# 0xfaded/pislam

Measured on AMD Instinct MI355X. Metric: ORB keypoints+descriptors/sec, 640x480 8-level pyramid, higher is better.
Workload: dtype u8

## Files before the change

### include/pislam_hip.h

```cpp
#ifndef PISLAM_HIP_H_
#define PISLAM_HIP_H_

#include <stddef.h>
#include <stdint.h>

#ifdef __cplusplus
extern "C" {
#endif

#define PISLAM_OK 0
#define PISLAM_ERR_INVALID (-1)
#define PISLAM_ERR_HIP (-2)
#define PISLAM_ERR_NOMEM (-3)
#define PISLAM_ERR_DIST (-4)

#define PISLAM_ABI_VERSION 2

typedef struct pislam_ctx pislam_ctx;

int pislam_abi_version(void);
int pislam_ctx_create(int device, pislam_ctx **ctx);
int pislam_ctx_destroy(pislam_ctx *ctx);
int pislam_ctx_set_stream(pislam_ctx *ctx, void *hip_stream);
int pislam_ctx_set_option(pislam_ctx *ctx, const char *key, int value);
int pislam_ctx_synchronize(pislam_ctx *ctx);
const char *pislam_last_error(const pislam_ctx *ctx);


int pislam_fast_detect(pislam_ctx *ctx, int vstep, int border, int width, int height,
                       const uint8_t *img, uint8_t *out, int threshold);

int pislam_fast_score_harris(pislam_ctx *ctx, int vstep, int border, int width, int height,
                             const uint8_t *img, int32_t threshold, uint8_t *out);

int pislam_fast_extract(pislam_ctx *ctx, int vstep, int border, int logBucketSize,
                        int bucketLimit, int width, int height, const uint8_t *out,
                        uint32_t *results, size_t capacity, size_t *count);

int pislam_orb_compute(pislam_ctx *ctx, int vstep, int words, const uint8_t *img,
                       const uint32_t *points, size_t n, uint32_t *descriptors);


int pislam_harris_score_points(pislam_ctx *ctx, int vstep, const uint8_t *img,
                               const uint32_t *points, size_t n, int32_t threshold,
                               uint8_t *scores);

size_t pislam_centroids_size(size_t n);
int pislam_orb_centroids(pislam_ctx *ctx, int vstep, const uint8_t *img,
                         const uint32_t *points, size_t n, int32_t *centroids);

int pislam_orb_angles(pislam_ctx *ctx, const int32_t *centroids, size_t n8, uint8_t *angles);

int pislam_brief_describe(pislam_ctx *ctx, int vstep, int words, const uint8_t *img,
                          const uint32_t *points, const uint8_t *rots, size_t n,
                          uint32_t *descriptors);

const int8_t *pislam_brief_table(void);


int pislam_gaussian5x5(pislam_ctx *ctx, int vstep, int width, int height, const uint8_t *img,
                       uint8_t *out);

int pislam_bilinear7_8(pislam_ctx *ctx, int vstep, int width, int height, const uint8_t *img,
                       uint8_t *out);
int pislam_bilinear13_16(pislam_ctx *ctx, int vstep, int width, int height, const uint8_t *img,
                         uint8_t *out);

typedef struct pislam_warp pislam_warp;
int pislam_warp_create(pislam_ctx *ctx, int width, int height, int src_width, int src_height, int log_cell,
                       const int32_t *mesh_x, const int32_t *mesh_y, int border, pislam_warp **warp);
int pislam_warp_destroy(pislam_warp *warp);
int pislam_warp_mesh_dims(int width, int height, int log_cell, int32_t *mesh_w, int32_t *mesh_h);
int pislam_warp_info(const pislam_warp *warp, int32_t info[4]);
int pislam_warp_batch(pislam_ctx *ctx, const pislam_warp *warp, const uint8_t *src, int src_vstep, size_t src_stride,
                      uint8_t *dst, int dst_vstep, size_t dst_stride, int batch);


typedef struct pislam_level {
  int32_t width;
  int32_t height;
  int32_t row0;
  int32_t col0;
} pislam_level;

typedef struct pislam_frontend_params {
  int32_t vstep;
  int32_t rows;
  int32_t nlevels;
  int32_t border;
  int32_t fast_threshold;
  int32_t harris_threshold;
  int32_t log_bucket_size;
  int32_t bucket_limit;
  int32_t words;
  int32_t max_keypoints;
} pislam_frontend_params;

int pislam_pyramid_layout(int width, int height, int nlevels, const int32_t *steps, int vstep_min,
                          pislam_level *levels, int32_t *vstep, int32_t *rows);
#define PISLAM_BUILD_BLUR 1
#define PISLAM_BUILD_MARGINS_CLEAN 2
#define PISLAM_BUILD_CHECK_MARGINS 4
int pislam_pyramid_build_batch(pislam_ctx *ctx, int nlevels, const int32_t *steps, const pislam_level *levels,
                               const uint8_t *frames, int frame_vstep, size_t frame_stride, int batch,
                               uint8_t *pyramids, int vstep, int rows, size_t pyramid_stride, int flags);

int pislam_orb_frontend_batch(pislam_ctx *ctx, const pislam_frontend_params *params,
                              const pislam_level *levels, const uint8_t *pyramids,
                              size_t pyramid_stride, int batch, uint32_t *keypoints,
                              uint32_t *descriptors, uint32_t *counts);

int pislam_frontend_reserve(pislam_ctx *ctx, const pislam_frontend_params *params,
                            const pislam_level *levels, int batch);

int pislam_frontend_get_score_map(pislam_ctx *ctx, int b, uint8_t *dst);

int pislam_frontend_last_timing(pislam_ctx *ctx, float *total_ms, float stage_ms[3]);

int pislam_frontend_last_stats(pislam_ctx *ctx, uint32_t stats[2]);

#define PISLAM_PATH_STAGED 1u
#define PISLAM_PATH_FUSED 2u
#define PISLAM_PATH_ONE_LAUNCH 4u
#define PISLAM_PATH_BUCKET_SELECT 8u
#define PISLAM_PATH_BUCKETS_IN_STRIPS 16u
#define PISLAM_PATH_GENERIC_ORB 32u
#define PISLAM_PATH_FRAME_TIMED_OUT 64u
unsigned pislam_frontend_last_path(const pislam_ctx *ctx);
#define PISLAM_COUNT_INVALID 0xffffffffu

int pislam_debug_build_plan(const pislam_frontend_params *params, const pislam_level *levels, int batch, int num_cus,
                            int lanes_in_flight, const char *options, uint32_t summary[8], char *err, size_t err_cap);

typedef struct pislam_pipeline pislam_pipeline;
int pislam_pipeline_create(int device, int depth, pislam_pipeline **pipe);
int pislam_pipeline_destroy(pislam_pipeline *pipe);
int pislam_pipeline_depth(const pislam_pipeline *pipe);
int pislam_pipeline_set_option(pislam_pipeline *pipe, const char *key, int value);
int pislam_pipeline_reserve(pislam_pipeline *pipe, const pislam_frontend_params *params, const pislam_level *levels,
                            int batch);
int pislam_pipeline_submit(pislam_pipeline *pipe, const pislam_frontend_params *params, const pislam_level *levels,
                           const uint8_t *pyramids, size_t pyramid_stride, int batch, uint32_t *keypoints,
                           uint32_t *descriptors, uint32_t *counts, void *input_stream, int order_after_input,
                           uint64_t *ticket);
int pislam_pipeline_wait(pislam_pipeline *pipe, uint64_t ticket, void *stream);
int pislam_pipeline_synchronize(pislam_pipeline *pipe);
int pislam_pipeline_stats(const pislam_pipeline *pipe, uint64_t stats[4]);
void *pislam_pipeline_stream(pislam_pipeline *pipe, uint64_t ticket);
pislam_ctx *pislam_pipeline_lane(pislam_pipeline *pipe, int lane);
const char *pislam_pipeline_last_error(const pislam_pipeline *pipe);

int pislam_debug_shader_clock(pislam_ctx *ctx, int micros, double *ghz);


int pislam_match_hamming(pislam_ctx *ctx, int words, const uint32_t *query, size_t nq,
                         const uint32_t *train, size_t nt, int32_t *idx, uint32_t *dist,
                         uint32_t *dist2);

int pislam_match_hamming_batch(pislam_ctx *ctx, int words, const uint32_t *query,
                               const uint32_t *qcounts, size_t q_stride, const uint32_t *train,
                               const uint32_t *tcounts, size_t t_stride, int batch, int32_t *idx,
                               uint32_t *dist, uint32_t *dist2);

int pislam_match_window_reserve(pislam_ctx *ctx, int words, const pislam_level *levels, int nlevels,
                                const int32_t *radius, size_t t_stride, int batch);
int pislam_match_hamming_window_batch(pislam_ctx *ctx, int words,
                                      const pislam_level *levels, int nlevels, const int32_t *radius,
                                      const uint32_t *qkp, const uint32_t *qdesc, const uint32_t *qcounts,
                                      size_t q_stride, const uint32_t *tkp, const uint32_t *tdesc,
                                      const uint32_t *tcounts, size_t t_stride, int batch, int32_t *idx,
                                      uint32_t *dist, uint32_t *dist2);

int pislam_match_scaled_window_reserve(pislam_ctx *ctx, int words, const pislam_level *levels, int nlevels,
                                       const int32_t *scale_q16, const int32_t *radius0, int level_span,
                                       size_t t_stride, int batch);
int pislam_match_hamming_scaled_window_batch(pislam_ctx *ctx, int words,
                                             const pislam_level *levels, int nlevels,
                                             const int32_t *scale_q16, const int32_t *radius0, int level_span,
                                             const uint32_t *qkp, const uint32_t *qdesc, const uint32_t *qcounts,
                                             const int32_t *qpred, size_t q_stride,
                                             const uint32_t *tkp, const uint32_t *tdesc, const uint32_t *tcounts,
                                             size_t t_stride, int batch, int32_t *idx, uint32_t *dist, uint32_t *dist2);

typedef struct pislam_stereo_params {
  int32_t level_span, min_disp, max_disp, max_hamming, sad_radius, search_radius, median_filter;
} pislam_stereo_params;
int pislam_match_stereo_reserve(pislam_ctx *ctx, int words, const pislam_level *levels, int nlevels,
                                const int32_t *scale_q16, const int32_t *row_radius0, const pislam_stereo_params *p,
                                size_t r_stride, int batch);
int pislam_match_stereo_batch(pislam_ctx *ctx, int words, const pislam_level *levels, int nlevels,
                              const int32_t *scale_q16, const int32_t *row_radius0, const pislam_stereo_params *p,
                              const uint8_t *left_pyr, const uint8_t *right_pyr, int vstep, int rows,
                              size_t pyramid_stride,
                              const uint32_t *lkp, const uint32_t *ldesc, const uint32_t *lcounts, size_t l_stride,
                              const uint32_t *rkp, const uint32_t *rdesc, const uint32_t *rcounts, size_t r_stride,
                              int batch, int32_t *idx, uint32_t *dist, int32_t *disp_q8, uint32_t *sad,
                              uint32_t *nstereo);


typedef struct pislam_vocab pislam_vocab;
int pislam_vocab_create(pislam_ctx *ctx, int words, int nnodes, const uint32_t *node_desc,
                        const int32_t *first_child, const int32_t *child_count, int group_depth,
                        pislam_vocab **vocab);
int pislam_vocab_destroy(pislam_vocab *vocab);
int pislam_vocab_nwords(const pislam_vocab *vocab);
int pislam_vocab_ngroups(const pislam_vocab *vocab);

int pislam_bow_transform_batch(pislam_ctx *ctx, const pislam_vocab *vocab, const uint32_t *desc,
                               const uint32_t *counts, size_t stride, int batch,
                               uint32_t *word, uint32_t *group, uint32_t *wdist);

int pislam_bow_vector_batch(pislam_ctx *ctx, const uint32_t *word, const uint32_t *counts, size_t stride, int batch,
                            uint32_t *bow_word, uint32_t *bow_tf, uint32_t *bow_n);

int pislam_match_bow_reserve(pislam_ctx *ctx, int words, int ngroups, size_t t_stride, int batch);
int pislam_match_hamming_bow_batch(pislam_ctx *ctx, int words, int ngroups,
                                   const uint32_t *qdesc, const uint32_t *qgroup, const uint32_t *qcounts, size_t q_stride,
                                   const uint32_t *tdesc, const uint32_t *tgroup, const uint32_t *tcounts, size_t t_stride,
                                   int batch, int32_t *idx, uint32_t *dist, uint32_t *dist2);


int pislam_orb_angles_batch(pislam_ctx *ctx, const uint8_t *pyramids, int vstep, int rows, size_t pyramid_stride,
                            const uint32_t *keypoints, const uint32_t *counts, size_t stride, int batch,
                            uint8_t *angles);

typedef struct pislam_select_params {
  int32_t max_dist;
  int32_t ratio_num, ratio_den;
  int32_t unique;
  int32_t rot_keep;
  int32_t rot_min_pct;
} pislam_select_params;
int pislam_match_select_batch(pislam_ctx *ctx, const pislam_select_params *p,
                              const int32_t *idx, const uint32_t *dist, const uint32_t *dist2,
                              const uint32_t *qcounts, size_t q_stride,
                              const uint32_t *tcounts, size_t t_stride,
                              const int32_t *back_idx, const uint8_t *qangle, const uint8_t *tangle, int batch,
                              int32_t *sel_q, int32_t *sel_t, uint32_t *nsel, uint8_t *status, uint32_t *rot_hist);


int pislam_bow_weight_batch(pislam_ctx *ctx, const uint32_t *bow_word, const uint32_t *bow_tf, const uint32_t *bow_n,
                            size_t stride, int batch, const uint32_t *idf, uint32_t nwords, uint32_t *bow_weight);

typedef struct pislam_bowdb pislam_bowdb;
int pislam_bowdb_create(pislam_ctx *ctx, uint32_t nwords, size_t stride, int capacity, pislam_bowdb **db);
int pislam_bowdb_destroy(pislam_bowdb *db);
int pislam_bowdb_size(const pislam_bowdb *db);
int pislam_bowdb_add_batch(pislam_ctx *ctx, pislam_bowdb *db, const uint32_t *bow_word, const uint32_t *bow_weight,
                           const uint32_t *bow_n, size_t stride, int batch, int32_t *first_id);
int pislam_bowdb_remove(pislam_ctx *ctx, pislam_bowdb *db, const int32_t *ids, int n);
int pislam_bowdb_clear(pislam_ctx *ctx, pislam_bowdb *db);

int pislam_bowdb_query_reserve(pislam_ctx *ctx, const pislam_bowdb *db, int batch, int topk);
int pislam_bowdb_query_batch(pislam_ctx *ctx, const pislam_bowdb *db, const uint32_t *q_word, const uint32_t *q_weight,
                             const uint32_t *q_n, size_t stride, int batch, const int32_t *id_limit, int min_common_pct,
                             int topk, int32_t *top_id, uint32_t *top_score, uint32_t *top_common, uint32_t *max_common);


#define PISLAM_DIST_ID_BYTES 128

int pislam_dist_shard(int global_batch, int rank, int world, int *first, int *count);

int pislam_dist_get_unique_id(uint8_t id[PISLAM_DIST_ID_BYTES]);

int pislam_dist_init(pislam_ctx *ctx, const uint8_t id[PISLAM_DIST_ID_BYTES], int rank, int world);
int pislam_dist_rank(const pislam_ctx *ctx);
int pislam_dist_world(const pislam_ctx *ctx);
int pislam_dist_comm_count(pislam_ctx *ctx);

int pislam_dist_allgather_counts(pislam_ctx *ctx, const uint32_t *local_counts, size_t n,
                                 uint32_t *all_counts);

int pislam_dist_fence(pislam_ctx *ctx, int back);

int pislam_dist_allgather_counts_on(pislam_ctx *ctx, void *producer_stream, const uint32_t *local_counts, size_t n,
                                    uint32_t *all_counts);
int pislam_dist_fence_on(pislam_ctx *ctx, int back, void *consumer_stream);

int pislam_dist_synchronize(pislam_ctx *ctx);

int pislam_dist_allreduce_max(pislam_ctx *ctx, double *value);

int pislam_dist_finalize(pislam_ctx *ctx);

#ifdef __cplusplus
// ... 4 lines not shown
```

### pislam_amd/capi.py

```python
from __future__ import annotations

import ctypes
import os

import numpy as np

from . import build as _build

PISLAM_OK = 0
ABI_VERSION = 2

_vp, _i, _sz = ctypes.c_void_p, ctypes.c_int, ctypes.c_size_t


class Level(ctypes.Structure):
    _fields_ = [("width", ctypes.c_int32), ("height", ctypes.c_int32),
                ("row0", ctypes.c_int32), ("col0", ctypes.c_int32)]


class FrontendParams(ctypes.Structure):
    _fields_ = [(n, ctypes.c_int32) for n in (
        "vstep", "rows", "nlevels", "border", "fast_threshold", "harris_threshold",
        "log_bucket_size", "bucket_limit", "words", "max_keypoints")]


class StereoParams(ctypes.Structure):
    _fields_ = [(n, ctypes.c_int32) for n in (
        "level_span", "min_disp", "max_disp", "max_hamming", "sad_radius", "search_radius", "median_filter")]


class SelectParams(ctypes.Structure):
    _fields_ = [(n, ctypes.c_int32) for n in (
        "max_dist", "ratio_num", "ratio_den", "unique", "rot_keep", "rot_min_pct")]


SYMBOLS = {
    "pislam_abi_version": (_i, []),
    "pislam_ctx_create": (_i, [_i, ctypes.POINTER(_vp)]),
    "pislam_ctx_destroy": (_i, [_vp]),
    "pislam_ctx_set_stream": (_i, [_vp, _vp]),
    "pislam_ctx_set_option": (_i, [_vp, ctypes.c_char_p, _i]),
    "pislam_ctx_synchronize": (_i, [_vp]),
    "pislam_last_error": (ctypes.c_char_p, [_vp]),
    "pislam_fast_detect": (_i, [_vp, _i, _i, _i, _i, _vp, _vp, _i]),
    "pislam_fast_score_harris": (_i, [_vp, _i, _i, _i, _i, _vp, ctypes.c_int32, _vp]),
    "pislam_fast_extract": (_i, [_vp, _i, _i, _i, _i, _i, _i, _vp, _vp, _sz, ctypes.POINTER(_sz)]),
    "pislam_orb_compute": (_i, [_vp, _i, _i, _vp, _vp, _sz, _vp]),
    "pislam_harris_score_points": (_i, [_vp, _i, _vp, _vp, _sz, ctypes.c_int32, _vp]),
    "pislam_centroids_size": (_sz, [_sz]),
    "pislam_orb_centroids": (_i, [_vp, _i, _vp, _vp, _sz, _vp]),
    "pislam_orb_angles": (_i, [_vp, _vp, _sz, _vp]),
    "pislam_brief_describe": (_i, [_vp, _i, _i, _vp, _vp, _vp, _sz, _vp]),
    "pislam_brief_table": (ctypes.POINTER(ctypes.c_int8), []),
    "pislam_gaussian5x5": (_i, [_vp, _i, _i, _i, _vp, _vp]),
    "pislam_bilinear7_8": (_i, [_vp, _i, _i, _i, _vp, _vp]),
    "pislam_bilinear13_16": (_i, [_vp, _i, _i, _i, _vp, _vp]),
    "pislam_warp_create": (_i, [_vp, _i, _i, _i, _i, _i, _vp, _vp, _i, ctypes.POINTER(_vp)]),
    "pislam_warp_destroy": (_i, [_vp]),
    "pislam_warp_mesh_dims": (_i, [_i, _i, _i, ctypes.POINTER(ctypes.c_int32), ctypes.POINTER(ctypes.c_int32)]),
    "pislam_warp_info": (_i, [_vp, ctypes.POINTER(ctypes.c_int32 * 4)]),
    "pislam_warp_batch": (_i, [_vp, _vp, _vp, _i, _sz, _vp, _i, _sz, _i]),
    "pislam_pyramid_layout": (_i, [_i, _i, _i, ctypes.POINTER(ctypes.c_int32), _i, ctypes.POINTER(Level),
                                   ctypes.POINTER(ctypes.c_int32), ctypes.POINTER(ctypes.c_int32)]),
    "pislam_pyramid_build_batch": (_i, [_vp, _i, ctypes.POINTER(ctypes.c_int32), ctypes.POINTER(Level), _vp, _i, _sz,
                                        _i, _vp, _i, _i, _sz, _i]),
    "pislam_orb_frontend_batch": (_i, [_vp, ctypes.POINTER(FrontendParams), ctypes.POINTER(Level), _vp,
                                       _sz, _i, _vp, _vp, _vp]),
    "pislam_frontend_reserve": (_i, [_vp, ctypes.POINTER(FrontendParams), ctypes.POINTER(Level), _i]),
    "pislam_frontend_get_score_map": (_i, [_vp, _i, _vp]),
    "pislam_frontend_last_timing": (_i, [_vp, ctypes.POINTER(ctypes.c_float),
                                         ctypes.POINTER(ctypes.c_float * 3)]),
    "pislam_frontend_last_stats": (_i, [_vp, ctypes.POINTER(ctypes.c_uint32 * 2)]),
    "pislam_frontend_last_path": (ctypes.c_uint, [_vp]),
    "pislam_debug_build_plan": (_i, [ctypes.POINTER(FrontendParams), ctypes.POINTER(Level), _i, _i, _i, ctypes.c_char_p,
                                     ctypes.POINTER(ctypes.c_uint32 * 8), ctypes.c_char_p, _sz]),
    "pislam_pipeline_create": (_i, [_i, _i, ctypes.POINTER(_vp)]),
    "pislam_pipeline_destroy": (_i, [_vp]),
    "pislam_pipeline_depth": (_i, [_vp]),
    "pislam_pipeline_set_option": (_i, [_vp, ctypes.c_char_p, _i]),
    "pislam_pipeline_reserve": (_i, [_vp, ctypes.POINTER(FrontendParams), ctypes.POINTER(Level), _i]),
    "pislam_pipeline_submit": (_i, [_vp, ctypes.POINTER(FrontendParams), ctypes.POINTER(Level), _vp, _sz, _i, _vp, _vp, _vp,
                                    _vp, _i, ctypes.POINTER(ctypes.c_uint64)]),
    "pislam_pipeline_wait": (_i, [_vp, ctypes.c_uint64, _vp]),
    "pislam_pipeline_synchronize": (_i, [_vp]),
    "pislam_pipeline_stats": (_i, [_vp, ctypes.POINTER(ctypes.c_uint64 * 4)]),
    "pislam_pipeline_stream": (_vp, [_vp, ctypes.c_uint64]),
    "pislam_pipeline_lane": (_vp, [_vp, _i]),
    "pislam_pipeline_last_error": (ctypes.c_char_p, [_vp]),
    "pislam_match_hamming": (_i, [_vp, _i, _vp, _sz, _vp, _sz, _vp, _vp, _vp]),
    "pislam_match_hamming_batch": (_i, [_vp, _i, _vp, _vp, _sz, _vp, _vp, _sz, _i, _vp, _vp, _vp]),
    "pislam_match_window_reserve": (_i, [_vp, _i, ctypes.POINTER(Level), _i, ctypes.POINTER(ctypes.c_int32), _sz, _i]),
    "pislam_match_hamming_window_batch": (_i, [_vp, _i, ctypes.POINTER(Level), _i, ctypes.POINTER(ctypes.c_int32), _vp, _vp,
                                               _vp, _sz, _vp, _vp, _vp, _sz, _i, _vp, _vp, _vp]),
    "pislam_match_scaled_window_reserve": (_i, [_vp, _i, ctypes.POINTER(Level), _i, ctypes.POINTER(ctypes.c_int32),
                                                ctypes.POINTER(ctypes.c_int32), _i, _sz, _i]),
    "pislam_match_hamming_scaled_window_batch": (_i, [_vp, _i, ctypes.POINTER(Level), _i, ctypes.POINTER(ctypes.c_int32),
                                                      ctypes.POINTER(ctypes.c_int32), _i, _vp, _vp, _vp, _vp, _sz, _vp,
                                                      _vp, _vp, _sz, _i, _vp, _vp, _vp]),
    "pislam_match_stereo_reserve": (_i, [_vp, _i, ctypes.POINTER(Level), _i, ctypes.POINTER(ctypes.c_int32),
                                         ctypes.POINTER(ctypes.c_int32), ctypes.POINTER(StereoParams), _sz, _i]),
    "pislam_match_stereo_batch": (_i, [_vp, _i, ctypes.POINTER(Level), _i, ctypes.POINTER(ctypes.c_int32),
                                       ctypes.POINTER(ctypes.c_int32), ctypes.POINTER(StereoParams), _vp, _vp, _i, _i,
                                       _sz, _vp, _vp, _vp, _sz, _vp, _vp, _vp, _sz, _i, _vp, _vp, _vp, _vp, _vp]),
    "pislam_vocab_create": (_i, [_vp, _i, _i, _vp, _vp, _vp, _i, ctypes.POINTER(_vp)]),
    "pislam_vocab_destroy": (_i, [_vp]),
    "pislam_vocab_nwords": (_i, [_vp]),
    "pislam_vocab_ngroups": (_i, [_vp]),
    "pislam_bow_transform_batch": (_i, [_vp, _vp, _vp, _vp, _sz, _i, _vp, _vp, _vp]),
    "pislam_bow_vector_batch": (_i, [_vp, _vp, _vp, _sz, _i, _vp, _vp, _vp]),
    "pislam_match_bow_reserve": (_i, [_vp, _i, _i, _sz, _i]),
    "pislam_match_hamming_bow_batch": (_i, [_vp, _i, _i, _vp, _vp, _vp, _sz, _vp, _vp, _vp, _sz, _i, _vp, _vp, _vp]),
    "pislam_orb_angles_batch": (_i, [_vp, _vp, _i, _i, _sz, _vp, _vp, _sz, _i, _vp]),
    "pislam_match_select_batch": (_i, [_vp, ctypes.POINTER(SelectParams), _vp, _vp, _vp, _vp, _sz, _vp, _sz, _vp, _vp, _vp,
                                       _i, _vp, _vp, _vp, _vp, _vp]),
    "pislam_bow_weight_batch": (_i, [_vp, _vp, _vp, _vp, _sz, _i, _vp, ctypes.c_uint32, _vp]),
    "pislam_bowdb_create": (_i, [_vp, ctypes.c_uint32, _sz, _i, ctypes.POINTER(_vp)]),
    "pislam_bowdb_destroy": (_i, [_vp]),
    "pislam_bowdb_size": (_i, [_vp]),
    "pislam_bowdb_add_batch": (_i, [_vp, _vp, _vp, _vp, _vp, _sz, _i, ctypes.POINTER(ctypes.c_int32)]),
    "pislam_bowdb_remove": (_i, [_vp, _vp, _vp, _i]),
    "pislam_bowdb_clear": (_i, [_vp, _vp]),
    "pislam_bowdb_query_reserve": (_i, [_vp, _vp, _i, _i]),
    "pislam_bowdb_query_batch": (_i, [_vp, _vp, _vp, _vp, _vp, _sz, _i, _vp, _i, _i, _vp, _vp, _vp, _vp]),
    "pislam_dist_shard": (_i, [_i, _i, _i, ctypes.POINTER(_i), ctypes.POINTER(_i)]),
    "pislam_dist_get_unique_id": (_i, [ctypes.c_char_p]),
    "pislam_dist_init": (_i, [_vp, ctypes.c_char_p, _i, _i]),
    "pislam_dist_rank": (_i, [_vp]),
    "pislam_dist_world": (_i, [_vp]),
    "pislam_dist_comm_count": (_i, [_vp]),
    "pislam_dist_allgather_counts": (_i, [_vp, _vp, _sz, _vp]),
    "pislam_dist_fence": (_i, [_vp, _i]),
    "pislam_dist_allgather_counts_on": (_i, [_vp, _vp, _vp, _sz, _vp]),
    "pislam_dist_fence_on": (_i, [_vp, _i, _vp]),
    "pislam_debug_shader_clock": (_i, [_vp, _i, ctypes.POINTER(ctypes.c_double)]),
    "pislam_dist_synchronize": (_i, [_vp]),
    "pislam_dist_allreduce_max": (_i, [_vp, ctypes.POINTER(ctypes.c_double)]),
    "pislam_dist_finalize": (_i, [_vp]),
}

_LIB = None


def library_path() -> str:
    return _build.LIB


def load(rebuild_if_stale: bool = True):
    global _LIB
    if _LIB is not None:
        return _LIB
    try:
        import torch
    except ImportError:
        pass
    _build.check_override()
    path = _build.LIB
    if rebuild_if_stale:
        try:
            path = _build.build()
        except Exception:
            if not os.path.exists(path):
                raise
    if not os.path.exists(path):
        raise ImportError(f"{path} is missing: run `python -m pislam_amd.build` (hipcc, gfx950). "
                          "pislam_amd has no CPU fallback.")
    lib = ctypes.CDLL(path)
    for name, (res, args) in SYMBOLS.items():
        fn = getattr(lib, name)
        fn.restype, fn.argtypes = res, args
    if lib.pislam_abi_version() != ABI_VERSION:
        raise ImportError("libpislam_hip.so ABI version mismatch")
    _LIB = lib
    return lib


class PislamError(RuntimeError):
    pass


def dist_unique_id() -> bytes:
    buf = ctypes.create_string_buffer(128)
    rc = load().pislam_dist_get_unique_id(buf)
    if rc != PISLAM_OK:
        raise PislamError(f"pislam_dist_get_unique_id failed ({rc}): RCCL not loadable?")
    return buf.raw


def dist_shard(global_batch: int, rank: int, world: int):
    first, count = _i(0), _i(0)
    rc = load().pislam_dist_shard(global_batch, rank, world, ctypes.byref(first), ctypes.byref(count))
    if rc != PISLAM_OK:
        raise PislamError(f"pislam_dist_shard failed ({rc})")
    return first.value, first.value + count.value


def ptr(a) -> int:
    if a is None:
        return 0
    if isinstance(a, np.ndarray):
        if not a.flags.c_contiguous:
            raise ValueError("array must be C-contiguous")
        return a.ctypes.data
    if hasattr(a, "data_ptr"):
        if not a.is_contiguous():
            raise ValueError("tensor must be contiguous")
        return a.data_ptr()
    if isinstance(a, int):
        return a
    raise TypeError(f"cannot take the address of {type(a)}")


class Context:

    def __init__(self, device: int = -1, stream: int | None = None):
        self.lib = load()
        h = _vp()
        rc = self.lib.pislam_ctx_create(device, ctypes.byref(h))
        if rc != PISLAM_OK:
            raise PislamError(f"pislam_ctx_create failed ({rc}): no usable HIP device? "
                              "(there is no CPU fallback)")
        self.h = h
        if stream is not None:
            self.set_stream(stream)

    @classmethod
    def borrowed(cls, handle):
        c = cls.__new__(cls)
        c.lib = load()
# ... 137 lines not shown
```

### pislam_amd/csrc/pislam_fused_kernels.h

```cpp
#pragma once
#include "pislam_dev.h"

#ifndef PISLAM_FRAME_SLEEP
#define PISLAM_FRAME_SLEEP 16
#endif
#ifndef PISLAM_OVL
#define PISLAM_OVL 1
#endif
#ifndef PISLAM_DIAG
#define PISLAM_DIAG 1
#endif
#ifndef PISLAM_ORB_PITCH_DW
#define PISLAM_ORB_PITCH_DW 12
#endif

namespace pf {

using namespace pdev;

typedef __attribute__((address_space(3))) uint8_t lds_u8;
typedef __attribute__((address_space(3))) uint32_t lds_u32;
typedef uint32_t u32x4 __attribute__((ext_vector_type(4)));
typedef __attribute__((address_space(3))) u32x4 lds_u4;

constexpr int MAX_ORDER = 160;
constexpr int MAX_LEVELS = 24;
constexpr int WAVES = 4;
constexpr int NT = WAVES * 64;
constexpr int QCAP_G = 128;
constexpr int QCAP_F = 192;
constexpr int QCAP = QCAP_G + QCAP_F;
constexpr int QH_SHARED = 1024;
constexpr int QN_SHARED = 512;
constexpr int QS_SHARED = 256;
constexpr int SHARED_Q = QH_SHARED + QN_SHARED;
constexpr int NMS_SCRATCH = 3 * QS_SHARED;
static_assert(NMS_SCRATCH <= WAVES * QCAP, "NMS scratch must fit the per-wave queue area");
static_assert(QS_SHARED <= NT, "one survivor per thread (ranks are held in a register across a barrier)");
constexpr uint32_t STRIP_DESCRIBED = 0x80000000u;

struct FusedLevel {
  int w, h;
  int row0, col0;
  int R;
  int nstrips;
  int strip0;
  int slot0;
  int nbx;
  int xend;
  int pitch;
  int tpitch;
  int nruns, run0;
  int apad;
  int qh;
  int tbytes;
  uint32_t vpr_recip;
  uint32_t tp_recip;
  int ex0, ex1;
  int xscore;
  int gfirst, gn;
};

struct FusedParams {
  int nlevels, strips_per_pyr, slots_per_pyr;
  int runs_per_pyr, run_len;
  int vstep, rows, border, thr;
  int32_t hthr;
  int batch;
  int lbs, limit;
  int words;
  int orb_in_strip;
  int order_n;
  int dump_score;
  int ablate;
  FusedLevel lv[MAX_LEVELS];
  uint32_t order[MAX_ORDER];
};

__device__ __forceinline__ void lds_barrier() {
  __builtin_amdgcn_fence(__ATOMIC_RELEASE, "workgroup", "local");
  __builtin_amdgcn_s_barrier();
  __builtin_amdgcn_fence(__ATOMIC_ACQUIRE, "workgroup", "local");
}

__device__ __forceinline__ uint32_t lds_add_rtn(uint32_t *p, uint32_t v) {
  uint32_t old;
  const uint32_t a = (uint32_t)(uintptr_t)(lds_u32 *)p;
  asm volatile("ds_add_rtn_u32 %0, %1, %2\n\ts_waitcnt lgkmcnt(0)" : "=v"(old) : "v"(a), "v"(v) : "memory");
  return old;
}

constexpr int PF_MAX = 4;

__device__ __forceinline__ uint32_t pack_xy(int x, int r) { return (uint32_t)x | ((uint32_t)r << 16); }


__device__ __attribute__((noinline)) void harris_overflow(lds_u8 *tile, lds_u8 *sc, int tpitch, int pitch, int32_t hthr,
                                                          bool valid, uint32_t e) {
  if (valid) {
    const int x = e & 0xffff, r = (e >> 16) & 0xff;
    sc[r * pitch + x] = harris_score_mm(tile + r * tpitch + x - 3, tpitch, hthr);
  }
}

constexpr int OWAVES = 4;
constexpr int ORB_PITCH = 4 * PISLAM_ORB_PITCH_DW;
__host__ __device__ constexpr int orb_row_ofs(int r) { return PISLAM_ORB_PITCH_DW == 12 ? r * 48 + 4 * (r >> 3) : r * ORB_PITCH; }
constexpr int ORB_PATCH_BYTES = PISLAM_ORB_PITCH_DW == 12 ? 32 * 48 + 32 : (31 * ORB_PITCH + 4 + 15) / 16 * 16;

__device__ __forceinline__ void half_sum2(int &a, int &b, int half) {
  a += __builtin_amdgcn_update_dpp(0, a, 0x111, 0xf, 0xf, true);
  b += __builtin_amdgcn_update_dpp(0, b, 0x111, 0xf, 0xf, true);
  a += __builtin_amdgcn_update_dpp(0, a, 0x112, 0xf, 0xf, true);
  b += __builtin_amdgcn_update_dpp(0, b, 0x112, 0xf, 0xf, true);
  a += __builtin_amdgcn_update_dpp(0, a, 0x114, 0xf, 0xf, true);
  b += __builtin_amdgcn_update_dpp(0, b, 0x114, 0xf, 0xf, true);
  a += __builtin_amdgcn_update_dpp(0, a, 0x118, 0xf, 0xf, true);
  b += __builtin_amdgcn_update_dpp(0, b, 0x118, 0xf, 0xf, true);
  a += __builtin_amdgcn_update_dpp(0, a, 0x142, 0xa, 0xf, false);
  b += __builtin_amdgcn_update_dpp(0, b, 0x142, 0xa, 0xf, false);
  const int a0 = __builtin_amdgcn_readlane(a, 31), a1 = __builtin_amdgcn_readlane(a, 63);
  const int b0 = __builtin_amdgcn_readlane(b, 31), b1 = __builtin_amdgcn_readlane(b, 63);
  a = half ? a1 : a0;
  b = half ? b1 : b0;
}

#ifndef PISLAM_FETCH_X3
#define PISLAM_FETCH_X3 1
#endif
#if PISLAM_FETCH_X3
constexpr int ORB_NLD = 4;
struct OrbPiece {
  uint32_t x, y, z;
};
struct OrbWin {
  OrbPiece w[ORB_NLD];
};
#else
constexpr int ORB_NLD = 3;
struct OrbWin {
  uint4 w[3];
};
#endif
struct OrbLane {
  int half, r;
  int sl_h[ORB_NLD], sl_park[ORB_NLD], sl_rel[ORB_NLD];
  bool sl_on[ORB_NLD];
  uint32_t m01[8], mdx[8];
};
__device__ __forceinline__ OrbLane orb_lane(int lane, int vstep) {
  OrbLane G;
  G.half = lane >> 5;
  G.r = lane & 31;
  const uint32_t *row = ::g_orb_masks.v[G.r];
#pragma unroll
  for (int k = 0; k < 8; k++) {
    G.m01[k] = row[k];
    G.mdx[k] = row[8 + k];
  }
#if PISLAM_FETCH_X3
#pragma unroll
  for (int j = 0; j < ORB_NLD; j++) {
    const int slot = lane + 64 * j;
    const int q = slot >> 2, k = slot & 3;
    const int h = q >= 31 ? 1 : 0, row = q - 31 * h;
    G.sl_h[j] = h;
    G.sl_on[j] = q < 62;
    G.sl_rel[j] = row * vstep + 12 * k;
    G.sl_park[j] = h * ORB_PATCH_BYTES + orb_row_ofs(row) + 12 * k;
  }
#else
#pragma unroll
  for (int j = 0; j < 3; j++) {
    const int slot = lane + 64 * j;
    const int h = slot >= 93 ? 1 : 0, within = slot - 93 * h;
    const int row = within / 3, chunk = within - 3 * row;
    G.sl_h[j] = h;
    G.sl_on[j] = slot < 186;
    G.sl_rel[j] = row * vstep + 16 * chunk;
    G.sl_park[j] = h * ORB_PATCH_BYTES + orb_row_ofs(row) + 16 * chunk;
  }
#endif
  return G;
}
__device__ __forceinline__ OrbWin orb_fetch(const OrbLane &G, uint32_t p0, uint32_t p1, const uint8_t *__restrict__ im,
                                            int vstep, uint32_t img_bytes32) {
  OrbWin f;
  const int org0 = (decode_y(p0) - 15) * vstep + (decode_x(p0) - 15);
  const int org1 = (decode_y(p1) - 15) * vstep + (decode_x(p1) - 15);
  const int d01 = org1 - org0;
#if PISLAM_FETCH_X3
#pragma unroll
  for (int j = 0; j < ORB_NLD; j++) {
    const uint32_t a = min(((uint32_t)(org0 + (d01 & -G.sl_h[j])) & ~15u) + (uint32_t)G.sl_rel[j], img_bytes32 - 12u);
    f.w[j] = *(const OrbPiece *)(im + a);
  }
#else
#pragma unroll
  for (int j = 0; j < 3; j++) {
    const uint32_t a = min((uint32_t)(org0 + G.sl_rel[j] + (d01 & -G.sl_h[j])) & ~15u, img_bytes32 - 16u);
    f.w[j] = *(const uint4 *)(im + a);
  }
#endif
  return f;
}
template <class TAB, bool GHOOKS = false>
__device__ __forceinline__ void orb_describe_rows(const OrbLane &G, const lds_u8 *prow4, const uint32_t sh3, const lds_u8 *bp,
                                                  const uint32_t *__restrict__ tab_base, const bool valid, const TAB *rtab,
                                                  int words, uint8_t *__restrict__ dst_base, const uint32_t dst_word,
                                                  const int glevel = 0) {
  const int half = G.half, r = G.r;
  uint32_t row[8];
  {
    uint32_t in[9];
#pragma unroll
    for (int k = 0; k < 9; k++) in[k] = *(const lds_u32 *)(prow4 + 4 * k);
#pragma unroll
    for (int k = 0; k < 8; k++) row[k] = __builtin_amdgcn_alignbyte(in[k + 1], in[k], sh3);
  }
  uint32_t sv = 0, left = 0, right = 0;
#pragma unroll
  for (int k = 0; k < 8; k++) sv = __builtin_amdgcn_udot4(row[k], G.m01[k], sv, false);
#pragma unroll
  for (int k = 0; k < 4; k++) left = __builtin_amdgcn_udot4(row[k], G.mdx[k], left, false);
#pragma unroll
  for (int k = 4; k < 8; k++) right = __builtin_amdgcn_udot4(row[k], G.mdx[k], right, false);
  int m10 = (int)right - (int)left, m01 = __mul24(r - 15, (int)sv);
  half_sum2(m10, m01, half);
  if (GHOOKS && glevel == 4) {
    asm volatile("" ::"v"(m10), "v"(m01));
    return;
  }
  const uint32_t rot = angle_bin_fast(m10, m01, rtab);
  if (GHOOKS && glevel == 5) {
    asm volatile("" ::"v"(rot));
    return;
  }
  const uint32_t *tab = tab_base + rot * 256 + r;
  uint32_t ent[8];
#pragma unroll
  for (int t = 0; t < 8; t++) ent[t] = tab[32 * t];
  if (GHOOKS && glevel == 6) {
#pragma unroll
    for (int t = 0; t < 8; t++) asm volatile("" ::"v"(ent[t]));
    return;
  }
  uint32_t pa[8], pb[8];
#pragma unroll
  for (int t = 0; t < 8; t++) pa[t] = bp[ent[t] & 0xffffu], pb[t] = bp[ent[t] >> 16];
  uint32_t acc = 0;
#pragma unroll
  for (int t = 7; t >= 0; t--) acc = __builtin_amdgcn_alignbit(acc, pa[t] - pb[t], 31);
  const uint32_t n1 = (uint32_t)__builtin_amdgcn_update_dpp(0, (int)acc, 0xf5, 0xf, 0xf, true);
  const uint32_t hw = __builtin_amdgcn_perm(n1, acc, 0x0c0c0400u);
  const uint32_t n2 = (uint32_t)__builtin_amdgcn_update_dpp(0, (int)hw, 0xaa, 0xf, 0xf, true);
  const uint32_t word4 = __builtin_amdgcn_perm(n2, hw, 0x05040100u);
  const uint32_t word = (uint32_t)__builtin_amdgcn_ds_bpermute((int)(4u * (32u * (uint32_t)half + 4u * ((uint32_t)r & 7u))), (int)word4);
  if (GHOOKS && glevel == 7) {
    asm volatile("" ::"v"(word));
    return;
  }
  if (valid && r < words) *(uint32_t *)(dst_base + (dst_word * 4u + 4u * (uint32_t)r)) = word;
}

template <class TAB, bool GHOOKS = false>
__device__ __forceinline__ void orb_describe(const OrbLane &G, const OrbWin &cur, uint32_t p0, uint32_t p1,
                                             lds_u8 *wave_patches, int vstep, const TAB *rtab, int words,
                                             uint8_t *__restrict__ dst_base, const uint32_t dst_word, const int glevel = 0) {
  const int half = G.half, r = G.r;
  if (GHOOKS && glevel == 2) {
#pragma unroll
    for (int j = 0; j < ORB_NLD; j++) asm volatile("" ::"v"(cur.w[j].x), "v"(cur.w[j].y), "v"(cur.w[j].z));
    return;
  }
  const uint32_t pme = half ? p1 : p0;
  const bool valid = pme != 0;
  const int x = decode_x(pme), y = decode_y(pme);
  const uint32_t sh = (uint32_t)(x + 1) & 15u;
#pragma unroll
  for (int j = 0; j < ORB_NLD; j++)
    if (G.sl_on[j]) {
      lds_u32 *d = (lds_u32 *)(wave_patches + G.sl_park[j]);
      d[0] = cur.w[j].x;
      d[1] = cur.w[j].y;
      d[2] = cur.w[j].z;
#if !PISLAM_FETCH_X3
      d[3] = cur.w[j].w;
#endif
    }
  if (GHOOKS && glevel == 3) return;
  lds_u8 *patch_l = wave_patches + half * ORB_PATCH_BYTES;
  orb_describe_rows<TAB, GHOOKS>(G, patch_l + orb_row_ofs(r) + (sh & ~3u), sh & 3u, patch_l + sh, ::g_brief_ofs.v, valid, rtab, words,
                                 dst_base, dst_word, glevel);
}

struct StripArgs {
  int border, thr, ablate, dump_score, lbs, limit, vstep, slots_per_pyr, strips_per_pyr;
  int32_t hthr;
  int words, orb;
};

template <bool VEC16, bool HOOKS, bool ALIAS, bool ORBK, bool BUCK>
__device__ __forceinline__ void strip_body(const StripArgs A, const FusedLevel L, const int pyr, const int s,
                                           const int ys, const int ye, lds_u8 *tile0, lds_u8 *sc, lds_u32 *queues,
                                           lds_u32 *shq, uint32_t *sh_ctr, uint32_t *sh_ctr_prev, bool &deferred,
                                           const uint8_t *__restrict__ im, const ptrdiff_t lim,
                                           uint32_t *__restrict__ stage_kp,
                                           uint32_t *__restrict__ strip_count, uint8_t *__restrict__ score_dump,
                                           size_t score_stride, const bool carry, const int tid,
                                           unsigned long long *__restrict__ prof, u32x4 (&pf)[PF_MAX],
                                           const bool pf_have, const bool pf_want, bool &pf_issued,
                                           uint32_t *__restrict__ ovf, const uint32_t ovf_id,
                                           uint32_t *__restrict__ stage_desc, const uint8_t *__restrict__ imb,
                                           const uint32_t img_bytes32) {
  const int B = A.border;
  const int Albs = BUCK ? A.lbs : 0;
  constexpr bool ORB = ALIAS && VEC16 && ORBK;
  const int pitch = L.pitch, tpitch = L.tpitch;
  const int cxa = B, cxb = L.xend;
  const int xbase = (cxa - 4) & ~15;
  lds_u8 *tile = tile0 - xbase;
  long long t_last = 0;
  if (HOOKS && prof) t_last = clock64();
  auto mark = [&](int phase) {
    if (HOOKS && prof && tid == 0) {
      const long long t = clock64();
      (void)__hip_atomic_fetch_add(&prof[phase], (unsigned long long)(t - t_last), __ATOMIC_RELAXED, __HIP_MEMORY_SCOPE_AGENT);
      t_last = t;
    }
  };
  const int lane = tid & 63;
  const int wave = __builtin_amdgcn_readfirstlane(tid >> 6);
  const bool carry_img = carry;
  constexpr bool OVL = PISLAM_OVL && ALIAS && !BUCK && !ORBK;
  const int cwave = OVL ? 1 : 0;
  bool need_sync = true;
  if (carry) {
    const int R = L.R;
    if (carry_img) {
      const int nv = (10 * tpitch) >> 4;
      if (OVL && VEC16 && pf_have) {
        const int i0 = (tid - (R - 10) * (tpitch >> 4)) & (NT - 1);
        for (int i = i0; i < nv; i += NT) ((lds_u4 *)tile0)[i] = ((const lds_u4 *)(tile0 + R * tpitch))[i];
        need_sync = false;
      } else {
        for (int i = tid; i < nv; i += NT) ((lds_u4 *)tile0)[i] = ((const lds_u4 *)(tile0 + R * tpitch))[i];
      }
    }
    if (!ALIAS) {
      const int nvs = (3 * pitch) >> 4;
      for (int i = tid; i < nvs; i += NT) ((lds_u4 *)sc)[i] = ((const lds_u4 *)(sc + R * pitch))[i];
    }
    if (wave == cwave) {
      lds_u32 *qn = ALIAS ? shq : shq + QH_SHARED;
      const int tn = (int)sh_ctr_prev[ALIAS ? 0 : 2];
      int kept = 0;
      for (int c0 = 0; c0 < tn; c0 += 64) {
        const uint32_t e = qn[min(c0 + lane, tn - 1)];
        const bool k = c0 + lane < tn && (int)((e >> 16) & 0xff) >= R && (!ALIAS || (e >> 24) != 0);
        const uint64_t m = __ballot(k);
        if (k) qn[kept + ballot_rank(m)] = e - ((uint32_t)R << 16);
        kept += __popcll(m);
      }
      if (lane < 8)
        sh_ctr[lane] = lane == 1 ? (uint32_t)(ALIAS ? L.qh : QH_SHARED) : (lane == 2 || (ALIAS && lane == 0)) ? (uint32_t)kept : 0u;
    }
    if (need_sync) lds_barrier();
    if (!ALIAS) {
      const int nz = (L.R * pitch) >> 4;
      for (int i = tid; i < nz; i += NT) ((lds_u4 *)(sc + 3 * pitch))[i] = (u32x4)(0u);
    }
  } else {
    if (!ALIAS) {
      const int nz = ((L.R + 3) * pitch) >> 4;
      for (int i = tid; i < nz; i += NT) ((lds_u4 *)sc)[i] = (u32x4)(0u);
    }
    if (tid < 8) sh_ctr[tid] = tid == 1 ? (uint32_t)(ALIAS ? L.qh : QH_SHARED) : 0u;
  }
  lds_u32 *qg = queues + wave * QCAP;
  lds_u32 *qf = qg + QCAP_G;
  lds_u32 *shq_h = shq;
  lds_u32 *shq_n = shq_h + QH_SHARED;
  const int qcap = ALIAS ? L.qh : QH_SHARED;
  int ng = 0, nf = 0;
  const int thr = A.thr;
  const int32_t hthr = A.hthr;
  const int ablate = HOOKS ? A.ablate : 0;
  const int Lw = L.w, Lxend = L.xend, Lh = L.h;
  const bool wmod = (Lw & 15) != 0;

  auto push_nonzero = [&](bool nz, uint32_t e) {
    const uint64_t m = __ballot(nz);
    if (m) {
      const int cnt = __popcll(m);
      int base = 0;
      if (lane == 0) base = (int)lds_add_rtn(&sh_ctr[2], (uint32_t)cnt);
      base = __builtin_amdgcn_readfirstlane(base);
      if (base + cnt <= QN_SHARED) {
        if (nz) shq_n[base + ballot_rank(m)] = e;
      } else if (lane == 0) {
        sh_ctr[3] = 1;
        sh_ctr[7] |= 2;
      }
    }
  };
  auto harris_batch = [&](bool valid, uint32_t e, int at) {
    uint8_t score = 0;
    if (ALIAS) {
      if (valid) {
        const int r = (int)__umulhi(e, L.tp_recip);
        const int x = (int)e - r * tpitch + xbase;
        score = x >= L.xscore ? (uint8_t)0xff : (ablate & 32) ? (uint8_t)200 : harris_score_mm(tile0 + e - 3, tpitch, hthr);
        shq_h[at] = (uint32_t)x | ((uint32_t)r << 16) | ((uint32_t)score << 24);
      }
    } else {
      if (valid) {
        const int x = e & 0xffff, r = (e >> 16) & 0xff;
        score = (ablate & 32) ? (uint8_t)200 : harris_score_mm(tile + r * tpitch + x - 3, tpitch, hthr);
        sc[r * pitch + x] = score;
      }
      push_nonzero(score != 0, e);
    }
  };
  const lds_u8 *tile3 = tile0 + 3 * tpitch;
  const uint32_t tp_recip = L.tp_recip;
  auto fast_batch = [&](bool valid, uint32_t k) {
    bool corner = false;
    if (valid) corner = fast9_mm(tile3 + k, tpitch, thr);
    uint32_t e = k;
    bool toh = corner;
    if (!ALIAS) {
      const int r = (int)__umulhi(k, tp_recip);
      const int x = (int)k - r * tpitch + xbase;
      e = (uint32_t)x | ((uint32_t)r << 16);
      toh = corner && x < L.xscore;
      if (corner && !toh) sc[r * pitch + x] = 0xff;
      push_nonzero(corner && !toh, e);
    }
    const bool q = ALIAS ? corner : toh;
    const uint64_t m = __ballot(q);
    if (m) {
      const int cnt = __popcll(m);
      int base = 0;
      if (lane == 0) base = (int)lds_add_rtn(&sh_ctr[0], (uint32_t)cnt);
      base = __builtin_amdgcn_readfirstlane(base);
      if (base + cnt <= qcap) {
        if (q) shq_h[base + ballot_rank(m)] = e;
      } else {
        if (lane == 0) {
          atomicMin(&sh_ctr[1], (uint32_t)base);
          sh_ctr[3] = 1;
          sh_ctr[7] |= 1;
        }
        if (!ALIAS) harris_overflow(tile, sc, tpitch, pitch, hthr, toh, e);
      }
    }
  };

  const int r_lo = carry ? 3 : (ys - 1 < B) ? 1 : 0;
  const int r_hi = min(ye + 2, Lh - B) - (ys - 1);
  const uint32_t nkb4 = ~((uint32_t)min(128 + ((thr + 1) >> 1), 255) * 0x01010101u);
  const uint32_t nkd4 = ~((uint32_t)(129 - ((thr + 2) >> 1)) * 0x01010101u);
  const bool aligned4 = ((B | Lxend) & 3) == 0;

  const uint32_t cspan = (uint32_t)((cxb + 3) & ~3) - (uint32_t)(cxa & ~3);
  const int xrel = xbase - (cxa & ~3);
  const uint32_t grp_base = (uint32_t)(uintptr_t)(tile3 - 4);
  auto pretest_batch = [&](const bool lane_valid, const uint32_t grp) {
    const uint32_t key = grp - grp_base;
    const int x0r = (int)key - (int)__umulhi(key, tp_recip) * tpitch + xrel;
    const bool valid = lane_valid && (uint32_t)x0r < cspan;
    const int x0 = x0r + (cxa & ~3);
    const lds_u8 *pb = (const lds_u8 *)(uintptr_t)grp;
    const uint32_t wl = *(const lds_u32 *)pb;
    const uint32_t wc = *(const lds_u32 *)(pb + 4);
    const uint32_t wr = *(const lds_u32 *)(pb + 8);
    const uint32_t wu = *(const lds_u32 *)(pb + 4 - 3 * tpitch);
    const uint32_t wd = *(const lds_u32 *)(pb + 4 + 3 * tpitch);
    const uint32_t nC = ~wc;
    const uint32_t hU = __builtin_amdgcn_lerp(wu, nC, 0x01010101u), hD = __builtin_amdgcn_lerp(wd, nC, 0x01010101u);
    const uint32_t hL = __builtin_amdgcn_lerp(__builtin_amdgcn_alignbyte(wc, wl, 1), nC, 0x01010101u);
    const uint32_t hR = __builtin_amdgcn_lerp(__builtin_amdgcn_alignbyte(wr, wc, 3), nC, 0x01010101u);
    const uint32_t bU = __builtin_amdgcn_lerp(hU, nkb4, 0x01010101u), bD = __builtin_amdgcn_lerp(hD, nkb4, 0x01010101u);
    const uint32_t bL = __builtin_amdgcn_lerp(hL, nkb4, 0x01010101u), bR = __builtin_amdgcn_lerp(hR, nkb4, 0x01010101u);
    const uint32_t dU = __builtin_amdgcn_lerp(hU, nkd4, 0x01010101u), dD = __builtin_amdgcn_lerp(hD, nkd4, 0x01010101u);
    const uint32_t dL = __builtin_amdgcn_lerp(hL, nkd4, 0x01010101u), dR = __builtin_amdgcn_lerp(hR, nkd4, 0x01010101u);
    uint32_t bright = (bU | bD) & (bL | bR);
    uint32_t notdark = (dU & dD) | (dL & dR);
#if PISLAM_DIAG
    {
      const lds_u8 *pu2 = pb - 2 * tpitch, *pd2 = pb + 2 * tpitch;
      const uint32_t ul = *(const lds_u32 *)pu2, uc = *(const lds_u32 *)(pu2 + 4), ur = *(const lds_u32 *)(pu2 + 8);
      const uint32_t dl = *(const lds_u32 *)pd2, dc = *(const lds_u32 *)(pd2 + 4), dr = *(const lds_u32 *)(pd2 + 8);
      const uint32_t h15 = __builtin_amdgcn_lerp(__builtin_amdgcn_alignbyte(uc, ul, 2), nC, 0x01010101u);
      const uint32_t h3 = __builtin_amdgcn_lerp(__builtin_amdgcn_alignbyte(ur, uc, 2), nC, 0x01010101u);
      const uint32_t h11 = __builtin_amdgcn_lerp(__builtin_amdgcn_alignbyte(dc, dl, 2), nC, 0x01010101u);
      const uint32_t h7 = __builtin_amdgcn_lerp(__builtin_amdgcn_alignbyte(dr, dc, 2), nC, 0x01010101u);
      const uint32_t b3 = __builtin_amdgcn_lerp(h3, nkb4, 0x01010101u), b11 = __builtin_amdgcn_lerp(h11, nkb4, 0x01010101u);
      const uint32_t b7 = __builtin_amdgcn_lerp(h7, nkb4, 0x01010101u), b15 = __builtin_amdgcn_lerp(h15, nkb4, 0x01010101u);
      const uint32_t d3 = __builtin_amdgcn_lerp(h3, nkd4, 0x01010101u), d11 = __builtin_amdgcn_lerp(h11, nkd4, 0x01010101u);
      const uint32_t d7 = __builtin_amdgcn_lerp(h7, nkd4, 0x01010101u), d15 = __builtin_amdgcn_lerp(h15, nkd4, 0x01010101u);
      bright &= (b3 | b11) & (b7 | b15);
      notdark |= (d3 & d11) | (d7 & d15);
    }
#endif
    const uint32_t pass = bright | ~notdark;
    uint64_t m0, m1, m2, m3;
    asm volatile("v_cmp_gt_i32_sdwa %0, 0, sext(%4) src0_sel:DWORD src1_sel:BYTE_0\n\t"
                 "v_cmp_gt_i32_sdwa %1, 0, sext(%4) src0_sel:DWORD src1_sel:BYTE_1\n\t"
                 "v_cmp_gt_i32_sdwa %2, 0, sext(%4) src0_sel:DWORD src1_sel:BYTE_2\n\t"
                 "v_cmp_gt_i32_e64 %3, 0, %4\n\ts_nop 1"
        : "=&s"(m0), "=&s"(m1), "=&s"(m2), "=&s"(m3)
        : "v"(valid ? pass : 0u));
    if (!aligned4) {
      m0 &= __ballot(x0 + 0 >= cxa && x0 + 0 < cxb);
      m1 &= __ballot(x0 + 1 >= cxa && x0 + 1 < cxb);
      m2 &= __ballot(x0 + 2 >= cxa && x0 + 2 < cxb);
      m3 &= __ballot(x0 + 3 >= cxa && x0 + 3 < cxb);
    }
    if ((m0 | m1 | m2 | m3) == 0) return;
    const bool p0 = __builtin_amdgcn_inverse_ballot_w64(m0), p1 = __builtin_amdgcn_inverse_ballot_w64(m1);
    const bool p2 = __builtin_amdgcn_inverse_ballot_w64(m2), p3 = __builtin_amdgcn_inverse_ballot_w64(m3);
    {
      lds_u32 *q = qf + nf;
      if (p0) q[ballot_rank(m0)] = key;
      q += __popcll(m0);
      if (p1) q[ballot_rank(m1)] = key + 1;
      nf += __popcll(m0) + __popcll(m1);
    }
    while (nf >= 64) {
      nf -= 64;
      if (!(ablate & 2)) fast_batch(true, qf[nf + lane]);
    }
    {
      lds_u32 *q = qf + nf;
      if (p2) q[ballot_rank(m2)] = key + 2;
      q += __popcll(m2);
      if (p3) q[ballot_rank(m3)] = key + 3;
      nf += __popcll(m2) + __popcll(m3);
    }
    while (nf >= 64) {
      nf -= 64;
      if (!(ablate & 2)) fast_batch(true, qf[nf + lane]);
    }
  };

  int h_begin = 0;
  {
    {
      const int y_lo = ys - 4;
      const int nrows = min(ye + 6, Lh) - y_lo;
      const int r_st0 = carry_img ? 10 : 0;
      if (carry_img && (ablate & 2048)) {
      } else if (VEC16 && carry_img && pf_have) {
        const int nvec = (nrows - 10) * (tpitch >> 4);
        lds_u4 *dstv = (lds_u4 *)(tile0 + 10 * tpitch) + tid;
#pragma unroll
        for (int k = 0; k < PF_MAX; k++)
          if (tid + NT * k < nvec) dstv[NT * k] = pf[k];
      } else if (VEC16) {
        const int vpr = tpitch >> 4;
        const int nvec = (nrows - r_st0) * vpr;
        const int gap = A.vstep - tpitch;
        const uint8_t *src0 = im + (uint32_t)((y_lo + r_st0) * A.vstep + xbase);
        lds_u4 *dstv = (lds_u4 *)(tile0 + r_st0 * tpitch);
        const bool tail = (uint32_t)((y_lo + nrows - 1) * A.vstep + xbase + tpitch) > (uint32_t)lim;
        if (!tail) {
          constexpr int ST_MAX = 6;
          for (int i0 = tid; i0 < nvec; i0 += NT * ST_MAX) {
            u32x4 st[ST_MAX];
#pragma unroll
            for (int k = 0; k < ST_MAX; k++) {
              const int i = i0 + NT * k;
              if (i < nvec) {
                const int row = (int)__umulhi((uint32_t)i, L.vpr_recip);
                st[k] = *(const u32x4 *)(src0 + (uint32_t)(16 * i + row * gap));
              }
            }
#pragma unroll
            for (int k = 0; k < ST_MAX; k++)
              if (i0 + NT * k < nvec) dstv[i0 + NT * k] = st[k];
          }
        } else {
          for (int i = tid; i < nvec; i += NT) {
            const int row = (int)__umulhi((uint32_t)i, L.vpr_recip);
            const ptrdiff_t off = (ptrdiff_t)(y_lo + r_st0) * A.vstep + xbase + (ptrdiff_t)16 * i + (ptrdiff_t)row * gap;
            u32x4 d;
            if (off + 16 <= lim) {
              d = *(const u32x4 *)(im + off);
            } else {
              uint32_t w0 = 0, w1 = 0, w2 = 0, w3 = 0;
#pragma unroll
              for (int k = 0; k < 16; k++) {
                const uint32_t b = off + k < lim ? (uint32_t)im[off + k] << (8 * (k & 3)) : 0u;
                if (k < 4) w0 |= b; else if (k < 8) w1 |= b; else if (k < 12) w2 |= b; else w3 |= b;
              }
              d = (u32x4){w0, w1, w2, w3};
            }
            dstv[i] = d;
          }
        }
      } else {
        for (int i = r_st0 * tpitch + tid; i < nrows * tpitch; i += NT) {
          const int r = i / tpitch, cx = i - r * tpitch;
          const ptrdiff_t off = (ptrdiff_t)(y_lo + r) * A.vstep + xbase + cx;
          tile0[r * tpitch + cx] = off < lim ? im[off] : (uint8_t)0;
        }
      }
    }
    lds_barrier();
    mark(0);
    if (ALIAS) h_begin = (int)sh_ctr[2];
    pf_issued = false;
    if (VEC16 && pf_want && L.R >= 10 && L.R * (tpitch >> 4) <= PF_MAX * NT) {
      const int vpr = tpitch >> 4;
      const int ylo_n = ye - 4, ye_n = min(ye + L.R, Lh - B);
      const int nrows_n = min(ye_n + 6, Lh) - ylo_n;
      if ((uint32_t)((ylo_n + nrows_n - 1) * A.vstep + xbase + tpitch) <= (uint32_t)lim) {
        const int nvec_n = (nrows_n - 10) * vpr, gap = A.vstep - tpitch;
        const uint8_t *src_n = im + (uint32_t)((ylo_n + 10) * A.vstep + xbase);
#pragma unroll
        for (int k = 0; k < PF_MAX; k++) {
          const int i = tid + NT * k;
          if (i < nvec_n) pf[k] = *(const u32x4 *)(src_n + (uint32_t)(16 * i + (int)__umulhi((uint32_t)i, L.vpr_recip) * gap));
        }
        pf_issued = true;
      }
    }
    if (ablate & 1) return;

    const int lin_lo = r_lo * tpitch, lin_n = max(r_hi - r_lo, 0) * tpitch;
    const int nfull = lin_n >> 8, rem = lin_n & 255;
    const uint32_t thr1x2 = (uint32_t)(thr + 1) * 0x10001u;
    auto prefilter_step = [&](const lds_u8 *pm, const lds_u8 *pu, const lds_u8 *pd, bool lane_ok) {
      const uint32_t wl = *(const lds_u32 *)pm;
      const uint32_t wc = *(const lds_u32 *)(pm + 4);
      const uint32_t wr = *(const lds_u32 *)(pm + 8);
      const uint32_t wu = *(const lds_u32 *)pu;
      const uint32_t wd = *(const lds_u32 *)pd;
      const uint32_t a = __builtin_amdgcn_sad_hi_u8(__builtin_amdgcn_alignbyte(wc, wl, 1), wc, __builtin_amdgcn_sad_u8(wu, wc, 0u));
      const uint32_t b = __builtin_amdgcn_sad_hi_u8(__builtin_amdgcn_alignbyte(wr, wc, 3), wc, __builtin_amdgcn_sad_u8(wd, wc, 0u));
      typedef unsigned short us2v __attribute__((ext_vector_type(2)));
      const uint32_t mm = __builtin_bit_cast(uint32_t, __builtin_elementwise_max(__builtin_bit_cast(us2v, a), __builtin_bit_cast(us2v, b)));
      const uint32_t mn = __builtin_bit_cast(uint32_t, __builtin_elementwise_min(__builtin_bit_cast(us2v, mm), __builtin_bit_cast(us2v, thr1x2)));
      const bool g = lane_ok && (mn == thr1x2);
      const uint64_t m = __ballot(g);
      if (m == 0) return;
      if (g) qg[ng + ballot_rank(m)] = (uint32_t)(uintptr_t)pm;
      ng += __popcll(m);
      if (ng >= 64) {
        ng -= 64;
        if (!(ablate & 16)) pretest_batch(true, qg[ng + lane]);
      }
    };
    {
      const lds_u8 *pm = tile3 + lin_lo + 256 * wave + 4 * lane - 4;
      const lds_u8 *pu = pm + 4 - 3 * tpitch, *pd = pm + 4 + 3 * tpitch;
      for (int st = wave; st < nfull; st += WAVES) {
        prefilter_step(pm, pu, pd, true);
        pm += 256 * WAVES;
        pu += 256 * WAVES;
        pd += 256 * WAVES;
      }
      if (rem && (nfull & (WAVES - 1)) == wave) prefilter_step(pm, pu, pd, 4 * lane < rem);
    }
    if (ng > 0 && !(ablate & 16)) pretest_batch(lane < ng, lane < ng ? qg[lane] : grp_base + (uint32_t)lin_lo);
    ng = 0;
    if (nf > 0 && !(ablate & 2)) fast_batch(lane < nf, qf[min(lane, nf - 1)]);
    nf = 0;
    lds_barrier();
    mark(1);
    {
      const int th = (int)min(sh_ctr[0], sh_ctr[1]);
      if (!(ablate & 4))
        for (int c0 = h_begin + wave * 64; c0 < th; c0 += WAVES * 64) {
          const int at = min(c0 + lane, th - 1);
          harris_batch(c0 + lane < th, shq_h[at], at);
        }
    }
    lds_barrier();
    mark(2);
  }
  tile = tile0;
  if ((ablate & 512) && tid == 0) sh_ctr[3] = 1;
  if (ablate & 512) lds_barrier();
  auto defer = [&]() {
    deferred = true;
    if (tid == 0) {
      const uint32_t at = atomicAdd(&ovf[0], 1u);
      if (ovf_id != 0xffffffffu) ovf[2 + at] = ovf_id;
      if (HOOKS && prof) prof[5] += (sh_ctr[7] & 1 ? 1ull : 0ull) + (sh_ctr[7] & 2 ? 1ull << 20 : 0ull) +
                                    (sh_ctr[7] & 4 ? 1ull << 40 : 0ull);
      sh_ctr[6] = 1;
    }
  };
  if (ALIAS) {
    if (sh_ctr[3] != 0) {
      defer();
      return;
    }
    const int nz = ((L.R + 3) * pitch) >> 4;
    for (int i = tid; i < nz; i += NT) ((lds_u4 *)sc)[i] = (u32x4)(0u);
    lds_barrier();
    const int tn = (int)sh_ctr[0];
    for (int i = tid; i < tn; i += NT) {
      const uint32_t e = shq_h[i];
      if (e >> 24) sc[(int)((e >> 16) & 0xff) * pitch + (int)(e & 0xffff)] = (uint8_t)(e >> 24);
    }
    lds_barrier();
  }

  if (HOOKS && A.dump_score) {
    uint8_t *dst = score_dump + (size_t)pyr * score_stride + (size_t)L.row0 * A.vstep + L.col0;
    for (int i = tid; i < (ye - ys) * pitch; i += NT) {
      const int r = i / pitch, x = i - r * pitch;
      if (x >= B && x < max(Lxend, wmod ? Lw + 2 : 0)) dst[(ptrdiff_t)(ys + r) * A.vstep + x] = sc[(r + 1) * pitch + x];
    }
  }

  if (ablate & 8) return;
  if (sh_ctr[3] == 0) {
    lds_u32 *shq_s = queues;
    lds_u32 *shq_k = shq_s + QS_SHARED;
    const int tn = (int)sh_ctr[ALIAS ? 0 : 2];
    const lds_u32 *nq = ALIAS ? shq_h : shq_n;
    const int own_rows = ye - ys;
    const int ex0q = L.ex0, ex1q = L.ex1;
    for (int c0 = wave * 64; c0 < tn; c0 += WAVES * 64) {
      const uint32_t e = nq[min(c0 + lane, tn - 1)];
      const bool valid = c0 + lane < tn && (!ALIAS || (e >> 24) != 0);
      const int x = e & 0xffff, r = (e >> 16) & 0xff;
      const int bx = B + ((x - B) & ~1);
      const bool owned = valid && r >= 1 && r <= own_rows && bx >= ex0q && bx < ex1q;
      uint32_t res = 0;
      if (owned) {
        const int cb = (x - 1) & ~3;
        const uint32_t shb = (uint32_t)(x - 1) & 3u;
        uint32_t w[3];
#pragma unroll
        for (int k = 0; k < 3; k++) {
          const lds_u8 *rowp = sc + (r - 1 + k) * pitch + cb;
          w[k] = __builtin_amdgcn_alignbyte(*(const lds_u32 *)(rowp + 4), *(const lds_u32 *)rowp, shb);
        }
        const uint32_t me = (w[1] >> 8) & 0xffu;
        const uint32_t rep = me * 0x01010101u;
        const uint32_t before = __builtin_amdgcn_perm(w[1], w[0], 0x04020100u);
        const uint32_t after = __builtin_amdgcn_perm(w[2], w[1], 0x06050402u);
        const uint32_t ge = __builtin_amdgcn_lerp(rep, ~before, 0x01010101u);
        const uint32_t le = __builtin_amdgcn_lerp(after, ~rep, 0x01010101u);
        if (((~ge | le) & 0x80808080u) == 0) res = encode_fast(me, (uint32_t)x, (uint32_t)(ys - 1 + r));
      }
      const uint64_t m = __ballot(res != 0);
      if (m) {
        const int cnt = __popcll(m);
        int base = 0;
        if (lane == 0) base = (int)lds_add_rtn(&sh_ctr[4], (uint32_t)cnt);
        base = __builtin_amdgcn_readfirstlane(base);
        if (base + cnt <= QS_SHARED) {
          if (res) {
            const int slot_i = base + ballot_rank(m);
            shq_s[slot_i] = res;
            shq_k[slot_i] = ((uint32_t)(decode_y(res) - B) >> 1) << 12 | ((uint32_t)(decode_x(res) - B) >> 1);
          }
        } else if (lane == 0) {
          sh_ctr[7] |= 4;
          sh_ctr[3] = 2;
        }
      }
    }
    lds_barrier();
    mark(3);
    if (sh_ctr[3] == 0) {
      if (ablate & 128) return;
      const int ns = (int)sh_ctr[4];
      const size_t strip_slot = (size_t)pyr * A.slots_per_pyr + L.slot0 + (size_t)s * (L.R >> 1) * L.nbx;
      const uint32_t add_xy = ((uint32_t)L.col0 << 12) | (uint32_t)L.row0;
      const bool orb = ORB && A.orb != 0;
      auto describe_strip = [&](const int n, const uint32_t my_rank) {
        lds_u8 *patches = (lds_u8 *)queues + NMS_SCRATCH * 4;
        lds_u8 *rtab = patches + WAVES * 2 * ORB_PATCH_BYTES;
        lds_barrier();
        if (tid < n) shq_k[tid] = my_rank;
        rtab[tid] = ::g_vrecpe_tab.v[tid & 255];
        lds_barrier();
        const OrbLane G = orb_lane(lane, A.vstep);
        lds_u8 *wave_patches = patches + wave * 2 * ORB_PATCH_BYTES;
        uint32_t *dbase = stage_desc + ((size_t)pyr * A.strips_per_pyr + L.strip0 + s) * (size_t)(QS_SHARED * A.words);
        for (int it = wave; 2 * it < n; it += WAVES) {
          const int i0 = 2 * it, i1 = min(i0 + 1, n - 1);
          const uint32_t r0 = shq_k[i0], r1 = i0 + 1 < n ? shq_k[i1] : 0xffffffffu;
          const uint32_t p0 = r0 != 0xffffffffu ? shq_s[i0] + add_xy : 0u;
          const uint32_t p1 = r1 != 0xffffffffu ? shq_s[i1] + add_xy : 0u;
          if ((p0 | p1) == 0) continue;
          const OrbWin w = orb_fetch(G, p0, p1, imb, A.vstep, img_bytes32);
          orb_describe(G, w, p0, p1, wave_patches, A.vstep, (const lds_u8 *)rtab, A.words, (uint8_t *)dbase,
                       (G.half ? r1 : r0) * (uint32_t)A.words);
        }
      };
      if (Albs == 0) {
        uint32_t my_rank = 0;
        if (ns <= 64) {
          if (wave == 0) {
            const uint32_t key = lane < ns ? shq_k[lane] : 0xffffffffu;
            int rank = 0;
            int r1 = 0, r2 = 0, r3 = 0;
            for (int j = 0; j < ns; j += 4) {
              rank += (uint32_t)__builtin_amdgcn_readlane((int)key, j) < key;
              r1 += (uint32_t)__builtin_amdgcn_readlane((int)key, j + 1) < key;
              r2 += (uint32_t)__builtin_amdgcn_readlane((int)key, j + 2) < key;
              r3 += (uint32_t)__builtin_amdgcn_readlane((int)key, j + 3) < key;
            }
            rank += r1 + r2 + r3;
            if (lane < ns) stage_kp[strip_slot + rank] = shq_s[lane] + add_xy;
            my_rank = (uint32_t)rank;
          }
        } else {
          for (int i = tid; i < ns; i += NT) {
            const uint32_t key = shq_k[i];
            int rank = 0;
            for (int j = 0; j < ns; j++) rank += shq_k[j] < key;
            stage_kp[strip_slot + rank] = shq_s[i] + add_xy;
            my_rank = (uint32_t)rank;
          }
        }
        if (tid == 0)
          strip_count[(size_t)pyr * A.strips_per_pyr + L.strip0 + s] = (uint32_t)ns | (orb ? STRIP_DESCRIBED : 0u);
        mark(4);
        if (orb && ns > 0) describe_strip(ns, my_rank);
        return;
      }
      const int lbs = Albs, limit = A.limit;
      if (ns <= 64) {
        uint32_t my_rank = 0xffffffffu;
        uint32_t kept = 0;
        if (wave == 0) {
          const uint32_t v = lane < ns ? shq_s[lane] : 0u;
          const uint32_t cell = lane < ns ? ((((uint32_t)(decode_y(v) - B) >> lbs) << 12) | ((uint32_t)(decode_x(v) - B) >> lbs)) : 0xffffffffu;
          int greater = 0, g1 = 0, less = 0, l1 = 0;
          for (int j = 0; j < ns; j += 2) {
            const uint32_t c0 = (uint32_t)__builtin_amdgcn_readlane((int)cell, j), v0 = (uint32_t)__builtin_amdgcn_readlane((int)v, j);
            const uint32_t c1 = (uint32_t)__builtin_amdgcn_readlane((int)cell, j + 1), v1 = (uint32_t)__builtin_amdgcn_readlane((int)v, j + 1);
            greater += (c0 == cell) & (v0 > v);
            g1 += (c1 == cell) & (v1 > v);
            less += (c0 < cell) | ((c0 == cell) & (v0 < v));
            l1 += (c1 < cell) | ((c1 == cell) & (v1 < v));
          }
          greater += g1;
          int rank = less + l1;
          const bool keep = lane < ns && greater < limit;
          const uint64_t km = __ballot(keep);
          uint64_t dm = __ballot(lane < ns && !keep);
          while (dm) {
            const int j = __builtin_ctzll(dm);
            dm &= dm - 1;
            const uint32_t cj = (uint32_t)__builtin_amdgcn_readlane((int)cell, j), vj = (uint32_t)__builtin_amdgcn_readlane((int)v, j);
            rank -= (cj < cell) | ((cj == cell) & (vj < v));
          }
          if (keep) {
            stage_kp[strip_slot + rank] = v + add_xy;
            my_rank = (uint32_t)rank;
          }
          kept = (uint32_t)__popcll(km);
        }
        if (tid == 0) strip_count[(size_t)pyr * A.strips_per_pyr + L.strip0 + s] = kept | (orb ? STRIP_DESCRIBED : 0u);
        mark(4);
        if (orb && ns > 0) describe_strip(ns, my_rank);
        return;
      }
      for (int i = tid; i < ns; i += NT) {
        const uint32_t v = shq_s[i];
        const uint32_t cell = (((uint32_t)(decode_y(v) - B) >> lbs) << 12) | ((uint32_t)(decode_x(v) - B) >> lbs);
        shq_k[i] = cell;
      }
      lds_barrier();
      lds_u32 *keep = shq_k + QS_SHARED;
      for (int i = tid; i < ns; i += NT) {
        const uint32_t v = shq_s[i], cell = shq_k[i];
        int greater = 0;
        for (int j = 0; j < ns; j++) greater += (shq_k[j] == cell) & (shq_s[j] > v);
        keep[i] = greater < limit;
      }
      lds_barrier();
      int kept_here = 0;
      uint32_t my_rank = 0xffffffffu;
      for (int i = tid; i < ns; i += NT) {
        if (!keep[i]) continue;
        const uint32_t v = shq_s[i], cell = shq_k[i];
        int rank = 0;
        for (int j = 0; j < ns; j++)
          rank += keep[j] & ((shq_k[j] < cell) | ((shq_k[j] == cell) & (shq_s[j] < v)));
        stage_kp[strip_slot + rank] = v + add_xy;
        my_rank = (uint32_t)rank;
        kept_here++;
      }
      if (kept_here) atomicAdd(&sh_ctr[5], (uint32_t)kept_here);
      lds_barrier();
      if (tid == 0) strip_count[(size_t)pyr * A.strips_per_pyr + L.strip0 + s] = sh_ctr[5] | (orb ? STRIP_DESCRIBED : 0u);
      if (orb && ns > 0) describe_strip(ns, my_rank);
      return;
    }
  }
  if constexpr (ALIAS) {
    defer();
    return;
  } else {
  if (tid == 0) sh_ctr[6] = 1;
  if (Albs != 0) {
    const int lbs = Albs, limit = A.limit, bs = 1 << lbs, hb = bs >> 1;
    const int cx0 = (L.ex0 - B) >> lbs;
    const int ncx = (L.ex1 - B - 1) / bs + 1 - cx0;
    const int ncy = (ye - ys + bs - 1) / bs;
    const int ncell = ncx * ncy, nblk = hb * hb;
    const int capc = min(limit, nblk);
    lds_u32 *cellres = (lds_u32 *)tile0;
    lds_u32 *cellcnt = cellres + ncell * capc;
    lds_u32 *cand = queues + wave * QCAP;
    const int xlimc = L.ex1;
    for (int cell = wave; cell < ncell; cell += WAVES) {
      const int cy = cell / ncx, cx = cx0 + (cell - cy * ncx);
      for (int i = lane; i < nblk; i += 64) {
        const int by = i / hb, bxi = i - by * hb;
        const int x = B + cx * bs + 2 * bxi, y = ys + cy * bs + 2 * by;
        uint32_t r0 = 0;
        if (x < xlimc && y < ye) r0 = nms_block(sc + (y - ys + 1) * pitch + x, pitch, x, y);
        cand[i] = r0;
      }
      int nf_c = 0;
      for (int k = 0; k < capc; k++) {
        uint32_t best = 0;
        for (int i = lane; i < nblk; i += 64) best = max(best, cand[i]);
        best = wave_max_u32(best);
        if (best == 0) break;
        for (int i = lane; i < nblk; i += 64)
          if (cand[i] == best) cand[i] = 0;
        if (lane == 0) cellres[cell * capc + k] = best;
        nf_c++;
      }
      if (lane == 0) cellcnt[cell] = (uint32_t)nf_c;
    }
    lds_barrier();
    const size_t strip_slot = (size_t)pyr * A.slots_per_pyr + L.slot0 + (size_t)s * (L.R >> 1) * L.nbx;
    const uint32_t add_xy = ((uint32_t)L.col0 << 12) | (uint32_t)L.row0;
    for (int cell = wave; cell < ncell; cell += WAVES) {
      const uint32_t n = cellcnt[cell];
      if (n == 0) continue;
      uint32_t off = 0;
      for (int k = lane; k < cell; k += 64) off += cellcnt[k];
      off = (uint32_t)wave_sum((int)off);
      if ((uint32_t)lane < n) stage_kp[strip_slot + off + lane] = cellres[cell * capc + (n - 1 - lane)] + add_xy;
    }
    if (wave == 0) {
      uint32_t tot = 0;
      for (int k = lane; k < ncell; k += 64) tot += cellcnt[k];
      tot = (uint32_t)wave_sum((int)tot);
      if (lane == 0) strip_count[(size_t)pyr * A.strips_per_pyr + L.strip0 + s] = tot;
    }
    return;
  }
  __shared__ uint32_t rowcnt[64];
  const int nbr = (ye - ys + 1) >> 1;
  const int xlim = L.ex1, xfirst = L.ex0;
  const int nbx = L.nbx;
  lds_u32 *rowbuf = (lds_u32 *)tile0;
  auto nms_pair = [&](const lds_u8 *srow, int x0, int y, uint32_t &ra, uint32_t &rb) {
    ra = rb = 0;
    const uint32_t m = *(const lds_u32 *)(srow + x0) | *(const lds_u32 *)(srow + pitch + x0);
    if (m != 0) {
      const lds_u8 *p0 = srow - pitch + x0;
      uint32_t a[4], b[4];
#pragma unroll
      for (int k = 0; k < 4; k++) {
        const uint32_t wl = *(const lds_u32 *)(p0 + k * pitch - 4), wc = *(const lds_u32 *)(p0 + k * pitch),
                       wr = *(const lds_u32 *)(p0 + k * pitch + 4);
        a[k] = __builtin_amdgcn_alignbyte(wc, wl, 3);
        b[k] = __builtin_amdgcn_alignbyte(wr, wc, 1);
      }
      const uint32_t a0 = a[0], a1 = a[1], a2 = a[2], a3 = a[3], b0 = b[0], b1 = b[1], b2 = b[2], b3 = b[3];
      if (x0 < xlim) ra = nms_block_regs(a0, a1, a2, a3, x0, y);
      if (x0 + 2 < xlim) rb = nms_block_regs(b0, b1, b2, b3, x0 + 2, y);
    }
  };
  const bool pairs = (xfirst & 3) == 0;
  for (int br = wave; br < nbr; br += WAVES) {
    const lds_u8 *srow = sc + (2 * br + 1) * pitch;
    lds_u32 *rb_out = rowbuf + br * nbx;
    uint32_t cnt = 0;
    if (pairs) {
      for (int x0 = xfirst + 4 * lane; x0 - 4 * lane < xlim; x0 += 256) {
        uint32_t ra, rb;
        nms_pair(srow, x0, ys + 2 * br, ra, rb);
        const uint64_t ma = __ballot(ra != 0), mb = __ballot(rb != 0);
        if ((ma | mb) == 0) continue;
        const uint32_t pos = cnt + ballot_rank(ma) + ballot_rank(mb);
        if (ra) rb_out[pos] = ra;
        if (rb) rb_out[pos + (ra != 0)] = rb;
        cnt += __popcll(ma) + __popcll(mb);
      }
    } else {
      for (int bx0 = 0; bx0 < nbx; bx0 += 64) {
        const int bx = bx0 + lane;
        uint32_t res = 0;
        if (xfirst + 2 * bx < xlim) res = nms_block(srow + xfirst + 2 * bx, pitch, xfirst + 2 * bx, ys + 2 * br);
        const uint64_t m = __ballot(res != 0);
        if (res) rb_out[cnt + ballot_rank(m)] = res;
        cnt += __popcll(m);
      }
    }
    if (lane == 0) rowcnt[br] = cnt;
  }
  lds_barrier();
  if (ablate & 128) return;
  const size_t strip_slot = (size_t)pyr * A.slots_per_pyr + L.slot0 + (size_t)s * (L.R >> 1) * nbx;
  const uint32_t add_xy = ((uint32_t)L.col0 << 12) | (uint32_t)L.row0;
  for (int br = wave; br < nbr; br += WAVES) {
    const uint32_t n = rowcnt[br];
    if (n == 0) continue;
    uint32_t off = 0;
    for (int k = 0; k < br; k++) off += rowcnt[k];
    for (uint32_t k = lane; k < n; k += 64) stage_kp[strip_slot + off + k] = rowbuf[br * nbx + k] + add_xy;
  }
  if (tid == 0) {
    uint32_t tot = 0;
    for (int k = 0; k < nbr; k++) tot += rowcnt[k];
    strip_count[(size_t)pyr * A.strips_per_pyr + L.strip0 + s] = tot;
  }
  }
}

struct StripLds {
  lds_u8 *tile, *sc;
  lds_u32 *queues, *shq;
};
template <bool ALIAS>
__device__ __forceinline__ StripLds strip_lds(uint8_t *smem, const FusedLevel &L) {
  StripLds m;
  if (ALIAS) {
    m.queues = (lds_u32 *)smem;
    m.sc = (lds_u8 *)smem + NMS_SCRATCH * 4;
    m.tile = (lds_u8 *)smem + WAVES * QCAP * 4 + L.apad;
    m.shq = (lds_u32 *)(m.tile + (L.R + 10) * L.tpitch);
  } else {
    m.tile = (lds_u8 *)smem;
    m.sc = m.tile + L.tbytes;
    m.queues = (lds_u32 *)(m.sc + (L.R + 3) * L.pitch);
    m.shq = m.queues + WAVES * QCAP;
  }
  return m;
}

template <bool VEC16, bool HOOKS, bool ALIAS, bool ORBK, bool BUCK, bool INLINE_OVF = false>
__device__ __forceinline__ void strips_role(const FusedParams &P, const uint8_t *__restrict__ pyramids, size_t pyr_stride,
                                            uint32_t *__restrict__ stage_kp, uint32_t *__restrict__ strip_count,
                                            uint8_t *__restrict__ score_dump, size_t score_stride,
                                            unsigned long long *__restrict__ prof, uint32_t *__restrict__ ovf,
                                            uint32_t *__restrict__ stage_desc, uint8_t *smem, uint32_t *sh_ctr, const int pyr,
                                            int run) {
  int li = 0;
  if (P.order_n > 0) {
    const uint32_t o = P.order[run];
    li = (int)(o >> 16);
    run = (int)(o & 0xffffu);
  } else {
    while (li + 1 < P.nlevels && run >= P.lv[li + 1].run0) li++;
    run -= P.lv[li].run0;
  }
  const int s0 = run * P.run_len, s1 = min(s0 + P.run_len, P.lv[li].nstrips);
  long long t_wg = 0;
  if (HOOKS && prof) {
    prof += (size_t)blockIdx.x * 8;
    t_wg = clock64();
  }
  bool carry = false, pf_have = false;
  unsigned long long redo = 0;
  u32x4 pf[PF_MAX];
#pragma unroll
  for (int k = 0; k < PF_MAX; k++) pf[k] = (u32x4)(0u);
  for (int s = s0; s < s1; s++) {
    int li_o = li, tid_o = (int)threadIdx.x;
    asm volatile("" : "+s"(li_o));
    asm volatile("" : "+v"(tid_o));
    const FusedLevel L = P.lv[li_o];
    const StripLds m = strip_lds<ALIAS>(smem, L);
    const uint8_t *im = pyramids + (size_t)pyr * pyr_stride + (size_t)L.row0 * P.vstep + L.col0;
    const ptrdiff_t lim = (ptrdiff_t)P.rows * P.vstep - ((ptrdiff_t)L.row0 * P.vstep + L.col0);
    StripArgs A{P.border, P.thr, P.ablate, P.dump_score, P.lbs, P.limit, P.vstep, P.slots_per_pyr,
                P.strips_per_pyr, P.hthr, P.words, P.orb_in_strip};
    asm volatile("" : "+s"(A.border), "+s"(A.thr), "+s"(A.lbs), "+s"(A.limit), "+s"(A.vstep), "+s"(A.slots_per_pyr),
                 "+s"(A.strips_per_pyr), "+s"(A.hthr), "+s"(A.words), "+s"(A.orb));
    const int ys = A.border + s * L.R;
    const int ye = min(ys + L.R, L.h - A.border);
    constexpr bool OVL = PISLAM_OVL && ALIAS && !BUCK && !ORBK;
    uint32_t *ctr = sh_ctr + (OVL ? 8 * (s & 1) : 0), *ctr_prev = sh_ctr + (OVL ? 8 * ((s & 1) ^ 1) : 0);
    bool deferred = false;
    strip_body<VEC16, HOOKS, ALIAS, ORBK, BUCK>(A, L, pyr, s, ys, ye, m.tile, m.sc, m.queues, m.shq, ctr, ctr_prev, deferred, im, lim,
                                    stage_kp, strip_count, score_dump, score_stride, carry, tid_o, prof, pf, pf_have, s + 1 < s1,
                                    pf_have, ovf, INLINE_OVF ? 0xffffffffu : ((uint32_t)pyr << 16) | (uint32_t)(L.strip0 + s), stage_desc,
                                    pyramids + (size_t)pyr * pyr_stride, (uint32_t)((size_t)P.rows * P.vstep));
    if (INLINE_OVF && ALIAS && deferred) redo |= 1ull << (s - s0);
    if (s + 1 < s1) {
      if (OVL && !(HOOKS && (P.ablate & 0xfbf))) {
        if (deferred) lds_barrier();
        carry = !deferred && L.R >= 10;
      } else {
        lds_barrier();
        carry = ctr[6] == 0 && L.R >= 10 && !(HOOKS && (P.ablate & 1024));
        lds_barrier();
      }
      if (HOOKS && prof && threadIdx.x == 0) prof[6] += 1ull;
    }
  }
  if (HOOKS && prof && threadIdx.x == 0) prof[7] += (unsigned long long)(clock64() - t_wg);
  if (INLINE_OVF && ALIAS) {
    redo = ((unsigned long long)(uint32_t)__builtin_amdgcn_readfirstlane((int)(uint32_t)redo)) |
           ((unsigned long long)(uint32_t)__builtin_amdgcn_readfirstlane((int)(uint32_t)(redo >> 32)) << 32);
    while (redo) {
      const int s = s0 + __builtin_ctzll(redo);
      redo &= redo - 1;
      lds_barrier();
      int li_o = li, tid_o = (int)threadIdx.x;
      asm volatile("" : "+s"(li_o));
      asm volatile("" : "+v"(tid_o));
      const FusedLevel L = P.lv[li_o];
      const StripLds m2 = strip_lds<false>(smem, L);
      const uint8_t *im = pyramids + (size_t)pyr * pyr_stride + (size_t)L.row0 * P.vstep + L.col0;
      const ptrdiff_t lim = (ptrdiff_t)P.rows * P.vstep - ((ptrdiff_t)L.row0 * P.vstep + L.col0);
      const StripArgs A{P.border, P.thr, 0, 0, P.lbs, P.limit, P.vstep, P.slots_per_pyr, P.strips_per_pyr, P.hthr, P.words, 0};
      const int ys = A.border + s * L.R, ye = min(ys + L.R, L.h - A.border);
      bool d2 = false, issued = false;
      strip_body<VEC16, false, false, false, true>(A, L, pyr, s, ys, ye, m2.tile, m2.sc, m2.queues, m2.shq, sh_ctr, sh_ctr, d2, im, lim,
                                                   stage_kp, strip_count, nullptr, 0, false, tid_o, nullptr, pf, false, false, issued,
                                                   nullptr, 0u, nullptr, nullptr, 0u);
    }
  }
}

template <bool VEC16, bool HOOKS, bool ALIAS, bool ORBK = false, bool BUCK = true>
__global__ __launch_bounds__(NT) void k_fused_strips(
    const FusedParams P, const uint8_t *__restrict__ pyramids, size_t pyr_stride,
    uint32_t *__restrict__ stage_kp, uint32_t *__restrict__ strip_count,
    uint8_t *__restrict__ score_dump, size_t score_stride, unsigned long long *__restrict__ prof,
    uint32_t *__restrict__ ovf, uint32_t *__restrict__ stage_desc) {
  extern __shared__ __attribute__((aligned(16))) uint8_t smem[];
  __shared__ uint32_t sh_ctr[16];
  const int xcd = blockIdx.x & 7, slot = blockIdx.x >> 3;
  const int groups = (P.batch + 7) >> 3;
  const int pyr = (slot % groups) * 8 + xcd;
  if (pyr >= P.batch) return;
  strips_role<VEC16, HOOKS, ALIAS, ORBK, BUCK>(P, pyramids, pyr_stride, stage_kp, strip_count, score_dump, score_stride, prof, ovf,
                                         stage_desc, smem, sh_ctr, pyr, slot / groups);
}

template <bool VEC16, bool HOOKS>
__global__ __launch_bounds__(NT) void k_fused_overflow(
    const FusedParams P, const uint8_t *__restrict__ pyramids, size_t pyr_stride,
    uint32_t *__restrict__ stage_kp, uint32_t *__restrict__ strip_count,
    uint8_t *__restrict__ score_dump, size_t score_stride, const uint32_t *__restrict__ ovf) {
  extern __shared__ __attribute__((aligned(16))) uint8_t smem[];
  __shared__ uint32_t sh_ctr[8];
  const uint32_t n = ovf[0];
  u32x4 pf[PF_MAX];
#pragma unroll
  for (int k = 0; k < PF_MAX; k++) pf[k] = (u32x4)(0u);
  for (uint32_t it = blockIdx.x; it < n; it += gridDim.x) {
    const uint32_t id = ovf[2 + it];
    int pyr_o = (int)(id >> 16), sg_o = (int)(id & 0xffffu), tid_o = (int)threadIdx.x;
    asm volatile("" : "+s"(pyr_o), "+s"(sg_o));
    asm volatile("" : "+v"(tid_o));
    if (pyr_o >= P.batch || sg_o >= P.strips_per_pyr) continue;
    int li = 0;
    while (li + 1 < P.nlevels && sg_o >= P.lv[li + 1].strip0) li++;
    const FusedLevel L = P.lv[li];
    const int s = sg_o - L.strip0;
    const StripLds m = strip_lds<false>(smem, L);
    const uint8_t *im = pyramids + (size_t)pyr_o * pyr_stride + (size_t)L.row0 * P.vstep + L.col0;
    const ptrdiff_t lim = (ptrdiff_t)P.rows * P.vstep - ((ptrdiff_t)L.row0 * P.vstep + L.col0);
    const StripArgs A{P.border, P.thr, P.ablate, P.dump_score, P.lbs, P.limit, P.vstep, P.slots_per_pyr,
                      P.strips_per_pyr, P.hthr, P.words, 0};
    const int ys = A.border + s * L.R;
    const int ye = min(ys + L.R, L.h - A.border);
    bool issued = false;
    bool deferred = false;
    strip_body<VEC16, HOOKS, false, false, true>(A, L, pyr_o, s, ys, ye, m.tile, m.sc, m.queues, m.shq, sh_ctr, sh_ctr, deferred, im, lim, stage_kp,
                                    strip_count, score_dump, score_stride, false, tid_o, nullptr, pf, false, false, issued,
                                    nullptr, 0u, nullptr, nullptr, 0u);
    lds_barrier();
  }
}

struct PlanStrip {
  int li;
  int s;
};
__device__ __forceinline__ PlanStrip plan_strip(const FusedParams &P, int i) {
  int li = 0;
  while (li + 1 < P.nlevels && i >= P.lv[li + 1].strip0) li++;
  return {li, i - P.lv[li].strip0};
}
__device__ __forceinline__ uint32_t strip_slot_of(const FusedParams &P, int li, int s) {
  return (uint32_t)(P.lv[li].slot0 + s * (P.lv[li].R >> 1) * P.lv[li].nbx);
}
template <class OFF>
__device__ __forceinline__ uint32_t final_position(const FusedParams &P, const OFF *soff, const uint32_t *__restrict__ stage,
                                                   int li, int s, uint32_t k, uint32_t v) {
  const int gn = P.lv[li].gn;
  if (gn == 1) return soff[P.lv[li].strip0 + s] + k;
  const int g0 = P.lv[li].gfirst;
  const int shift = P.lbs ? P.lbs : 1;
  const int r = (decode_y(v) - P.lv[li].row0 - P.border) >> shift;
  uint32_t pos = soff[P.lv[g0].strip0] + k;
  for (int t = 0; t < gn; t++) {
    const int e = g0 + t, j = P.lv[e].strip0 + s;
    pos += soff[j] - soff[P.lv[e].strip0];
    if (e == li) continue;
    const int lim = r + (e < li ? 1 : 0);
    const uint32_t *list = stage + strip_slot_of(P, e, s);
    uint32_t lo = 0, hi = soff[j + 1] - soff[j];
    while (lo < hi) {
      const uint32_t m = (lo + hi) >> 1;
      if (((decode_y(list[m]) - P.lv[e].row0 - P.border) >> shift) < lim) lo = m + 1; else hi = m;
    }
    pos += lo;
  }
  return pos;
}

__global__ __launch_bounds__(256) void k_gather(const FusedParams P,
                                                const uint32_t *__restrict__ stage_kp,
                                                const uint32_t *__restrict__ strip_count,
                                                uint32_t *__restrict__ kp, size_t kp_stride,
                                                uint32_t cap, uint32_t *__restrict__ counts,
                                                uint32_t *__restrict__ ovf_reset) {
  extern __shared__ uint32_t soff[];
  __shared__ uint32_t wsum[4];
  __shared__ uint32_t carry;
  if (ovf_reset && blockIdx.x == 0 && threadIdx.x == 0) {
    ovf_reset[1] = ovf_reset[0];
    ovf_reset[0] = 0;
  }
  const int pyr = blockIdx.x, tid = threadIdx.x, lane = tid & 63, wv = tid >> 6;
  const int S = P.strips_per_pyr;
  const uint32_t *cnt = strip_count + (size_t)pyr * S;
  if (tid == 0) carry = 0;
  __syncthreads();
  for (int base = 0; base < S; base += 256) {
    const int i = base + tid;
    const uint32_t v = i < S ? (cnt[i] & ~STRIP_DESCRIBED) : 0;
    uint32_t incl = v;
#pragma unroll
    for (int d = 1; d < 64; d <<= 1) {
      const uint32_t t = (uint32_t)__shfl_up((int)incl, d, 64);
      if (lane >= d) incl += t;
    }
    if (lane == 63) wsum[wv] = incl;
    __syncthreads();
    uint32_t pre = carry;
    for (int w = 0; w < wv; w++) pre += wsum[w];
    if (i < S) soff[i] = pre + incl - v;
    __syncthreads();
    if (tid == 255) carry = pre + incl;
    __syncthreads();
  }
  if (tid == 0) {
    soff[S] = carry;
    counts[pyr] = carry;
  }
  __syncthreads();
  const uint32_t *stage = stage_kp + (size_t)pyr * P.slots_per_pyr;
  for (int st = wv; st < S; st += 4) {
    const uint32_t n = soff[st + 1] - soff[st];
    if (n == 0) continue;
    const PlanStrip ps = plan_strip(P, st);
    const uint32_t *list = stage + strip_slot_of(P, ps.li, ps.s);
    for (uint32_t k = lane; k < n; k += 64) {
      const uint32_t v = list[k];
      const uint32_t pos = final_position(P, soff, stage, ps.li, ps.s, k, v);
      if (pos < cap) kp[(size_t)pyr * kp_stride + pos] = v;
    }
  }
}

struct SelectPlan {
  int nlevels, lbs, limit, border;
  int units_per_pyr, uslots_per_pyr;
  int row0[16], col0[16], h[16];
  int g0[16], gn[16];
  int unit0[16], nunits[16];
  int cap[16], uslot0[16];
  int nb_max;
};
static_assert(sizeof(FusedParams) + sizeof(SelectPlan) + 5 * sizeof(void *) <= 4096, "k_bucket_select's arguments exceed the 4 KiB kernarg segment");
constexpr int SEL_WAVES = 4;
constexpr int SEL_NB = 1024;
constexpr int SEL_REC = 24, SEL_ML = 6;
__global__ __launch_bounds__(64 * SEL_WAVES) void k_bucket_select(const FusedParams F, const SelectPlan Q,
                                                                   const uint32_t *__restrict__ stage_kp,
                                                                   const uint32_t *__restrict__ strip_count,
                                                                   uint32_t *__restrict__ ustage, uint32_t *__restrict__ ucount,
                                                                   const uint32_t *__restrict__ utab) {
  extern __shared__ uint32_t sel_lds[];
  const int lane = threadIdx.x & 63, wv = __builtin_amdgcn_readfirstlane((int)(threadIdx.x >> 6));
  uint32_t *sbuf = sel_lds + (size_t)wv * (64 + 2 * Q.nb_max);
  uint32_t *bcnt = sbuf + 64, *bpre = bcnt + Q.nb_max;
  const int pyr = blockIdx.y, u = (int)blockIdx.x * SEL_WAVES + wv;
  if (u >= Q.units_per_pyr) return;
  const uint32_t *rec = utab + (size_t)u * SEL_REC;
  const int nl_rec = (int)rec[0], l = (int)rec[1], cr = (int)rec[2];
  const int lbs = Q.lbs, limit = Q.limit, B = Q.border;
  const int y0 = B + (cr << lbs), y1 = min(y0 + (1 << lbs), Q.h[l] - B);
  const int yrow0 = (int)rec[4] - B, xcol0 = (int)rec[5];
  const uint32_t *stage = stage_kp + (size_t)pyr * F.slots_per_pyr;
  const uint32_t *cnt = strip_count + (size_t)pyr * F.strips_per_pyr;
  uint32_t *out = ustage + (size_t)pyr * Q.uslots_per_pyr + rec[3];
  auto for_each_chunk = [&](auto f) {
    for (int t = 0; t < Q.gn[l]; t++) {
      const int e = Q.g0[l] + t, R = F.lv[e].R;
      const int s_lo = (y0 - B) / R, s_hi = min((y1 - 1 - B) / R, F.lv[e].nstrips - 1);
      for (int sidx = s_lo; sidx <= s_hi; sidx++) {
        const uint32_t n = cnt[F.lv[e].strip0 + sidx] & ~STRIP_DESCRIBED;
        const uint32_t *list = stage + F.lv[e].slot0 + (size_t)sidx * (R >> 1) * F.lv[e].nbx;
        for (uint32_t q0 = 0; q0 < n; q0 += 64) {
          const uint32_t q = q0 + (uint32_t)lane;
          const uint32_t v = q < n ? list[q] : 0u;
          f(v, q < n && (int)((uint32_t)(decode_y(v) - yrow0 - B) >> lbs) == cr);
        }
      }
    }
  };
  auto bucket_of = [&](uint32_t v) -> uint32_t { return (uint32_t)(decode_x(v) - xcol0) >> lbs; };
  int n_unit = 0;
  auto collect = [&](uint32_t v, bool in) {
    const uint64_t m = __ballot(in);
    if (in) {
      const int at = n_unit + ballot_rank(m);
      if (at < 64) sbuf[at] = v;
    }
    n_unit += __popcll(m);
  };
  constexpr int ML = SEL_ML;
  if (nl_rec >= 0 && nl_rec <= ML) {
    const int nl = nl_rec;
    uint32_t vj[ML], nj[ML];
#pragma unroll
    for (int j = 0; j < ML; j++)
      if (j < nl) {
        nj[j] = cnt[rec[16 + j]] & ~STRIP_DESCRIBED;
        vj[j] = stage[rec[8 + j] + (uint32_t)lane];
      }
#pragma unroll
    for (int j = 0; j < ML; j++)
      if (j < nl) {
        const uint32_t n = nj[j];
        collect(vj[j], (uint32_t)lane < n && (int)((uint32_t)(decode_y(vj[j]) - yrow0 - B) >> lbs) == cr);
        const uint32_t *list = stage + rec[8 + j];
        for (uint32_t q0 = 64; q0 < n; q0 += 64) {
          const uint32_t q = q0 + (uint32_t)lane;
          const uint32_t v = q < n ? list[q] : 0u;
          collect(v, q < n && (int)((uint32_t)(decode_y(v) - yrow0 - B) >> lbs) == cr);
        }
      }
  } else {
    for_each_chunk(collect);
  }
  if (n_unit == 0) {
    if (lane == 0) ucount[(size_t)pyr * Q.units_per_pyr + u] = 0;
    return;
  }
  if (n_unit <= 64) {
    const uint32_t v = lane < n_unit ? sbuf[lane] : 0u;
    const uint32_t b = lane < n_unit ? bucket_of(v) : 0xffffffffu;
    int greater = 0, g1 = 0, less = 0, l1 = 0;
    for (int j = 0; j < n_unit; j += 2) {
      const uint32_t b0 = (uint32_t)__builtin_amdgcn_readlane((int)b, j), v0 = (uint32_t)__builtin_amdgcn_readlane((int)v, j);
      const uint32_t b1 = (uint32_t)__builtin_amdgcn_readlane((int)b, j + 1), v1 = (uint32_t)__builtin_amdgcn_readlane((int)v, j + 1);
      greater += (b0 == b) & (v0 > v);
      g1 += (b1 == b) & (v1 > v);
      less += (b0 < b) | ((b0 == b) & (v0 < v));
      l1 += (b1 < b) | ((b1 == b) & (v1 < v));
    }
    greater += g1;
    int rank = less + l1;
    const bool keep = lane < n_unit && greater < limit;
    const uint64_t km = __ballot(keep);
    uint64_t dm = __ballot(lane < n_unit && !keep);
    while (dm) {
      const int j = __builtin_ctzll(dm);
      dm &= dm - 1;
      const uint32_t bj = (uint32_t)__builtin_amdgcn_readlane((int)b, j), vj = (uint32_t)__builtin_amdgcn_readlane((int)v, j);
      rank -= (bj < b) | ((bj == b) & (vj < v));
    }
    if (keep) out[rank] = v;
    if (lane == 0) ucount[(size_t)pyr * Q.units_per_pyr + u] = (uint32_t)__popcll(km);
    return;
  }
  const int ncx = Q.cap[l] / limit;
  for (int i = lane; i < ncx; i += 64) bcnt[i] = 0;
  for_each_chunk([&](uint32_t v, bool in) {
    if (in) atomicAdd(&bcnt[bucket_of(v)], 1u);
  });
  constexpr int PER = SEL_NB / 64;
  uint32_t sum = 0;
  for (int k = 0; k < PER; k++) {
    const int i = PER * lane + k;
    sum += i < ncx ? min(bcnt[i], (uint32_t)limit) : 0u;
  }
  uint32_t incl = sum;
#pragma unroll
  for (int d = 1; d < 64; d <<= 1) {
    const uint32_t t = (uint32_t)__shfl_up((int)incl, d, 64);
    if (lane >= d) incl += t;
  }
  const uint32_t total = (uint32_t)__builtin_amdgcn_readlane((int)incl, 63);
  uint32_t run = incl - sum;
  for (int k = 0; k < PER; k++) {
    const int i = PER * lane + k;
    if (i < ncx) {
      bpre[i] = run;
      run += min(bcnt[i], (uint32_t)limit);
    }
  }
  for_each_chunk([&](uint32_t v, bool in) {
    const uint32_t b = in ? bucket_of(v) : 0xffffffffu;
    int greater = 0, smaller = 0;
    for_each_chunk([&](uint32_t w, bool win) {
      const uint32_t bw = win ? bucket_of(w) : 0xfffffffeu;
      for (int j = 0; j < 64; j++) {
        const uint32_t bj = (uint32_t)__builtin_amdgcn_readlane((int)bw, j), wj = (uint32_t)__builtin_amdgcn_readlane((int)w, j);
        greater += (bj == b) & (wj > v);
        smaller += (bj == b) & (wj < v);
      }
    });
    if (in && greater < limit) {
      const uint32_t c = bcnt[b];
      out[bpre[b] + (uint32_t)smaller - (c - min(c, (uint32_t)limit))] = v;
    }
  });
  if (lane == 0) ucount[(size_t)pyr * Q.units_per_pyr + u] = total;
}

struct OrbShared {
  uint32_t wsum[4];
  uint32_t carry, ntodo, flag, pad;
  uint8_t rtab[256];
};
__host__ __device__ constexpr size_t orb_lds_bytes(int strips_per_pyr, size_t per_max) {
  return sizeof(OrbShared) + (size_t)OWAVES * 2 * ORB_PATCH_BYTES + sizeof(uint32_t) * (((size_t)strips_per_pyr + 1 + 3) & ~(size_t)3) +
         sizeof(uint32_t) * (((size_t)strips_per_pyr + 3) & ~(size_t)3) +
         sizeof(uint32_t) * 2 * per_max;
}

struct NoWait {
  __device__ __forceinline__ bool operator()() const { return true; }
};
template <class WAIT = NoWait, bool GHOOKS = false>
__device__ __forceinline__ void orb_role(const FusedParams &P, const uint8_t *__restrict__ pyramids, size_t pyr_stride,
                                         const uint32_t *__restrict__ stage_kp, const uint32_t *__restrict__ strip_count,
                                         const uint32_t *__restrict__ stage_desc, uint32_t *__restrict__ kp, size_t kp_stride,
                                         uint32_t cap, uint32_t *__restrict__ counts, uint32_t *__restrict__ desc,
                                         size_t desc_stride, int words, uint32_t per_max, uint8_t *osm_all, const int pyr,
                                         const int ch, const int nch, WAIT wait_producers = WAIT()) {
  OrbShared *sh = (OrbShared *)osm_all;
  uint8_t *osm = osm_all + sizeof(OrbShared);
  sh->rtab[threadIdx.x] = ::g_vrecpe_tab.v[threadIdx.x];
  const lds_u8 *rtab = (const lds_u8 *)sh->rtab;
  const int tid = threadIdx.x, lane = tid & 63;
  const int wv = __builtin_amdgcn_readfirstlane(tid >> 6);
  const int S = P.strips_per_pyr;
  const OrbLane G = orb_lane(lane, P.vstep);
  if (!wait_producers()) return;
  uint8_t *patches = osm;
  uint32_t *soff = (uint32_t *)(osm + OWAVES * 2 * ORB_PATCH_BYTES);
  uint32_t *sslot = soff + ((S + 1 + 3) & ~3);
  uint32_t *kpl = sslot + ((S + 3) & ~3);
  uint32_t *kpos = kpl + per_max;
  for (int i = tid; i < S; i += 256) {
    const PlanStrip ps = plan_strip(P, i);
    sslot[i] = strip_slot_of(P, ps.li, ps.s) | (P.lv[ps.li].gn > 1 ? 0x80000000u : 0u);
  }

  const uint32_t *cnt = strip_count + (size_t)pyr * S;
  if (tid == 0) sh->carry = 0;
  __syncthreads();
  for (int base = 0; base < S; base += 256) {
    const int i = base + tid;
    const uint32_t v = i < S ? (cnt[i] & ~STRIP_DESCRIBED) : 0;
    uint32_t incl = v;
#pragma unroll
    for (int d = 1; d < 64; d <<= 1) {
      const uint32_t t = (uint32_t)__shfl_up((int)incl, d, 64);
      if (lane >= d) incl += t;
    }
    if (lane == 63) sh->wsum[wv] = incl;
    __syncthreads();
    uint32_t pre = sh->carry;
    for (int w = 0; w < wv; w++) pre += sh->wsum[w];
    if (i < S) soff[i] = pre + incl - v;
    __syncthreads();
    if (tid == 255) sh->carry = pre + incl;
    __syncthreads();
  }
  const uint32_t total = sh->carry;
  if (tid == 0) {
    soff[S] = total;
    if (ch == 0) counts[pyr] = total;
  }
  __syncthreads();
  const uint32_t per = (total + nch - 1) / nch;
  const uint32_t lo = min((uint32_t)ch * per, total), hi = min(lo + per, total);
  if (lo >= hi) return;

  const uint32_t *stage = stage_kp + (size_t)pyr * P.slots_per_pyr;
  const uint32_t *sd = stage_desc + (size_t)pyr * S * QS_SHARED * words;
  uint32_t *dsc = desc + (size_t)pyr * desc_stride;
  const uint8_t *im = pyramids + (size_t)pyr * pyr_stride;
  const uint32_t img_bytes32 = (uint32_t)((size_t)P.rows * P.vstep);
  const int vstep = P.vstep;
  lds_u8 *wave_patches = (lds_u8 *)(patches + (wv * 2) * ORB_PATCH_BYTES);
  const lds_u32 *kpl_l = (const lds_u32 *)kpl, *kpos_l = (const lds_u32 *)kpos;
  for (uint32_t c0 = lo; c0 < hi; c0 += per_max) {
    const uint32_t c1 = min(c0 + per_max, hi);
    if (tid == 0) sh->ntodo = 0;
    __syncthreads();
    for (uint32_t e = c0 + tid; e < c1; e += 256) {
      int a = 0, b = S;
      while (b - a > 1) {
        const int m = (a + b) >> 1;
        if (soff[m] <= e) a = m; else b = m;
      }
      const uint32_t k = e - soff[a];
      const uint32_t ss = sslot[a];
      const uint32_t v = stage[(ss & 0x7fffffffu) + k];
      uint32_t pos = e;
      if (ss >> 31) {
        const PlanStrip ps = plan_strip(P, a);
        pos = final_position(P, soff, stage, ps.li, ps.s, k, v);
      }
      if (pos >= cap) continue;
      kp[(size_t)pyr * kp_stride + pos] = v;
      if (cnt[a] & STRIP_DESCRIBED) {
        const uint32_t *src = sd + ((size_t)a * QS_SHARED + k) * words;
        for (int w = 0; w < words; w++) dsc[(size_t)pos * words + w] = src[w];
      } else {
        const uint32_t slot = atomicAdd(&sh->ntodo, 1u);
        kpl[slot] = v;
        kpos[slot] = pos;
      }
    }
    __syncthreads();
    const uint32_t nt = sh->ntodo;
    const int glevel = GHOOKS ? (P.ablate >> 20) & 15 : 0;
    if (nt != 0 && !(P.ablate & 64) && glevel != 1) {
      const uint32_t npairs = (nt + 1) >> 1;
      auto pair_of = [&](uint32_t it, uint32_t &p0, uint32_t &p1, uint32_t &q0, uint32_t &q1) {
        const bool h0 = it < npairs, h1 = it < npairs && 2 * it + 1 < nt;
        p0 = h0 ? kpl_l[2 * it] : 0u;
        q0 = h0 ? kpos_l[2 * it] : 0u;
        p1 = h1 ? kpl_l[2 * it + 1] : 0u;
        q1 = h1 ? kpos_l[2 * it + 1] : 0u;
      };
      uint32_t a0, a1, b0, b1, qa0, qa1, qb0, qb1;
      pair_of(wv, a0, a1, qa0, qa1);
      OrbWin wa = orb_fetch(G, a0, a1, im, vstep, img_bytes32), wb;
      for (uint32_t it = wv; it < npairs; it += 2 * OWAVES) {
        pair_of(it + OWAVES, b0, b1, qb0, qb1);
        wb = orb_fetch(G, b0, b1, im, vstep, img_bytes32);
        orb_describe<lds_u8, GHOOKS>(G, wa, a0, a1, wave_patches, vstep, rtab, words, (uint8_t *)dsc, (G.half ? qa1 : qa0) * (uint32_t)words, glevel);
        if (it + OWAVES >= npairs) break;
        pair_of(it + 2 * OWAVES, a0, a1, qa0, qa1);
        wa = orb_fetch(G, a0, a1, im, vstep, img_bytes32);
        orb_describe<lds_u8, GHOOKS>(G, wb, b0, b1, wave_patches, vstep, rtab, words, (uint8_t *)dsc, (G.half ? qb1 : qb0) * (uint32_t)words, glevel);
      }
    }
    __syncthreads();
  }
}

template <bool GHOOKS>
__global__ __launch_bounds__(256) __attribute__((amdgpu_waves_per_eu(6))) void k_gather_orb(
    const FusedParams P, const uint8_t *__restrict__ pyramids, size_t pyr_stride,
    const uint32_t *__restrict__ stage_kp, const uint32_t *__restrict__ strip_count,
    const uint32_t *__restrict__ stage_desc,
    uint32_t *__restrict__ kp, size_t kp_stride, uint32_t cap, uint32_t *__restrict__ counts,
    uint32_t *__restrict__ desc, size_t desc_stride, int words, uint32_t per_max, uint32_t *__restrict__ ovf_reset) {
  asm volatile("" ::: "v79");
  extern __shared__ __attribute__((aligned(16))) uint8_t osm[];
  if (ovf_reset && blockIdx.x == 0 && blockIdx.y == 0 && threadIdx.x == 0) {
    ovf_reset[1] = ovf_reset[0];
    ovf_reset[0] = 0;
  }
  orb_role<NoWait, GHOOKS>(P, pyramids, pyr_stride, stage_kp, strip_count, stage_desc, kp, kp_stride, cap, counts, desc, desc_stride,
                           words, per_max, osm, (int)blockIdx.y, (int)blockIdx.x, (int)gridDim.x);
}

constexpr int FRAME_SYNC_PYR = 8, FRAME_SYNC_DONE = 8, FRAME_SYNC_POISON = 9, FRAME_SYNC_WORDS = 12;
constexpr uint32_t COUNT_INVALID = 0xffffffffu;
__global__ __launch_bounds__(NT) void k_frame(const FusedParams P, const uint8_t *__restrict__ pyramids, size_t pyr_stride,
                                              uint32_t *__restrict__ stage_kp, uint32_t *__restrict__ strip_count,
                                              uint32_t *__restrict__ kp, size_t kp_stride, uint32_t cap,
                                              uint32_t *__restrict__ counts, uint32_t *__restrict__ desc, size_t desc_stride,
                                              int words, uint32_t per_max, int nch, uint32_t *__restrict__ sync,
                                              uint32_t *__restrict__ ovf, uint32_t *__restrict__ hflag, uint32_t test) {
  extern __shared__ __attribute__((aligned(16))) uint8_t smem[];
  __shared__ uint32_t sh_ctr[16];
  const int n_strip = P.batch * P.runs_per_pyr;
  if ((int)blockIdx.x < n_strip) {
    const int pyr = (int)blockIdx.x % P.batch, run = (int)blockIdx.x / P.batch;
    strips_role<true, false, true, false, false, true>(P, pyramids, pyr_stride, stage_kp, strip_count, nullptr, 0, nullptr, ovf,
                                                       nullptr, smem, sh_ctr, pyr, run);
    __syncthreads();
    if (threadIdx.x == 0 && !((test & 1u) && blockIdx.x == 0))
      (void)__hip_atomic_fetch_add(&sync[pyr], 1u, __ATOMIC_RELEASE, __HIP_MEMORY_SCOPE_AGENT);
    return;
  }
  const int ob = (int)blockIdx.x - n_strip, pyr = ob / nch, ch = ob - pyr * nch;
  __shared__ uint32_t sh_ok;
  auto wait = [&]() -> bool {
    if (threadIdx.x == 0) {
      uint32_t ok = 0;
      const bool poisoned = __hip_atomic_load(&sync[FRAME_SYNC_POISON], __ATOMIC_RELAXED, __HIP_MEMORY_SCOPE_AGENT) != 0;
      const int limit = poisoned ? 0 : 1 << (((test >> 8) & 31u) ? ((test >> 8) & 31u) : 20u);
      for (int it = 0; it < limit; it++) {
        if (__hip_atomic_load(&sync[pyr], __ATOMIC_RELAXED, __HIP_MEMORY_SCOPE_AGENT) >= (uint32_t)P.runs_per_pyr) {
          ok = 1;
          break;
        }
        __builtin_amdgcn_s_sleep(PISLAM_FRAME_SLEEP);
      }
      __builtin_amdgcn_fence(__ATOMIC_ACQUIRE, "agent");
      if (!ok) {
        __hip_atomic_store(&sync[FRAME_SYNC_POISON], 1u, __ATOMIC_RELAXED, __HIP_MEMORY_SCOPE_AGENT);
        __hip_atomic_store(hflag, 1u, __ATOMIC_RELAXED, __HIP_MEMORY_SCOPE_SYSTEM);
        if (ch == 0) counts[pyr] = COUNT_INVALID;
      }
      sh_ok = ok;
    }
    __syncthreads();
    return sh_ok != 0;
  };
  orb_role(P, pyramids, pyr_stride, stage_kp, strip_count, nullptr, kp, kp_stride, cap, counts, desc, desc_stride, words, per_max,
           smem, pyr, ch, nch, wait);
  __syncthreads();
  if (threadIdx.x == 0 && sh_ok != 0) {
    const uint32_t done = __hip_atomic_fetch_add(&sync[FRAME_SYNC_DONE], 1u, __ATOMIC_RELAXED, __HIP_MEMORY_SCOPE_AGENT);
    if (done + 1 == (uint32_t)(P.batch * nch)) {
      for (int i = 0; i <= FRAME_SYNC_DONE; i++) __hip_atomic_store(&sync[i], 0u, __ATOMIC_RELAXED, __HIP_MEMORY_SCOPE_AGENT);
      ovf[1] = __hip_atomic_load(&ovf[0], __ATOMIC_RELAXED, __HIP_MEMORY_SCOPE_AGENT);
      __hip_atomic_store(&ovf[0], 0u, __ATOMIC_RELAXED, __HIP_MEMORY_SCOPE_AGENT);
    }
  }
}

}
```

### pislam_amd/csrc/pislam_hip.hip

```cpp
#include <hip/hip_runtime.h>
#include <stdint.h>
#include <stdio.h>
#include <stdlib.h>
#include <string.h>

#include <algorithm>
#include <cmath>
#include <functional>
#include <string>
#include <type_traits>
#include <vector>

#include "../../include/pislam_hip.h"

__device__ const uint32_t g_brief_tab[30 * 256] = {
#include "brief_table.inc"
};
static constexpr uint32_t h_brief_tab_packed[30 * 256] = {
#include "brief_table.inc"
};
struct BriefOfsTab {
  uint32_t v[30 * 256];
};
#include "pislam_dev.h"
__device__ const pdev::VrecpeTab g_vrecpe_tab = pdev::make_vrecpe_tab();
__device__ const pdev::OrbMaskTab g_orb_masks = pdev::make_orb_mask_tab();
extern __device__ const BriefOfsTab g_brief_ofs;
#include "pislam_stage_kernels.h"
#include "pislam_fused_kernels.h"
static constexpr int brief_row_ofs(int r) { return pf::orb_row_ofs(r); }
static constexpr BriefOfsTab make_brief_ofs() {
  BriefOfsTab t{};
  for (int i = 0; i < 30 * 256; i++) {
    const uint32_t e = h_brief_tab_packed[i];
    const int dx0 = (int8_t)(e & 0xff), dy0 = (int8_t)((e >> 8) & 0xff);
    const int dx1 = (int8_t)((e >> 16) & 0xff), dy1 = (int8_t)(e >> 24);
    const int rot = i >> 8, k = i & 255;
    t.v[rot * 256 + 32 * (k & 7) + (k >> 3)] =
        (uint32_t)(brief_row_ofs(dy0 + 15) + dx0 + 15) | ((uint32_t)(brief_row_ofs(dy1 + 15) + dx1 + 15) << 16);
  }
  return t;
}
__device__ const BriefOfsTab g_brief_ofs = make_brief_ofs();

#include "pislam_prep_kernels.h"
#include "pislam_match_kernels.h"
#include "pislam_bow_kernels.h"
#include "pislam_bowdb_kernels.h"
#include "pislam_select_kernels.h"
#include "pislam_warp_kernels.h"

#define PISLAM_EXPORT extern "C" __attribute__((visibility("default")))

namespace {

struct DevBuf {
  void *p = nullptr;
  size_t cap = 0;
  unsigned long long reallocs = 0;
  int ensure(size_t bytes, bool *grew = nullptr) {
    if (grew) *grew = false;
    if (bytes <= cap) return PISLAM_OK;
    if (p) (void)hipFree(p);
    p = nullptr;
    cap = 0;
    size_t want = std::max<size_t>(bytes, 256);
    if (hipMalloc(&p, want) != hipSuccess) {
      (void)hipGetLastError();
      return PISLAM_ERR_NOMEM;
    }
    cap = want;
    reallocs++;
    if (grew) *grew = true;
    return PISLAM_OK;
  }
  void release() {
    if (p) (void)hipFree(p);
    p = nullptr;
    cap = 0;
    reallocs++;
  }
  template <class T>
  T *as() const { return (T *)p; }
};

}

struct pislam_dist_state;

struct pislam_ctx {
  int device = 0;
  hipStream_t stream = nullptr;
  hipStream_t own_stream = nullptr;
  pislam_dist_state *dist = nullptr;
  std::string err;
  DevBuf s_img, s_out, s_pts, s_desc, s_misc, s_rots, s_tmp;
  DevBuf w_cnt, w_off, w_total, w_cellkp;
  DevBuf w_score, w_stage, w_stripcnt, w_work, w_prof, w_ovf, w_stagedesc;
  DevBuf w_ustage, w_ucount;
  struct CellIndex {
    DevBuf off, meta, desc;
  };
  CellIndex w_win, w_sc, w_st;
  CellIndex w_bow;
  DevBuf w_db;
  struct PlanTable {
    std::vector<uint32_t> host;
    DevBuf dev;
  };
  std::vector<PlanTable *> plan_tables;
  const uint32_t *cur_utab = nullptr;
  DevBuf w_sync;
  uint32_t *frame_flag = nullptr;
  uint32_t *frame_flag_dev = nullptr;
  bool frame_disabled = false;
  unsigned long long frame_timeouts = 0;
  int opt_frame_test = 0;
  DevBuf w_chain;
  size_t chain_words = 0;
  bool chain_disabled = false;
  int opt_build_chain = 0;
  int num_cus = 0;
  int opt_pipeline = 0;
  int opt_dump_score = 0;
  int opt_strip_rows = 0;
  int opt_ablate = 0;
  int opt_bucket_round_up = 0;
  int opt_orb_chunks = 0;
  uint32_t last_strips = 0;
  int opt_repeat_strips = 1;
  int opt_alias = 1;
  int opt_run_len = 0;
  int lanes_in_flight = 1;
  int opt_lds_pad = 0;
  int opt_wgs_per_cu = 0;
  int opt_strip_px = 16384;
  int opt_strip_rows_max = 0;
  int opt_run_order = 1;
  int opt_tile_cols = 0;
  int opt_bucket_select = 1;
  int opt_frame = 1;
  int opt_orb_in_strip = 0;
  int opt_match_mfma = 1;
  int opt_warp_direct = 0;
  int opt_dist_rccl_single = 0;
  int last_pipeline = 0;
  unsigned last_path = 0;
  size_t score_bytes_valid = 0;
  pislam_frontend_params last_params{};
  std::vector<pislam_level> last_levels;
  int last_batch = 0;
  size_t last_stride = 0;
  hipEvent_t ev[4] = {nullptr, nullptr, nullptr, nullptr};
  bool timing_valid = false;
  static constexpr int MAX_SUB = 16;
  int opt_sub_batches = 1;
  int opt_sub_mb = 0;
  hipStream_t aux_stream = nullptr;
  hipEvent_t ev_sub[MAX_SUB] = {};
  hipEvent_t ev_join = nullptr;
  int ovf_nsub = 0;
  size_t ovf_stride = 0;
  unsigned long long ovf_layouts = 0;
  unsigned long long table_uploads = 0;
  unsigned long long workspace_generation() const {
    unsigned long long g = ovf_layouts + table_uploads + frame_timeouts;
    for (const DevBuf *b : {&w_cnt, &w_off, &w_total, &w_cellkp, &w_score, &w_stage, &w_stripcnt, &w_work, &w_prof,
                            &w_ovf, &w_stagedesc, &w_ustage, &w_ucount, &w_sync, &w_chain})
      g += b->reallocs;
    return g;
  }
};

namespace {

int fail(pislam_ctx *c, int code, const char *what, hipError_t e = hipSuccess) {
  if (c) {
    c->err = what;
    if (e != hipSuccess) {
      c->err += ": ";
      c->err += hipGetErrorString(e);
    }
  }
  (void)hipGetLastError();
  return code;
}

#define HIPCHK(c, call)                                                   \
  do {                                                                    \
    hipError_t e_ = (call);                                               \
    if (e_ != hipSuccess) return fail((c), PISLAM_ERR_HIP, #call, e_);    \
  } while (0)

#define PCHK(call)                     \
  do {                                 \
    int r_ = (call);                   \
    if (r_ != PISLAM_OK) return r_;    \
  } while (0)

bool is_device_ptr(const void *p) {
  if (!p) return false;
  hipPointerAttribute_t a;
  hipError_t e = hipPointerGetAttributes(&a, p);
  if (e != hipSuccess) {
    (void)hipGetLastError();
    return false;
  }
  return a.type == hipMemoryTypeDevice || a.type == hipMemoryTypeManaged;
}

struct Staged {
  const void *host = nullptr;
  void *dev = nullptr;
  size_t bytes = 0;
};

int stage_in(pislam_ctx *c, DevBuf &buf, const void *p, size_t bytes, Staged *s, bool copy = true) {
  s->bytes = bytes;
  if (bytes == 0 || is_device_ptr(p)) {
    s->host = nullptr;
    s->dev = (void *)p;
    return PISLAM_OK;
  }
  if (buf.ensure(bytes) != PISLAM_OK) return fail(c, PISLAM_ERR_NOMEM, "hipMalloc(staging)");
  s->host = p;
  s->dev = buf.p;
  if (copy) HIPCHK(c, hipMemcpyAsync(buf.p, p, bytes, hipMemcpyHostToDevice, c->stream));
  return PISLAM_OK;
}

int stage_out(pislam_ctx *c, const Staged &s, void *host_dst, size_t bytes) {
  if (!s.host || bytes == 0) return PISLAM_OK;
  HIPCHK(c, hipMemcpyAsync(host_dst, s.dev, bytes, hipMemcpyDeviceToHost, c->stream));
  return PISLAM_OK;
}

int sync(pislam_ctx *c) {
  HIPCHK(c, hipStreamSynchronize(c->stream));
  return PISLAM_OK;
}

int launch_ok(pislam_ctx *c, const char *what) {
  hipError_t e = hipGetLastError();
  if (e != hipSuccess) return fail(c, PISLAM_ERR_HIP, what, e);
  return PISLAM_OK;
}

inline int cdiv(int a, int b) { return (a + b - 1) / b; }

int ensure_fault_flag(pislam_ctx *c) {
  if (c->frame_flag) return PISLAM_OK;
  void *h = nullptr, *d = nullptr;
  if (hipHostMalloc(&h, 64, hipHostMallocMapped) != hipSuccess || hipHostGetDevicePointer(&d, h, 0) != hipSuccess) {
    (void)hipGetLastError();
    if (h) (void)hipHostFree(h);
    return fail(c, PISLAM_ERR_NOMEM, "hipHostMalloc(fault flag)");
  }
  c->frame_flag = (uint32_t *)h;
  c->frame_flag_dev = (uint32_t *)d;
  ((volatile uint32_t *)c->frame_flag)[0] = 0;
  ((volatile uint32_t *)c->frame_flag)[1] = 0;
  return PISLAM_OK;
}
int check_frame_poison(pislam_ctx *c) {
// ... 1003 lines not shown
    *F = tall;
    *lds_bytes = l0;
    *lds_alias_bytes = l1;
  }
  return true;
}

int choose_sub_batches(const pislam_ctx *c, const pislam_frontend_params *p, int batch) {
  if (c->opt_dump_score || c->opt_ablate || c->opt_pipeline == 1) return 1;
  int n = c->opt_sub_batches;
  if (n == 0) {
    const double mb = (double)p->rows * p->vstep * batch / (1024.0 * 1024.0);
    const double target = c->opt_sub_mb > 0 ? c->opt_sub_mb : 128.0;
    n = (int)(mb / target + 0.5);
    n = std::min(n, batch / 16);
  }
  return std::max(1, std::min(std::min(n, batch), (int)pislam_ctx::MAX_SUB));
}

int prepare_ovf(pislam_ctx *c, int nsub, size_t stride) {
  bool grew = false;
  if (c->w_ovf.ensure(sizeof(uint32_t) * stride * nsub, &grew) != PISLAM_OK)
    return fail(c, PISLAM_ERR_NOMEM, "hipMalloc(overflow list)");
  const size_t lay = nsub == 1 ? 0 : stride;
  if (grew || c->ovf_nsub != nsub || c->ovf_stride != lay) {
    HIPCHK(c, hipMemsetAsync(c->w_ovf.p, 0, c->w_ovf.cap, c->stream));
    c->ovf_nsub = nsub;
    c->ovf_stride = lay;
    c->ovf_layouts++;
  }
  return PISLAM_OK;
}

int ensure_aux(pislam_ctx *c, int nsub) {
  if (!c->aux_stream) HIPCHK(c, hipStreamCreateWithFlags(&c->aux_stream, hipStreamNonBlocking));
  if (!c->ev_join) HIPCHK(c, hipEventCreateWithFlags(&c->ev_join, hipEventDisableTiming));
  for (int i = 0; i < nsub; i++)
    if (!c->ev_sub[i]) HIPCHK(c, hipEventCreateWithFlags(&c->ev_sub[i], hipEventDisableTiming));
  return PISLAM_OK;
}

int build_select_plan(pislam_ctx *c, const pislam_frontend_params *p, const pf::FusedParams &Fplan, pf::SelectPlan *Qp,
                      pf::FusedParams *Up) {
  pf::SelectPlan &Q = *Qp;
  pf::FusedParams &U = *Up;
  memset(&Q, 0, sizeof(Q));
  memset(&U, 0, sizeof(U));
  const int lbs = p->log_bucket_size, bs = 1 << lbs, B = p->border;
  Q.lbs = lbs;
  Q.limit = p->bucket_limit;
  Q.border = B;
  int nreal = 0;
  for (int e = 0; e < Fplan.nlevels; e++) {
    if (Fplan.lv[e].gfirst != e) continue;
    if (nreal >= 16) return fail(c, PISLAM_ERR_INVALID, "too many levels for the bucket selection pass");
    const int l = nreal++;
    const int gn = std::max(1, Fplan.lv[e].gn);
    const pf::FusedLevel &last = Fplan.lv[e + gn - 1];
    const int wl = last.col0 + last.w - Fplan.lv[e].col0, hl = Fplan.lv[e].h;
    const int nx = wl - 2 * B, ny = hl - 2 * B;
    Q.row0[l] = Fplan.lv[e].row0;
    Q.col0[l] = Fplan.lv[e].col0;
    Q.h[l] = hl;
    Q.g0[l] = e;
    Q.gn[l] = gn;
    Q.unit0[l] = Q.units_per_pyr;
    Q.nunits[l] = (nx > 0 && ny > 0) ? cdiv(ny, bs) : 0;
    Q.cap[l] = (nx > 0 ? ((nx - 1) >> lbs) + 1 : 1) * p->bucket_limit;
    Q.uslot0[l] = Q.uslots_per_pyr;
    Q.nb_max = std::max(Q.nb_max, Q.cap[l] / p->bucket_limit);
    Q.units_per_pyr += Q.nunits[l];
    Q.uslots_per_pyr += Q.nunits[l] * Q.cap[l];
    pf::FusedLevel &ul = U.lv[l];
    ul.w = wl;
    ul.h = hl;
    ul.row0 = Q.row0[l];
    ul.col0 = Q.col0[l];
    ul.R = 2;
    ul.nbx = Q.cap[l];
    ul.nstrips = Q.nunits[l];
    ul.strip0 = Q.unit0[l];
    ul.slot0 = Q.uslot0[l];
    ul.gfirst = l;
    ul.gn = 1;
  }
  Q.nlevels = nreal;
  U.nlevels = nreal;
  U.strips_per_pyr = Q.units_per_pyr;
  U.slots_per_pyr = Q.uslots_per_pyr;
  U.vstep = p->vstep;
  U.rows = p->rows;
  U.border = B;
  U.lbs = lbs;
  U.limit = p->bucket_limit;
  U.words = p->words;
  U.ablate = Fplan.ablate;
  if (Q.units_per_pyr == 0) return fail(c, PISLAM_ERR_INVALID, "no extractable level");
  return PISLAM_OK;
}

int plan_table(pislam_ctx *c, const std::vector<uint32_t> &t, const uint32_t **out) {
  for (size_t i = 0; i < c->plan_tables.size(); i++)
    if (c->plan_tables[i]->host == t) {
      std::rotate(c->plan_tables.begin() + i, c->plan_tables.begin() + i + 1, c->plan_tables.end());
      *out = c->plan_tables.back()->dev.as<uint32_t>();
      return PISLAM_OK;
    }
  if (c->plan_tables.size() >= 64) {
    HIPCHK(c, hipStreamSynchronize(c->stream));
    c->plan_tables.front()->dev.release();
    delete c->plan_tables.front();
    c->plan_tables.erase(c->plan_tables.begin());
    c->table_uploads++;
  }
  pislam_ctx::PlanTable *pt = new pislam_ctx::PlanTable();
  pt->host = t;
  if (pt->dev.ensure(sizeof(uint32_t) * pt->host.size()) != PISLAM_OK) {
    delete pt;
    return fail(c, PISLAM_ERR_NOMEM, "hipMalloc(plan table)");
  }
  c->plan_tables.push_back(pt);
  HIPCHK(c, hipMemcpyAsync(pt->dev.p, pt->host.data(), sizeof(uint32_t) * pt->host.size(), hipMemcpyHostToDevice, c->stream));
  *out = pt->dev.as<uint32_t>();
  return PISLAM_OK;
}

std::vector<uint32_t> unit_table(const pislam_frontend_params *p, const pf::FusedParams &F, const pf::SelectPlan &Q) {
  std::vector<uint32_t> t((size_t)Q.units_per_pyr * pf::SEL_REC, 0u);
  const int B = p->border, lbs = p->log_bucket_size, bs = 1 << lbs;
  for (int l = 0; l < Q.nlevels; l++)
    for (int cr = 0; cr < Q.nunits[l]; cr++) {
      uint32_t *r = &t[(size_t)(Q.unit0[l] + cr) * pf::SEL_REC];
      const int y0 = B + (cr << lbs), y1 = std::min(y0 + bs, Q.h[l] - B);
      int nl = 0;
      for (int k = 0; k < Q.gn[l]; k++) {
        const pf::FusedLevel &E = F.lv[Q.g0[l] + k];
        const int s_lo = (y0 - B) / E.R, s_hi = std::min((y1 - 1 - B) / E.R, E.nstrips - 1);
        for (int sidx = s_lo; sidx <= s_hi; sidx++, nl++)
          if (nl < pf::SEL_ML) {
            r[8 + nl] = (uint32_t)(E.slot0 + sidx * (E.R >> 1) * E.nbx);
            r[16 + nl] = (uint32_t)(E.strip0 + sidx);
          }
      }
      r[0] = nl <= pf::SEL_ML ? (uint32_t)nl : 0xffffffffu;
      r[1] = (uint32_t)l;
      r[2] = (uint32_t)cr;
      r[3] = (uint32_t)(Q.uslot0[l] + cr * Q.cap[l]);
      r[4] = (uint32_t)(Q.row0[l] + B);
      r[5] = (uint32_t)(Q.col0[l] + B);
    }
  return t;
}

constexpr int FRAME_MAX_BATCH = 8;
constexpr int FRAME_DEFAULT_BATCH = 2;
inline int frame_max_batch(const pislam_ctx *c) { return c->opt_frame <= 0 ? 0 : c->opt_frame == 1 ? FRAME_DEFAULT_BATCH : std::min(c->opt_frame, FRAME_MAX_BATCH); }
static_assert(FRAME_MAX_BATCH <= pf::FRAME_SYNC_PYR, "k_frame's hand-over counters");
int ensure_frame_sync(pislam_ctx *c) {
  bool grew = false;
  if (c->w_sync.ensure(sizeof(uint32_t) * pf::FRAME_SYNC_WORDS, &grew) != PISLAM_OK)
    return fail(c, PISLAM_ERR_NOMEM, "hipMalloc(frame sync)");
  if (grew) HIPCHK(c, hipMemsetAsync(c->w_sync.p, 0, c->w_sync.cap, c->stream));
  return ensure_fault_flag(c);
}
struct FrontendPlan {
  bool fused = false;
  int nsub = 1, submax = 0;
  pf::FusedParams F{};
  size_t lds = 0, lds_alias = 0, klds = 0;
  bool sel = false;
  pf::SelectPlan Q{};
  pf::FusedParams U{};
  std::vector<uint32_t> utab;
  size_t sel_lds = 0, glds = 0;
  bool alias = false;
  size_t ovf_stride = 0, sdesc_per_pyr = 0;
  bool generic_orb = false;
  bool frame = false;
  int nch = 0, fch = 0;
  size_t per_max = 0, olds = 0, fper = 0, flds = 0;
};

int plan_frontend(pislam_ctx *c, const pislam_frontend_params *p, const pislam_level *lv, int batch, FrontendPlan *P) {
  P->nsub = choose_sub_batches(c, p, batch);
  P->submax = batch / P->nsub + (batch % P->nsub ? 1 : 0);
  P->fused = c->opt_pipeline != 1 && build_fused_plan(c, p, lv, P->submax, &P->F, &P->lds, &P->lds_alias);
  const pf::FusedParams &F = P->F;
  const int S = F.strips_per_pyr, nsub = P->nsub, submax = P->submax;
  if (!P->fused || S == 0) return PISLAM_OK;
  P->sel = p->log_bucket_size != 0 && F.lbs == 0;
  if (P->sel) {
    PCHK(build_select_plan(c, p, F, &P->Q, &P->U));
    P->utab = unit_table(p, F, P->Q);
    P->sel_lds = sizeof(uint32_t) * pf::SEL_WAVES * (64 + 2 * (size_t)P->Q.nb_max);
  }
  const int Sg = P->sel ? P->Q.units_per_pyr : S;
  P->sdesc_per_pyr = F.orb_in_strip ? (size_t)S * pf::QS_SHARED * (size_t)p->words : 0;
  P->alias = c->opt_alias && submax <= 65535 && S <= 65535;
  P->ovf_stride = 2 + (size_t)S * submax;
  P->klds = P->alias ? P->lds_alias : P->lds;
  P->generic_orb = p->vstep % 16 != 0 || (size_t)p->rows * p->vstep > 0x7fffffffu;
  P->glds = sizeof(uint32_t) * (Sg + 1);
  if (!P->generic_orb) {
    long px = 0;
    for (int l = 0; l < F.nlevels; l++) px += (long)(F.lv[l].ex1 - F.lv[l].ex0) * F.lv[l].nstrips * F.lv[l].R;
    const int by_px = (int)(px / 70000);
    int nch = std::min(64, submax >= 128 ? std::max(8, by_px) : std::max(by_px, std::max(16, 4096 / submax)));
    if (nsub == 1) {
      const long slots = 7L * std::max(1, c->num_cus);
      long best = nch, bestd = 1L << 40;
      for (long m = 1; m <= 64; m++) {
        const long cand = m * slots / submax;
        if (cand < 4 || cand > 64) continue;
        const long d = std::labs(cand - nch);
        if (d < bestd) {
          bestd = d;
          best = cand;
        }
      }
      nch = (int)best;
    } else {
      nch = std::min(64, std::max(8, by_px));
    }
    P->nch = c->opt_orb_chunks > 0 ? c->opt_orb_chunks : nch;
    P->per_max = ((size_t)p->max_keypoints + P->nch - 1) / P->nch;
    P->olds = pf::orb_lds_bytes(Sg, P->per_max);
  }
  if (P->alias && !P->sel && F.lbs == 0 && !F.dump_score && !F.ablate && !P->generic_orb && nsub == 1 && !F.orb_in_strip &&
      c->opt_repeat_strips <= 1 && batch <= frame_max_batch(c)) {
    P->fch = c->opt_orb_chunks > 0 ? std::min(c->opt_orb_chunks, 128) : std::min(64, std::max(16, 128 / batch));
    P->fper = ((size_t)p->max_keypoints + P->fch - 1) / P->fch;
    P->flds = std::max(std::max(P->lds_alias, P->lds), pf::orb_lds_bytes(S, P->fper));
    const long wg_per_cu = std::max<long>(1, std::min<long>(5, CU_LDS / (long)std::max<size_t>(P->flds, 1)));
    const long slots_per_xcd = wg_per_cu * std::max(1, c->num_cus / 8);
    const long waiting_per_xcd = ((long)std::max(1, c->lanes_in_flight) * batch * P->fch + 7) / 8;
    P->frame = P->flds <= LDS_CAP && 4 * waiting_per_xcd <= slots_per_xcd;
  }
  return PISLAM_OK;
}

const char *strip_plan_violation(const FrontendPlan &P, const pislam_frontend_params *p) {
  const pf::FusedParams &F = P.F;
  if (F.nlevels < 1 || F.nlevels > pf::MAX_LEVELS) return "entries";
  int strips = 0, slots = 0, runs = 0;
  for (int l = 0; l < F.nlevels; l++) {
    const pf::FusedLevel &L = F.lv[l];
    if (L.strip0 != strips || L.slot0 != slots || L.run0 != runs) return "prefix sums";
    if (L.nstrips < 0 || (L.nstrips > 0 && (L.R < 2 || (L.R & 1)))) return "strip height";
    if (L.nstrips > 0) {
      if (L.col0 < 0 || L.row0 < 0 || L.col0 + L.w > p->vstep || L.row0 + L.h > p->rows) return "entry outside the pyramid";
      if (L.tpitch % 16 || L.pitch % 16 || L.tpitch <= 0) return "pitch";
      if ((L.R + 10) * L.tpitch > (int)LDS_CAP) return "tile larger than the LDS";
      if (L.gfirst < 0 || L.gfirst > l || L.gn < 1 || L.gfirst + L.gn > F.nlevels) return "tile group";
      if (L.ex0 < p->border || L.ex1 > L.w || L.ex0 > L.ex1) return "owned columns";
      if (cdiv(L.nstrips, F.run_len) != L.nruns) return "runs";
      if ((uint64_t)L.vpr_recip * (uint64_t)(L.tpitch / 16) < (1ull << 32)) return "vpr_recip";
      if ((uint64_t)L.tp_recip * (uint64_t)L.tpitch < (1ull << 32)) return "tp_recip";
      if (L.qh < pf::QH_SHARED) return "corner queue";
    }
    strips += L.nstrips;
    slots += L.nstrips * (L.R / 2) * L.nbx;
    runs += L.nruns;
  }
  if (strips != F.strips_per_pyr || slots != F.slots_per_pyr || runs != F.runs_per_pyr) return "totals";
  if (F.order_n) {
    if (F.order_n != runs || runs > pf::MAX_ORDER) return "order size";
    std::vector<int> seen((size_t)runs, 0);
    for (int i = 0; i < F.order_n; i++) {
      const int e = (int)(F.order[i] >> 16), r = (int)(F.order[i] & 0xffff);
      if (e >= F.nlevels || r >= F.lv[e].nruns) return "order entry";
      seen[(size_t)(F.lv[e].run0 + r)]++;
    }
    for (int v : seen)
      if (v != 1) return "order is not a permutation of the runs";
  }
  if (P.lds_alias > (size_t)CU_LDS) return "aliased LDS size";
  return nullptr;
}

const char *select_plan_violation(const FrontendPlan &P, const pislam_frontend_params *p) {
  const pf::SelectPlan &Q = P.Q;
  int units = 0, uslots = 0;
  for (int l = 0; l < Q.nlevels; l++) {
    if (Q.unit0[l] != units || Q.uslot0[l] != uslots) return "selection plan prefix sums";
    if (Q.g0[l] < 0 || Q.g0[l] + Q.gn[l] > P.F.nlevels) return "selection plan entries";
    if (Q.cap[l] / p->bucket_limit > pf::SEL_NB) return "more buckets than the selection pass holds";
    units += Q.nunits[l];
    uslots += Q.nunits[l] * Q.cap[l];
  }
  if (units != Q.units_per_pyr || uslots != Q.uslots_per_pyr) return "selection plan totals";
  return nullptr;
}

int reserve_frontend(pislam_ctx *c, const pislam_frontend_params *p, const pislam_level *lv, const FrontendPlan &P, int batch) {
  const size_t pyr_bytes = (size_t)p->rows * p->vstep;
  bool grew = false;
  if (c->w_score.ensure(pyr_bytes * batch, &grew) != PISLAM_OK)
    return fail(c, PISLAM_ERR_NOMEM, "hipMalloc(score map)");
  const bool same_shape = !grew && c->last_batch >= batch && c->last_params.vstep == p->vstep &&
                          c->last_params.rows == p->rows && c->last_params.nlevels == p->nlevels &&
                          c->last_params.border == p->border && (int)c->last_levels.size() == p->nlevels &&
                          memcmp(c->last_levels.data(), lv, sizeof(pislam_level) * p->nlevels) == 0;
  if (!same_shape) {
    HIPCHK(c, hipMemsetAsync(c->w_score.p, 0, pyr_bytes * batch, c->stream));
    c->last_params = *p;
    c->last_levels.assign(lv, lv + p->nlevels);
    c->last_batch = batch;
  }
  size_t maxn = 1;
  for (int l = 0; l < p->nlevels; l++) {
    const int ny = lv[l].height - 2 * p->border, nx = lv[l].width - 2 * p->border;
    if (ny <= 0 || nx <= 0) continue;
    const int bs = 1 << p->log_bucket_size;
    maxn = std::max<size_t>(maxn, p->log_bucket_size == 0 ? (size_t)cdiv(ny, 2) : (size_t)((nx - 1) / bs + 1) * ((ny - 1) / bs + 1));
  }
  if (c->w_cnt.ensure(sizeof(uint32_t) * maxn * batch) != PISLAM_OK ||
      c->w_off.ensure(sizeof(uint32_t) * maxn * batch) != PISLAM_OK ||
      (p->log_bucket_size &&
       c->w_cellkp.ensure(sizeof(uint32_t) * maxn * batch * p->bucket_limit) != PISLAM_OK))
    return fail(c, PISLAM_ERR_NOMEM, "hipMalloc(extract scratch)");
  if (!P.fused || P.F.strips_per_pyr == 0) return PISLAM_OK;
  if (c->w_stage.ensure(sizeof(uint32_t) * ((size_t)P.F.slots_per_pyr * batch + 64)) != PISLAM_OK ||
      c->w_stripcnt.ensure(sizeof(uint32_t) * (size_t)P.F.strips_per_pyr * batch) != PISLAM_OK ||
      c->w_stagedesc.ensure(sizeof(uint32_t) * P.sdesc_per_pyr * batch) != PISLAM_OK)
    return fail(c, PISLAM_ERR_NOMEM, "hipMalloc(fused staging)");
  if (P.alias) PCHK(prepare_ovf(c, P.nsub, P.ovf_stride));
  if (P.nsub > 1) PCHK(ensure_aux(c, P.nsub));
  if (batch <= frame_max_batch(c)) PCHK(ensure_frame_sync(c));
  if (P.sel) {
    if (c->w_ustage.ensure(sizeof(uint32_t) * (size_t)P.Q.uslots_per_pyr * batch) != PISLAM_OK ||
        c->w_ucount.ensure(sizeof(uint32_t) * (size_t)P.Q.units_per_pyr * batch) != PISLAM_OK)
      return fail(c, PISLAM_ERR_NOMEM, "hipMalloc(bucket selection staging)");
    PCHK(plan_table(c, P.utab, &c->cur_utab));
  }
  return PISLAM_OK;
}

#define RAISE_LDS_LIMIT(c, kern, bytes)                                                                                \
  do {                                                                                                                 \
    if ((bytes) > LDS_OPT_IN)                                                                                          \
      HIPCHK(c, hipFuncSetAttribute((const void *)kern, hipFuncAttributeMaxDynamicSharedMemorySize, (int)bytes));      \
  } while (0)

using StripKernT = void (*)(const pf::FusedParams, const uint8_t *, size_t, uint32_t *, uint32_t *, uint8_t *, size_t,
                            unsigned long long *, uint32_t *, uint32_t *);
using OvfKernT = void (*)(const pf::FusedParams, const uint8_t *, size_t, uint32_t *, uint32_t *, uint8_t *, size_t, const uint32_t *);

StripKernT strip_kernel(bool vec, bool alias, bool hooks, bool orb_in_strip, int lbs) {
  static const StripKernT kerns[8] = {
      pf::k_fused_strips<false, false, false>, pf::k_fused_strips<false, false, true>,
      pf::k_fused_strips<false, true, false>,  pf::k_fused_strips<false, true, true>,
      pf::k_fused_strips<true, false, false>,  pf::k_fused_strips<true, false, true>,
      pf::k_fused_strips<true, true, false>,   pf::k_fused_strips<true, true, true>};
  static const StripKernT kerns_orb[2] = {pf::k_fused_strips<true, false, true, true>, pf::k_fused_strips<true, true, true, true>};
  static const StripKernT kerns_nb[2] = {pf::k_fused_strips<true, false, true, false, false>,
                                         pf::k_fused_strips<true, true, true, false, false>};
  return (orb_in_strip && vec && alias) ? kerns_orb[hooks ? 1 : 0]
         : (vec && alias && lbs == 0)   ? kerns_nb[hooks ? 1 : 0]
                                        : kerns[(vec ? 4 : 0) | (hooks ? 2 : 0) | (alias ? 1 : 0)];
}
OvfKernT overflow_kernel(bool vec, bool hooks) {
  static const OvfKernT okerns[4] = {pf::k_fused_overflow<false, false>, pf::k_fused_overflow<false, true>,
                                     pf::k_fused_overflow<true, false>, pf::k_fused_overflow<true, true>};
  return okerns[(vec ? 2 : 0) | (hooks ? 1 : 0)];
}
auto gather_orb_kernel(int ablate) { return (ablate >> 20) & 15 ? pf::k_gather_orb<true> : pf::k_gather_orb<false>; }

int launch_orb_batch(pislam_ctx *c, hipStream_t stream, const pislam_frontend_params *p, const uint8_t *pyramids, size_t stride,
                     int n, const uint32_t *kp, const uint32_t *counts, uint32_t *desc) {
  hipLaunchKernelGGL(pk::k_orb<0>, dim3(cdiv(p->max_keypoints, 4), 1, n), dim3(256), 0, stream, pyramids, p->vstep, stride, kp,
                     (size_t)p->max_keypoints, counts, 0u, (uint32_t)p->max_keypoints, p->words, desc,
                     (size_t)p->max_keypoints * p->words, (int32_t *)nullptr, (const uint8_t *)nullptr);
  return launch_ok(c, "k_orb<batch>");
}

int report_strip_profile(pislam_ctx *c, const unsigned long long *prof, size_t prof_n, hipStream_t M, double ns, unsigned workgroups) {
  std::vector<unsigned long long> hv(prof_n);
  HIPCHK(c, hipMemcpyAsync(hv.data(), prof, prof_n * sizeof(unsigned long long), hipMemcpyDeviceToHost, M));
  HIPCHK(c, hipStreamSynchronize(M));
  double h[8] = {0};
  unsigned long long why[3] = {0, 0, 0};
  for (size_t i = 0; i < prof_n; i++) {
    if ((i & 7) == 5) {
      why[0] += hv[i] & 0xfffff;
      why[1] += (hv[i] >> 20) & 0xfffff;
      why[2] += hv[i] >> 40;
    } else {
      h[i & 7] += (double)hv[i];
    }
  }
  fprintf(stderr, "[pislam prof] deferred strips by reason: corner queue %llu, score queue %llu, survivor buffer %llu\n",
          why[0], why[1], why[2]);
  fprintf(stderr, "[pislam prof] cycles/strip: stage %.0f classify %.0f harris %.0f nms %.0f emit %.0f "
                  "(strips %.0f, carried %.0f, workgroups %u, lifetime %.0f/strip)\n",
          h[0] / ns, h[1] / ns, h[2] / ns, h[3] / ns, h[4] / ns, ns, h[6], workgroups, h[7] / ns);
  return PISLAM_OK;
}

struct FusedCall {
  const pislam_frontend_params *p;
  const FrontendPlan &P;
  const uint8_t *pyramids;
  size_t stride;
  int batch;
  uint32_t *kp, *desc, *counts;
  StripKernT kern;
  OvfKernT okern;
  decltype(gather_orb_kernel(0)) gkern;
  bool fork;
  hipStream_t M, X;
};

int launch_frame(pislam_ctx *c, const FusedCall &k) {
  const pislam_frontend_params *p = k.p;
  const FrontendPlan &P = k.P;
  RAISE_LDS_LIMIT(c, pf::k_frame, P.flds);
  pf::FusedParams F = P.F;
  F.batch = k.batch;
  const unsigned grid = (unsigned)(k.batch * F.runs_per_pyr + k.batch * P.fch);
  hipLaunchKernelGGL(pf::k_frame, dim3(grid), dim3(pf::NT), P.flds, c->stream, F, k.pyramids, k.stride, c->w_stage.as<uint32_t>(),
                     c->w_stripcnt.as<uint32_t>(), k.kp, (size_t)p->max_keypoints, (uint32_t)p->max_keypoints, k.counts, k.desc,
                     (size_t)p->max_keypoints * p->words, p->words, (uint32_t)P.fper, P.fch, c->w_sync.as<uint32_t>(),
                     c->w_ovf.as<uint32_t>(), c->frame_flag_dev, (uint32_t)c->opt_frame_test);
  PCHK(launch_ok(c, "k_frame"));
  c->last_path = PISLAM_PATH_FUSED | PISLAM_PATH_ONE_LAUNCH;
  HIPCHK(c, hipEventRecord(c->ev[1], c->stream));
  HIPCHK(c, hipEventRecord(c->ev[2], c->stream));
  return PISLAM_OK;
}

int launch_sub_batch(pislam_ctx *c, const FusedCall &k, int sub) {
  const pislam_frontend_params *p = k.p;
  const FrontendPlan &P = k.P;
  const int S = P.F.strips_per_pyr, nsub = P.nsub, base = k.batch / nsub, rem = k.batch % nsub;
  const int first = sub * base + std::min(sub, rem), n = base + (sub < rem ? 1 : 0);
  const hipStream_t M = k.M, X = k.X;
  pf::FusedParams F = P.F;
  F.batch = n;
  const size_t dump_stride = (size_t)p->rows * p->vstep;
  const uint8_t *s_pyr = k.pyramids + (size_t)first * k.stride;
  uint32_t *s_stage = c->w_stage.as<uint32_t>() + (size_t)first * F.slots_per_pyr;
  uint32_t *s_cnt = c->w_stripcnt.as<uint32_t>() + (size_t)first * S;
  uint32_t *s_sdesc = c->w_stagedesc.as<uint32_t>() + (size_t)first * P.sdesc_per_pyr;
  uint8_t *s_dump = F.dump_score ? c->w_score.as<uint8_t>() + (size_t)first * dump_stride : nullptr;
  uint32_t *s_kp = k.kp + (size_t)first * p->max_keypoints;
  uint32_t *s_desc = k.desc + (size_t)first * p->max_keypoints * p->words;
  uint32_t *s_counts = k.counts + first;
  uint32_t *ovf = P.alias ? c->w_ovf.as<uint32_t>() + (size_t)sub * P.ovf_stride : nullptr;
  const dim3 grid((unsigned)(cdiv(n, 8) * F.runs_per_pyr * 8));
  unsigned long long *prof = nullptr;
  const size_t prof_n = (size_t)grid.x * 8;
  if (F.ablate & 8192) {
    if (c->w_prof.ensure(prof_n * sizeof(unsigned long long)) != PISLAM_OK) return fail(c, PISLAM_ERR_NOMEM, "hipMalloc(prof)");
    prof = c->w_prof.as<unsigned long long>();
    HIPCHK(c, hipMemsetAsync(prof, 0, prof_n * sizeof(unsigned long long), M));
  }
  for (int rep = 0; rep < std::max(1, c->opt_repeat_strips); rep++) {
    if (rep && ovf) HIPCHK(c, hipMemsetAsync(ovf, 0, sizeof(uint32_t), M));
    hipLaunchKernelGGL(k.kern, grid, dim3(pf::NT), P.klds, M, F, s_pyr, k.stride, s_stage, s_cnt, s_dump, dump_stride, prof, ovf,
                       s_sdesc);
  }
  if (prof) PCHK(report_strip_profile(c, prof, prof_n, M, (double)S * n, grid.x));
  PCHK(launch_ok(c, "k_fused_strips"));
  if (nsub > 1) {
    if (k.fork) {
      HIPCHK(c, hipEventRecord(c->ev_sub[sub], M));
      HIPCHK(c, hipStreamWaitEvent(X, c->ev_sub[sub], 0));
    }
    if (sub == nsub - 1) {
      HIPCHK(c, hipEventRecord(c->ev[1], M));
      HIPCHK(c, hipEventRecord(c->ev[2], M));
    }
  } else {
    HIPCHK(c, hipEventRecord(c->ev[1], M));
  }
  if (P.alias) {
    hipLaunchKernelGGL(k.okern, dim3((unsigned)std::max(8, c->num_cus / 2)), dim3(pf::NT), P.lds, X, F, s_pyr, k.stride, s_stage,
                       s_cnt, s_dump, dump_stride, (const uint32_t *)ovf);
    PCHK(launch_ok(c, "k_fused_overflow"));
  }
  if (nsub == 1) HIPCHK(c, hipEventRecord(c->ev[2], M));
  pf::FusedParams G = F;
  const uint32_t *g_stage = s_stage, *g_cnt = s_cnt;
  if (P.sel) {
    uint32_t *u_stage = c->w_ustage.as<uint32_t>() + (size_t)first * P.Q.uslots_per_pyr;
    uint32_t *u_cnt = c->w_ucount.as<uint32_t>() + (size_t)first * P.Q.units_per_pyr;
    hipLaunchKernelGGL(pf::k_bucket_select, dim3(cdiv(P.Q.units_per_pyr, pf::SEL_WAVES), n), dim3(64 * pf::SEL_WAVES), P.sel_lds, X, F, P.Q,
                       (const uint32_t *)s_stage, (const uint32_t *)s_cnt, u_stage, u_cnt, c->cur_utab);
    PCHK(launch_ok(c, "k_bucket_select"));
    G = P.U;
    G.batch = n;
    g_stage = u_stage;
    g_cnt = u_cnt;
  }
  if (P.generic_orb) {
    c->last_path |= PISLAM_PATH_GENERIC_ORB;
    hipLaunchKernelGGL(pf::k_gather, dim3(n), dim3(256), P.glds, X, G, g_stage, g_cnt, s_kp,
                       (size_t)p->max_keypoints, (uint32_t)p->max_keypoints, s_counts, ovf);
    PCHK(launch_ok(c, "k_gather"));
    return launch_orb_batch(c, X, p, s_pyr, k.stride, n, s_kp, s_counts, s_desc);
  }
  hipLaunchKernelGGL(k.gkern, dim3(P.nch, n), dim3(256), P.olds, X, G, s_pyr, k.stride, g_stage, g_cnt,
                     (const uint32_t *)s_sdesc, s_kp, (size_t)p->max_keypoints, (uint32_t)p->max_keypoints, s_counts,
                     s_desc, (size_t)p->max_keypoints * p->words, p->words, (uint32_t)P.per_max, ovf);
  return launch_ok(c, "k_gather_orb");
}

int run_fused(pislam_ctx *c, const pislam_frontend_params *p, const FrontendPlan &P, const uint8_t *pyramids, size_t stride,
              int batch, uint32_t *kp, uint32_t *desc, uint32_t *counts) {
  const int nsub = P.nsub;
  c->last_path = PISLAM_PATH_FUSED | (P.sel ? PISLAM_PATH_BUCKET_SELECT : 0u) | (P.F.lbs != 0 ? PISLAM_PATH_BUCKETS_IN_STRIPS : 0u);
  bool vec = ((uintptr_t)pyramids % 16 == 0) && (stride % 16 == 0) && (p->vstep % 16 == 0);
  for (int l = 0; l < P.F.nlevels; l++) vec = vec && (P.F.lv[l].col0 % 16 == 0);
  if (P.alias) c->last_strips = (uint32_t)P.F.strips_per_pyr * (uint32_t)batch;
  hipStreamCaptureStatus capture = hipStreamCaptureStatusNone;
  if (nsub > 1 && hipStreamIsCapturing(c->stream, &capture) != hipSuccess) {
    (void)hipGetLastError();
    capture = hipStreamCaptureStatusNone;
  }
  const bool fork = nsub > 1 && capture == hipStreamCaptureStatusNone;
  const bool hooks = P.F.dump_score || P.F.ablate;
  const StripKernT kern = strip_kernel(vec, P.alias, hooks, P.F.orb_in_strip, P.F.lbs);
  if (P.klds > LDS_CAP) return fail(c, PISLAM_ERR_INVALID, "level too wide for the strip kernel's LDS tiles");
  RAISE_LDS_LIMIT(c, kern, P.klds);
  const OvfKernT okern = overflow_kernel(vec, hooks);
  if (P.alias) RAISE_LDS_LIMIT(c, okern, P.lds);
  const auto gkern = gather_orb_kernel(P.F.ablate);
  if (!P.generic_orb) {
    if (P.olds > LDS_CAP) return fail(c, PISLAM_ERR_INVALID, "max_keypoints too large for the fused ORB kernel");
    RAISE_LDS_LIMIT(c, gkern, P.olds);
  }
  const FusedCall k{p, P, pyramids, stride, batch, kp, desc, counts, kern, okern, gkern, fork, c->stream, fork ? c->aux_stream : c->stream};
  if (c->frame_disabled) c->last_path |= PISLAM_PATH_FRAME_TIMED_OUT;
  if (P.frame && vec && !c->frame_disabled) return launch_frame(c, k);
  for (int sub = 0; sub < nsub; sub++) PCHK(launch_sub_batch(c, k, sub));
  if (fork) {
    HIPCHK(c, hipEventRecord(c->ev_join, k.X));
    HIPCHK(c, hipStreamWaitEvent(k.M, c->ev_join, 0));
  }
  return PISLAM_OK;
}

int run_staged(pislam_ctx *c, const pislam_frontend_params *p, const pislam_level *lv, const uint8_t *pyramids, size_t stride,
               int batch, uint32_t *kp, uint32_t *desc, uint32_t *counts) {
  const size_t pyr_bytes = (size_t)p->rows * p->vstep;
  uint8_t *score = c->w_score.as<uint8_t>();
  HIPCHK(c, hipMemsetAsync(counts, 0, sizeof(uint32_t) * batch, c->stream));
  const bool same = stride == pyr_bytes;
  for (int l = 0; l < p->nlevels; l++) {
    const size_t off = (size_t)lv[l].row0 * p->vstep + lv[l].col0;
    if (same) {
      PCHK(launch_detect(c, pyramids + off, score + off, p->vstep, pyr_bytes, batch, p->border,
                         lv[l].width, lv[l].height, p->fast_threshold));
      PCHK(launch_harris(c, pyramids + off, score + off, p->vstep, pyr_bytes, batch, p->border,
                         lv[l].width, lv[l].height, p->harris_threshold));
    } else {
      for (int b = 0; b < batch; b++) {
        PCHK(launch_detect(c, pyramids + b * stride + off, score + b * pyr_bytes + off, p->vstep, 0, 1,
                           p->border, lv[l].width, lv[l].height, p->fast_threshold));
        PCHK(launch_harris(c, pyramids + b * stride + off, score + b * pyr_bytes + off, p->vstep, 0, 1,
                           p->border, lv[l].width, lv[l].height, p->harris_threshold));
      }
    }
  }
  HIPCHK(c, hipEventRecord(c->ev[1], c->stream));
  for (int l = 0; l < p->nlevels; l++) {
    const size_t off = (size_t)lv[l].row0 * p->vstep + lv[l].col0;
    const uint32_t add_xy = ((uint32_t)lv[l].col0 << 12) | (uint32_t)lv[l].row0;
    PCHK(launch_extract(c, score + off, p->vstep, pyr_bytes, batch, p->border, p->log_bucket_size,
                        p->bucket_limit, lv[l].width, lv[l].height, kp, (size_t)p->max_keypoints,
                        (uint32_t)p->max_keypoints, add_xy, counts));
  }
  HIPCHK(c, hipEventRecord(c->ev[2], c->stream));
  return launch_orb_batch(c, c->stream, p, pyramids, stride, batch, kp, counts, desc);
}

}

PISLAM_EXPORT int pislam_debug_build_plan(const pislam_frontend_params *p, const pislam_level *lv, int batch, int num_cus,
                                          int lanes_in_flight, const char *options, uint32_t summary[8], char *err, size_t err_cap) {
  pislam_ctx c;
  auto say = [&](int rc) {
    if (err && err_cap) snprintf(err, err_cap, "%s", c.err.c_str());
    return rc;
  };
  auto bad = [&](const char *what) {
    c.err = std::string("plan invariant violated: ") + what;
    return say(PISLAM_ERR_HIP);
  };
  c.num_cus = num_cus > 0 ? num_cus : 256;
  c.lanes_in_flight = lanes_in_flight > 0 ? lanes_in_flight : 1;
  if (!summary) return PISLAM_ERR_INVALID;
  memset(summary, 0, sizeof(uint32_t) * 8);
  for (const char *q = options; q && *q;) {
    const char *e = strchr(q, ','), *eq = strchr(q, '=');
    const size_t len = e ? (size_t)(e - q) : strlen(q);
    if (!eq || (size_t)(eq - q) >= len) {
      c.err = "options: key=value[,key=value...]";
      return say(PISLAM_ERR_INVALID);
    }
    const std::string key(q, eq - q);
    if (key == "own_stream") {
      c.err = "own_stream needs a device";
      return say(PISLAM_ERR_INVALID);
    }
    const int rc = pislam_ctx_set_option(&c, key.c_str(), atoi(eq + 1));
    if (rc != PISLAM_OK) return say(rc);
    q += len + (e ? 1 : 0);
  }
  const int rc = check_params(&c, p, lv, batch);
  if (rc != PISLAM_OK) return say(rc);
  FrontendPlan P;
  const int plan_rc = plan_frontend(&c, p, lv, batch, &P);
  if (!P.fused) {
    c.err = "no strip plan for these parameters (the staged pipeline takes the call)";
    return say(PISLAM_ERR_INVALID);
  }
  if (const char *what = strip_plan_violation(P, p)) return bad(what);
  const uint32_t strip_summary[7] = {(uint32_t)P.F.nlevels,       (uint32_t)P.F.strips_per_pyr, (uint32_t)P.F.runs_per_pyr,
                                     (uint32_t)P.F.slots_per_pyr, (uint32_t)P.F.run_len,        (uint32_t)P.lds,
                                     (uint32_t)P.lds_alias};
  memcpy(summary, strip_summary, sizeof(strip_summary));
  if (plan_rc != PISLAM_OK) return say(plan_rc);
  if (P.sel) {
    if (const char *what = select_plan_violation(P, p)) return bad(what);
    summary[7] = (uint32_t)P.Q.units_per_pyr;
  }
  return PISLAM_OK;
}

PISLAM_EXPORT int pislam_frontend_reserve(pislam_ctx *c, const pislam_frontend_params *p,
                                          const pislam_level *lv, int batch) {
  PCHK(check_params(c, p, lv, batch));
  HIPCHK(c, hipSetDevice(c->device));
  FrontendPlan P;
  PCHK(plan_frontend(c, p, lv, batch, &P));
  return reserve_frontend(c, p, lv, P, batch);
}

PISLAM_EXPORT int pislam_orb_frontend_batch(pislam_ctx *c, const pislam_frontend_params *p,
                                            const pislam_level *lv, const uint8_t *pyramids,
                                            size_t stride, int batch, uint32_t *kp, uint32_t *desc,
                                            uint32_t *counts) {
  PCHK(check_params(c, p, lv, batch));
  HIPCHK(c, hipSetDevice(c->device));
  PCHK(check_frame_poison(c));
  if (!pyramids || !kp || !desc || !counts) return fail(c, PISLAM_ERR_INVALID, "null pointer");
  if (stride < (size_t)p->rows * p->vstep) return fail(c, PISLAM_ERR_INVALID, "pyramid_stride too small");
  if (!is_device_ptr(pyramids) || !is_device_ptr(kp) || !is_device_ptr(desc) || !is_device_ptr(counts))
    return fail(c, PISLAM_ERR_INVALID, "the batch path takes device pointers only");
  FrontendPlan P;
  PCHK(plan_frontend(c, p, lv, batch, &P));
  if (c->opt_pipeline >= 2 && !P.fused)
    return fail(c, PISLAM_ERR_INVALID, "fused pipeline unavailable for these parameters (bucket size / LDS size)");
  PCHK(reserve_frontend(c, p, lv, P, batch));
  c->last_stride = (size_t)p->rows * p->vstep;
  c->last_pipeline = P.fused ? 2 : 1;
  c->last_path = P.fused ? PISLAM_PATH_FUSED : PISLAM_PATH_STAGED;
  HIPCHK(c, hipEventRecord(c->ev[0], c->stream));
  if (P.fused && P.F.strips_per_pyr == 0) {
    HIPCHK(c, hipMemsetAsync(counts, 0, sizeof(uint32_t) * batch, c->stream));
    for (int i = 1; i < 4; i++) HIPCHK(c, hipEventRecord(c->ev[i], c->stream));
    c->timing_valid = true;
    c->last_strips = 0;
    return PISLAM_OK;
  }
  PCHK(P.fused ? run_fused(c, p, P, pyramids, stride, batch, kp, desc, counts)
               : run_staged(c, p, lv, pyramids, stride, batch, kp, desc, counts));
  HIPCHK(c, hipEventRecord(c->ev[3], c->stream));
  c->timing_valid = true;
  return PISLAM_OK;
}

PISLAM_EXPORT int pislam_frontend_get_score_map(pislam_ctx *c, int b, uint8_t *dst) {
  if (!c || !dst) return PISLAM_ERR_INVALID;
  if (b < 0 || b >= c->last_batch || !c->w_score.p || !c->last_stride)
    return fail(c, PISLAM_ERR_INVALID, "no score map for that pyramid");
  if (c->last_pipeline == 2 && !c->opt_dump_score)
    return fail(c, PISLAM_ERR_INVALID, "the fused pipeline keeps the score map in LDS (set option dump_score)");
  HIPCHK(c, hipSetDevice(c->device));
  const size_t bytes = c->last_stride;
  HIPCHK(c, hipMemcpyAsync(dst, c->w_score.as<uint8_t>() + (size_t)b * bytes, bytes, hipMemcpyDefault,
                           c->stream));
  return sync(c);
}

PISLAM_EXPORT int pislam_frontend_last_stats(pislam_ctx *c, uint32_t stats[2]) {
  if (!c || !stats) return PISLAM_ERR_INVALID;
  stats[0] = stats[1] = 0;
  if (!c->w_ovf.p || !c->last_strips) return PISLAM_OK;
  HIPCHK(c, hipSetDevice(c->device));
  PCHK(sync(c));
  PCHK(check_frame_poison(c));
  uint32_t prev[pislam_ctx::MAX_SUB] = {};
  for (int i = 0; i < c->ovf_nsub; i++)
    HIPCHK(c, hipMemcpyAsync(&prev[i], c->w_ovf.as<uint32_t>() + (size_t)i * c->ovf_stride + 1, sizeof(uint32_t),
                             hipMemcpyDeviceToHost, c->stream));
  PCHK(sync(c));
  for (int i = 0; i < c->ovf_nsub; i++) stats[0] += prev[i];
  stats[1] = c->last_strips;
  return PISLAM_OK;
}

PISLAM_EXPORT unsigned pislam_frontend_last_path(const pislam_ctx *c) { return c ? c->last_path : 0u; }

PISLAM_EXPORT int pislam_frontend_last_timing(pislam_ctx *c, float *total_ms, float stage_ms[3]) {
  if (!c) return PISLAM_ERR_INVALID;
  if (!c->timing_valid) return fail(c, PISLAM_ERR_INVALID, "no batch call recorded");
  HIPCHK(c, hipEventSynchronize(c->ev[3]));
  if (total_ms) HIPCHK(c, hipEventElapsedTime(total_ms, c->ev[0], c->ev[3]));
  if (stage_ms)
    for (int i = 0; i < 3; i++) HIPCHK(c, hipEventElapsedTime(&stage_ms[i], c->ev[i], c->ev[i + 1]));
  return PISLAM_OK;
}

namespace {
__global__ void k_shader_clock(unsigned long long ticks_100mhz, unsigned long long *out) {
  const unsigned long long w0 = wall_clock64(), c0 = (unsigned long long)clock64();
  unsigned long long w1 = w0;
  while (w1 - w0 < ticks_100mhz) w1 = wall_clock64();
  const unsigned long long c1 = (unsigned long long)clock64();
  if (threadIdx.x == 0) {
    out[0] = c1 - c0;
    out[1] = w1 - w0;
  }
}
}

PISLAM_EXPORT int pislam_debug_shader_clock(pislam_ctx *c, int micros, double *ghz) {
  if (!c || !ghz) return PISLAM_ERR_INVALID;
  if (micros < 1 || micros > 100000) return fail(c, PISLAM_ERR_INVALID, "micros must be 1..100000");
  HIPCHK(c, hipSetDevice(c->device));
  if (c->w_total.ensure(2 * sizeof(unsigned long long)) != PISLAM_OK) return fail(c, PISLAM_ERR_NOMEM, "hipMalloc");
  hipLaunchKernelGGL(k_shader_clock, dim3(1), dim3(64), 0, c->stream, (unsigned long long)micros * 100ull,
                     c->w_total.as<unsigned long long>());
  PCHK(launch_ok(c, "k_shader_clock"));
  unsigned long long r[2] = {0, 0};
  HIPCHK(c, hipMemcpyAsync(r, c->w_total.p, sizeof(r), hipMemcpyDeviceToHost, c->stream));
  PCHK(sync(c));
  *ghz = r[1] ? (double)r[0] / (double)r[1] * 0.1 : 0.0;
  return PISLAM_OK;
}


namespace {

int check_words(pislam_ctx *c, int words) {
  if (words != 1 && words != 2 && words != 4 && words != 8) return fail(c, PISLAM_ERR_INVALID, "words must be 1, 2, 4 or 8");
  return PISLAM_OK;
}
int check_batch(pislam_ctx *c, int batch) {
  if (batch < 0 || batch > 65535) return fail(c, PISLAM_ERR_INVALID, "batch must be 0..65535");
  return PISLAM_OK;
}
int check_train_stride(pislam_ctx *c, size_t t_stride, const char *what) {
  if (t_stride > 65535) return fail(c, PISLAM_ERR_INVALID, what);
  return PISLAM_OK;
}

template <class F>
void with_words(int words, F &&f) {
  switch (words) {
    case 1: f(std::integral_constant<int, 1>{}); break;
    case 2: f(std::integral_constant<int, 2>{}); break;
    case 4: f(std::integral_constant<int, 4>{}); break;
    default: f(std::integral_constant<int, 8>{}); break;
  }
}

template <class F>
void with_sad_radius(int sad_radius, F &&f) {
  switch (sad_radius) {
    case 1: f(std::integral_constant<int, 1>{}); break;
    case 2: f(std::integral_constant<int, 2>{}); break;
    case 3: f(std::integral_constant<int, 3>{}); break;
    case 4: f(std::integral_constant<int, 4>{}); break;
    case 5: f(std::integral_constant<int, 5>{}); break;
    case 6: f(std::integral_constant<int, 6>{}); break;
    default: f(std::integral_constant<int, 7>{}); break;
  }
// ... 1157 lines not shown
```

Baseline: 1.231 billion.

## Precompute per-strip plan records on host and load them as scalar tables

Per-strip geometry (source offsets, vector counts, tail/prefetch flags, prefilter run bounds, output slot and coordinate offset) is now computed once on the host into a 64-byte record per strip. The records are uploaded with the plan, and the strip, overflow and gather kernels read them through scalar loads instead of recomputing rows, bounds and slots per strip. The aim is to remove scalar/vector integer arithmetic and branch logic from the strip kernels. In exchange each strip does an extra scalar memory load, and a host-side validator plus a debug API are added to check that the table tiles each level correctly.

```diff
diff --git a/include/pislam_hip.h b/include/pislam_hip.h
--- a/include/pislam_hip.h
+++ b/include/pislam_hip.h
@@ -131,6 +131,10 @@
 
 int pislam_debug_build_plan(const pislam_frontend_params *params, const pislam_level *levels, int batch, int num_cus,
                             int lanes_in_flight, const char *options, uint32_t summary[8], char *err, size_t err_cap);
+
+int pislam_debug_build_plan_table(const pislam_frontend_params *params, const pislam_level *levels, int batch, int num_cus,
+                                  int lanes_in_flight, const char *options, uint32_t summary[8], uint32_t *table,
+                                  size_t table_cap, size_t *table_n, char *err, size_t err_cap);
 
 typedef struct pislam_pipeline pislam_pipeline;
 int pislam_pipeline_create(int device, int depth, pislam_pipeline **pipe);
diff --git a/pislam_amd/capi.py b/pislam_amd/capi.py
--- a/pislam_amd/capi.py
+++ b/pislam_amd/capi.py
@@ -74,6 +74,8 @@
     "pislam_frontend_last_path": (ctypes.c_uint, [_vp]),
     "pislam_debug_build_plan": (_i, [ctypes.POINTER(FrontendParams), ctypes.POINTER(Level), _i, _i, _i, ctypes.c_char_p,
                                      ctypes.POINTER(ctypes.c_uint32 * 8), ctypes.c_char_p, _sz]),
+    "pislam_debug_build_plan_table": (_i, [ctypes.POINTER(FrontendParams), ctypes.POINTER(Level), _i, _i, _i, ctypes.c_char_p,
+                                           ctypes.POINTER(ctypes.c_uint32 * 8), _vp, _sz, ctypes.POINTER(_sz), ctypes.c_char_p, _sz]),
     "pislam_pipeline_create": (_i, [_i, _i, ctypes.POINTER(_vp)]),
     "pislam_pipeline_destroy": (_i, [_vp]),
     "pislam_pipeline_depth": (_i, [_vp]),
diff --git a/pislam_amd/csrc/pislam_fused_kernels.h b/pislam_amd/csrc/pislam_fused_kernels.h
--- a/pislam_amd/csrc/pislam_fused_kernels.h
+++ b/pislam_amd/csrc/pislam_fused_kernels.h
@@ -76,6 +76,37 @@
   FusedLevel lv[MAX_LEVELS];
   uint32_t order[MAX_ORDER];
 };
+
+struct StripStage {
+  uint32_t rows;
+  uint32_t flags;
+  uint32_t src;
+  int nvec, nvec_c;
+  uint32_t src_n;
+  int nvec_n;
+  uint32_t pad;
+};
+struct StripRun {
+  int lin_lo, lin_n;
+  int lin_lo_c, lin_n_c;
+};
+struct StripOut {
+  int ys, own_rows;
+  uint32_t slot;
+  uint32_t add_xy;
+};
+struct alignas(64) StripRec {
+  StripStage st;
+  StripRun run;
+  StripOut out;
+};
+static_assert(sizeof(StripRec) == 64, "one 16-dword scalar load per strip");
+constexpr int REC_DW = sizeof(StripRec) / 4;
+constexpr uint32_t STRIP_RLO1 = 1;
+constexpr uint32_t STRIP_TAIL = 2;
+constexpr uint32_t STRIP_PF = 4;
+__host__ __device__ constexpr size_t plan_tab_gather(int S) { return (size_t)REC_DW * S; }
+__host__ __device__ constexpr size_t plan_tab_units(int S) { return (size_t)(REC_DW + 2) * S; }
 
 __device__ __forceinline__ void lds_barrier() {
   __builtin_amdgcn_fence(__ATOMIC_RELEASE, "workgroup", "local");
@@ -301,10 +332,9 @@
 };
 
 template <bool VEC16, bool HOOKS, bool ALIAS, bool ORBK, bool BUCK>
-__device__ __forceinline__ void strip_body(const StripArgs A, const FusedLevel L, const int pyr, const int s,
-                                           const int ys, const int ye, lds_u8 *tile0, lds_u8 *sc, lds_u32 *queues,
+__device__ __forceinline__ void strip_body(const StripArgs A, const FusedLevel L, const int pyr, const uint32_t sid,
+                                           const StripRec *__restrict__ recs, lds_u8 *tile0, lds_u8 *sc, lds_u32 *queues,
                                            lds_u32 *shq, uint32_t *sh_ctr, uint32_t *sh_ctr_prev, bool &deferred,
-                                           const uint8_t *__restrict__ im, const ptrdiff_t lim,
                                            uint32_t *__restrict__ stage_kp,
                                            uint32_t *__restrict__ strip_count, uint8_t *__restrict__ score_dump,
                                            size_t score_stride, const bool carry, const int tid,
@@ -314,6 +344,14 @@
                                            uint32_t *__restrict__ stage_desc, const uint8_t *__restrict__ imb,
                                            const uint32_t img_bytes32) {
   const int B = A.border;
+  typedef __attribute__((address_space(4))) const StripRec crec;
+  auto rec = [&]() {
+    uint32_t i = sid;
+    asm volatile("" : "+s"(i));
+    return (crec *)(recs + i);
+  };
+  const auto *qs = &rec()->st;
+  const StripStage St{qs->rows, qs->flags, qs->src, qs->nvec, qs->nvec_c, qs->src_n, qs->nvec_n, 0u};
   const int Albs = BUCK ? A.lbs : 0;
   constexpr bool ORB = ALIAS && VEC16 && ORBK;
   const int pitch = L.pitch, tpitch = L.tpitch;
@@ -386,7 +424,7 @@
   const int thr = A.thr;
   const int32_t hthr = A.hthr;
   const int ablate = HOOKS ? A.ablate : 0;
-  const int Lw = L.w, Lxend = L.xend, Lh = L.h;
+  const int Lw = L.w, Lxend = L.xend;
   const bool wmod = (Lw & 15) != 0;
 
   auto push_nonzero = [&](bool nz, uint32_t e) {
@@ -457,8 +495,6 @@
     }
   };
 
-  const int r_lo = carry ? 3 : (ys - 1 < B) ? 1 : 0;
-  const int r_hi = min(ye + 2, Lh - B) - (ys - 1);
   const uint32_t nkb4 = ~((uint32_t)min(128 + ((thr + 1) >> 1), 255) * 0x01010101u);
   const uint32_t nkd4 = ~((uint32_t)(129 - ((thr + 2) >> 1)) * 0x01010101u);
   const bool aligned4 = ((B | Lxend) & 3) == 0;
@@ -546,26 +582,25 @@
   };
 
   int h_begin = 0;
+  const auto *qr = carry ? &rec()->run.lin_lo_c : &rec()->run.lin_lo;
+  const int lin_lo = qr[0], lin_n = qr[1];
   {
     {
-      const int y_lo = ys - 4;
-      const int nrows = min(ye + 6, Lh) - y_lo;
       const int r_st0 = carry_img ? 10 : 0;
+      const uint32_t src_ofs = St.src + (carry_img ? 10u * (uint32_t)A.vstep : 0u);
       if (carry_img && (ablate & 2048)) {
       } else if (VEC16 && carry_img && pf_have) {
-        const int nvec = (nrows - 10) * (tpitch >> 4);
+        const int nvec = St.nvec_c;
         lds_u4 *dstv = (lds_u4 *)(tile0 + 10 * tpitch) + tid;
 #pragma unroll
         for (int k = 0; k < PF_MAX; k++)
           if (tid + NT * k < nvec) dstv[NT * k] = pf[k];
       } else if (VEC16) {
-        const int vpr = tpitch >> 4;
-        const int nvec = (nrows - r_st0) * vpr;
+        const int nvec = carry_img ? St.nvec_c : St.nvec;
         const int gap = A.vstep - tpitch;
-        const uint8_t *src0 = im + (uint32_t)((y_lo + r_st0) * A.vstep + xbase);
+        const uint8_t *src0 = imb + src_ofs;
         lds_u4 *dstv = (lds_u4 *)(tile0 + r_st0 * tpitch);
-        const bool tail = (uint32_t)((y_lo + nrows - 1) * A.vstep + xbase + tpitch) > (uint32_t)lim;
-        if (!tail) {
+        if (!(St.flags & STRIP_TAIL)) {
           constexpr int ST_MAX = 6;
           for (int i0 = tid; i0 < nvec; i0 += NT * ST_MAX) {
             u32x4 st[ST_MAX];
@@ -584,15 +619,16 @@
         } else {
           for (int i = tid; i < nvec; i += NT) {
             const int row = (int)__umulhi((uint32_t)i, L.vpr_recip);
-            const ptrdiff_t off = (ptrdiff_t)(y_lo + r_st0) * A.vstep + xbase + (ptrdiff_t)16 * i + (ptrdiff_t)row * gap;
+            const ptrdiff_t lim = (ptrdiff_t)img_bytes32;
+            const ptrdiff_t off = (ptrdiff_t)src_ofs + (ptrdiff_t)16 * i + (ptrdiff_t)row * gap;
             u32x4 d;
             if (off + 16 <= lim) {
-              d = *(const u32x4 *)(im + off);
+              d = *(const u32x4 *)(imb + off);
             } else {
               uint32_t w0 = 0, w1 = 0, w2 = 0, w3 = 0;
 #pragma unroll
               for (int k = 0; k < 16; k++) {
-                const uint32_t b = off + k < lim ? (uint32_t)im[off + k] << (8 * (k & 3)) : 0u;
+                const uint32_t b = off + k < lim ? (uint32_t)imb[off + k] << (8 * (k & 3)) : 0u;
                 if (k < 4) w0 |= b; else if (k < 8) w1 |= b; else if (k < 12) w2 |= b; else w3 |= b;
               }
               d = (u32x4){w0, w1, w2, w3};
@@ -601,10 +637,11 @@
           }
         }
       } else {
+        const int nrows = (int)(St.rows & 0xffffu);
         for (int i = r_st0 * tpitch + tid; i < nrows * tpitch; i += NT) {
           const int r = i / tpitch, cx = i - r * tpitch;
-          const ptrdiff_t off = (ptrdiff_t)(y_lo + r) * A.vstep + xbase + cx;
-          tile0[r * tpitch + cx] = off < lim ? im[off] : (uint8_t)0;
+          const ptrdiff_t off = (ptrdiff_t)St.src + (ptrdiff_t)r * A.vstep + cx;
+          tile0[r * tpitch + cx] = off < (ptrdiff_t)img_bytes32 ? imb[off] : (uint8_t)0;
         }
       }
     }
@@ -612,24 +649,18 @@
     mark(0);
     if (ALIAS) h_begin = (int)sh_ctr[2];
     pf_issued = false;
-    if (VEC16 && pf_want && L.R >= 10 && L.R * (tpitch >> 4) <= PF_MAX * NT) {
-      const int vpr = tpitch >> 4;
-      const int ylo_n = ye - 4, ye_n = min(ye + L.R, Lh - B);
-      const int nrows_n = min(ye_n + 6, Lh) - ylo_n;
-      if ((uint32_t)((ylo_n + nrows_n - 1) * A.vstep + xbase + tpitch) <= (uint32_t)lim) {
-        const int nvec_n = (nrows_n - 10) * vpr, gap = A.vstep - tpitch;
-        const uint8_t *src_n = im + (uint32_t)((ylo_n + 10) * A.vstep + xbase);
-#pragma unroll
-        for (int k = 0; k < PF_MAX; k++) {
-          const int i = tid + NT * k;
-          if (i < nvec_n) pf[k] = *(const u32x4 *)(src_n + (uint32_t)(16 * i + (int)__umulhi((uint32_t)i, L.vpr_recip) * gap));
-        }
-        pf_issued = true;
-      }
+    if (VEC16 && pf_want && (St.flags & STRIP_PF)) {
+      const int nvec_n = St.nvec_n, gap = A.vstep - tpitch;
+      const uint8_t *src_n = imb + St.src_n;
+#pragma unroll
+      for (int k = 0; k < PF_MAX; k++) {
+        const int i = tid + NT * k;
+        if (i < nvec_n) pf[k] = *(const u32x4 *)(src_n + (uint32_t)(16 * i + (int)__umulhi((uint32_t)i, L.vpr_recip) * gap));
+      }
+      pf_issued = true;
     }
     if (ablate & 1) return;
 
-    const int lin_lo = r_lo * tpitch, lin_n = max(r_hi - r_lo, 0) * tpitch;
     const int nfull = lin_n >> 8, rem = lin_n & 255;
     const uint32_t thr1x2 = (uint32_t)(thr + 1) * 0x10001u;
     auto prefilter_step = [&](const lds_u8 *pm, const lds_u8 *pu, const lds_u8 *pd, bool lane_ok) {
@@ -681,6 +712,9 @@
     lds_barrier();
     mark(2);
   }
+  const auto *qo = &rec()->out;
+  const StripOut Ro{qo->ys, qo->own_rows, qo->slot, qo->add_xy};
+  const int ys = Ro.ys, ye = ys + Ro.own_rows;
   tile = tile0;
   if ((ablate & 512) && tid == 0) sh_ctr[3] = 1;
   if (ablate & 512) lds_barrier();
@@ -724,7 +758,7 @@
     lds_u32 *shq_k = shq_s + QS_SHARED;
     const int tn = (int)sh_ctr[ALIAS ? 0 : 2];
     const lds_u32 *nq = ALIAS ? shq_h : shq_n;
-    const int own_rows = ye - ys;
+    const int own_rows = Ro.own_rows;
     const int ex0q = L.ex0, ex1q = L.ex1;
     for (int c0 = wave * 64; c0 < tn; c0 += WAVES * 64) {
       const uint32_t e = nq[min(c0 + lane, tn - 1)];
@@ -773,8 +807,8 @@
     if (sh_ctr[3] == 0) {
       if (ablate & 128) return;
       const int ns = (int)sh_ctr[4];
-      const size_t strip_slot = (size_t)pyr * A.slots_per_pyr + L.slot0 + (size_t)s * (L.R >> 1) * L.nbx;
-      const uint32_t add_xy = ((uint32_t)L.col0 << 12) | (uint32_t)L.row0;
+      const size_t strip_slot = (size_t)pyr * A.slots_per_pyr + Ro.slot;
+      const uint32_t add_xy = Ro.add_xy;
       const bool orb = ORB && A.orb != 0;
       auto describe_strip = [&](const int n, const uint32_t my_rank) {
         lds_u8 *patches = (lds_u8 *)queues + NMS_SCRATCH * 4;
@@ -785,7 +819,7 @@
         lds_barrier();
         const OrbLane G = orb_lane(lane, A.vstep);
         lds_u8 *wave_patches = patches + wave * 2 * ORB_PATCH_BYTES;
-        uint32_t *dbase = stage_desc + ((size_t)pyr * A.strips_per_pyr + L.strip0 + s) * (size_t)(QS_SHARED * A.words);
+        uint32_t *dbase = stage_desc + ((size_t)pyr * A.strips_per_pyr + sid) * (size_t)(QS_SHARED * A.words);
         for (int it = wave; 2 * it < n; it += WAVES) {
           const int i0 = 2 * it, i1 = min(i0 + 1, n - 1);
           const uint32_t r0 = shq_k[i0], r1 = i0 + 1 < n ? shq_k[i1] : 0xffffffffu;
@@ -824,7 +858,7 @@
           }
         }
         if (tid == 0)
-          strip_count[(size_t)pyr * A.strips_per_pyr + L.strip0 + s] = (uint32_t)ns | (orb ? STRIP_DESCRIBED : 0u);
+          strip_count[(size_t)pyr * A.strips_per_pyr + sid] = (uint32_t)ns | (orb ? STRIP_DESCRIBED : 0u);
         mark(4);
         if (orb && ns > 0) describe_strip(ns, my_rank);
         return;
@@ -862,7 +896,7 @@
           }
           kept = (uint32_t)__popcll(km);
         }
-        if (tid == 0) strip_count[(size_t)pyr * A.strips_per_pyr + L.strip0 + s] = kept | (orb ? STRIP_DESCRIBED : 0u);
+        if (tid == 0) strip_count[(size_t)pyr * A.strips_per_pyr + sid] = kept | (orb ? STRIP_DESCRIBED : 0u);
         mark(4);
         if (orb && ns > 0) describe_strip(ns, my_rank);
         return;
@@ -895,7 +929,7 @@
       }
       if (kept_here) atomicAdd(&sh_ctr[5], (uint32_t)kept_here);
       lds_barrier();
-      if (tid == 0) strip_count[(size_t)pyr * A.strips_per_pyr + L.strip0 + s] = sh_ctr[5] | (orb ? STRIP_DESCRIBED : 0u);
+      if (tid == 0) strip_count[(size_t)pyr * A.strips_per_pyr + sid] = sh_ctr[5] | (orb ? STRIP_DESCRIBED : 0u);
       if (orb && ns > 0) describe_strip(ns, my_rank);
       return;
     }
@@ -939,8 +973,8 @@
       if (lane == 0) cellcnt[cell] = (uint32_t)nf_c;
     }
     lds_barrier();
-    const size_t strip_slot = (size_t)pyr * A.slots_per_pyr + L.slot0 + (size_t)s * (L.R >> 1) * L.nbx;
-    const uint32_t add_xy = ((uint32_t)L.col0 << 12) | (uint32_t)L.row0;
+    const size_t strip_slot = (size_t)pyr * A.slots_per_pyr + Ro.slot;
+    const uint32_t add_xy = Ro.add_xy;
     for (int cell = wave; cell < ncell; cell += WAVES) {
       const uint32_t n = cellcnt[cell];
       if (n == 0) continue;
@@ -953,7 +987,7 @@
       uint32_t tot = 0;
       for (int k = lane; k < ncell; k += 64) tot += cellcnt[k];
       tot = (uint32_t)wave_sum((int)tot);
-      if (lane == 0) strip_count[(size_t)pyr * A.strips_per_pyr + L.strip0 + s] = tot;
+      if (lane == 0) strip_count[(size_t)pyr * A.strips_per_pyr + sid] = tot;
     }
     return;
   }
@@ -1010,8 +1044,8 @@
   }
   lds_barrier();
   if (ablate & 128) return;
-  const size_t strip_slot = (size_t)pyr * A.slots_per_pyr + L.slot0 + (size_t)s * (L.R >> 1) * nbx;
-  const uint32_t add_xy = ((uint32_t)L.col0 << 12) | (uint32_t)L.row0;
+  const size_t strip_slot = (size_t)pyr * A.slots_per_pyr + Ro.slot;
+  const uint32_t add_xy = Ro.add_xy;
   for (int br = wave; br < nbr; br += WAVES) {
     const uint32_t n = rowcnt[br];
     if (n == 0) continue;
@@ -1022,7 +1056,7 @@
   if (tid == 0) {
     uint32_t tot = 0;
     for (int k = 0; k < nbr; k++) tot += rowcnt[k];
-    strip_count[(size_t)pyr * A.strips_per_pyr + L.strip0 + s] = tot;
+    strip_count[(size_t)pyr * A.strips_per_pyr + sid] = tot;
   }
   }
 }
@@ -1053,8 +1087,8 @@
                                             uint32_t *__restrict__ stage_kp, uint32_t *__restrict__ strip_count,
                                             uint8_t *__restrict__ score_dump, size_t score_stride,
                                             unsigned long long *__restrict__ prof, uint32_t *__restrict__ ovf,
-                                            uint32_t *__restrict__ stage_desc, uint8_t *smem, uint32_t *sh_ctr, const int pyr,
-                                            int run) {
+                                            uint32_t *__restrict__ stage_desc, const StripRec *__restrict__ recs, uint8_t *smem,
+                                            uint32_t *sh_ctr, const int pyr, int run) {
   int li = 0;
   if (P.order_n > 0) {
     const uint32_t o = P.order[run];
@@ -1065,6 +1099,7 @@
     run -= P.lv[li].run0;
   }
   const int s0 = run * P.run_len, s1 = min(s0 + P.run_len, P.lv[li].nstrips);
+  const int sid0 = P.lv[li].strip0;
   long long t_wg = 0;
   if (HOOKS && prof) {
     prof += (size_t)blockIdx.x * 8;
@@ -1080,22 +1115,21 @@
     asm volatile("" : "+s"(li_o));
     asm volatile("" : "+v"(tid_o));
     const FusedLevel L = P.lv[li_o];
+    const uint32_t sid = (uint32_t)(sid0 + s);
     const StripLds m = strip_lds<ALIAS>(smem, L);
-    const uint8_t *im = pyramids + (size_t)pyr * pyr_stride + (size_t)L.row0 * P.vstep + L.col0;
-    const ptrdiff_t lim = (ptrdiff_t)P.rows * P.vstep - ((ptrdiff_t)L.row0 * P.vstep + L.col0);
     StripArgs A{P.border, P.thr, P.ablate, P.dump_score, P.lbs, P.limit, P.vstep, P.slots_per_pyr,
                 P.strips_per_pyr, P.hthr, P.words, P.orb_in_strip};
     asm volatile("" : "+s"(A.border), "+s"(A.thr), "+s"(A.lbs), "+s"(A.limit), "+s"(A.vstep), "+s"(A.slots_per_pyr),
                  "+s"(A.strips_per_pyr), "+s"(A.hthr), "+s"(A.words), "+s"(A.orb));
-    const int ys = A.border + s * L.R;
-    const int ye = min(ys + L.R, L.h - A.border);
+    int rows_o = P.rows, pyr_b = pyr;
+    asm volatile("" : "+s"(rows_o), "+s"(pyr_b));
     constexpr bool OVL = PISLAM_OVL && ALIAS && !BUCK && !ORBK;
     uint32_t *ctr = sh_ctr + (OVL ? 8 * (s & 1) : 0), *ctr_prev = sh_ctr + (OVL ? 8 * ((s & 1) ^ 1) : 0);
     bool deferred = false;
-    strip_body<VEC16, HOOKS, ALIAS, ORBK, BUCK>(A, L, pyr, s, ys, ye, m.tile, m.sc, m.queues, m.shq, ctr, ctr_prev, deferred, im, lim,
+    strip_body<VEC16, HOOKS, ALIAS, ORBK, BUCK>(A, L, pyr, sid, recs, m.tile, m.sc, m.queues, m.shq, ctr, ctr_prev, deferred,
                                     stage_kp, strip_count, score_dump, score_stride, carry, tid_o, prof, pf, pf_have, s + 1 < s1,
-                                    pf_have, ovf, INLINE_OVF ? 0xffffffffu : ((uint32_t)pyr << 16) | (uint32_t)(L.strip0 + s), stage_desc,
-                                    pyramids + (size_t)pyr * pyr_stride, (uint32_t)((size_t)P.rows * P.vstep));
+                                    pf_have, ovf, INLINE_OVF ? 0xffffffffu : ((uint32_t)pyr << 16) | sid, stage_desc,
+                                    pyramids + (size_t)pyr_b * pyr_stride, (uint32_t)rows_o * (uint32_t)A.vstep);
     if (INLINE_OVF && ALIAS && deferred) redo |= 1ull << (s - s0);
     if (s + 1 < s1) {
       if (OVL && !(HOOKS && (P.ablate & 0xfbf))) {
@@ -1121,15 +1155,14 @@
       asm volatile("" : "+s"(li_o));
       asm volatile("" : "+v"(tid_o));
       const FusedLevel L = P.lv[li_o];
+      const uint32_t sid = (uint32_t)(sid0 + s);
       const StripLds m2 = strip_lds<false>(smem, L);
-      const uint8_t *im = pyramids + (size_t)pyr * pyr_stride + (size_t)L.row0 * P.vstep + L.col0;
-      const ptrdiff_t lim = (ptrdiff_t)P.rows * P.vstep - ((ptrdiff_t)L.row0 * P.vstep + L.col0);
       const StripArgs A{P.border, P.thr, 0, 0, P.lbs, P.limit, P.vstep, P.slots_per_pyr, P.strips_per_pyr, P.hthr, P.words, 0};
-      const int ys = A.border + s * L.R, ye = min(ys + L.R, L.h - A.border);
       bool d2 = false, issued = false;
-      strip_body<VEC16, false, false, false, true>(A, L, pyr, s, ys, ye, m2.tile, m2.sc, m2.queues, m2.shq, sh_ctr, sh_ctr, d2, im, lim,
+      strip_body<VEC16, false, false, false, true>(A, L, pyr, sid, recs, m2.tile, m2.sc, m2.queues, m2.shq, sh_ctr, sh_ctr, d2,
                                                    stage_kp, strip_count, nullptr, 0, false, tid_o, nullptr, pf, false, false, issued,
-                                                   nullptr, 0u, nullptr, nullptr, 0u);
+                                                   nullptr, 0u, nullptr, pyramids + (size_t)pyr * pyr_stride,
+                                                   (uint32_t)((size_t)P.rows * P.vstep));
     }
   }
 }
@@ -1139,7 +1172,7 @@
     const FusedParams P, const uint8_t *__restrict__ pyramids, size_t pyr_stride,
     uint32_t *__restrict__ stage_kp, uint32_t *__restrict__ strip_count,
     uint8_t *__restrict__ score_dump, size_t score_stride, unsigned long long *__restrict__ prof,
-    uint32_t *__restrict__ ovf, uint32_t *__restrict__ stage_desc) {
+    uint32_t *__restrict__ ovf, uint32_t *__restrict__ stage_desc, const uint32_t *__restrict__ ptab) {
   extern __shared__ __attribute__((aligned(16))) uint8_t smem[];
   __shared__ uint32_t sh_ctr[16];
   const int xcd = blockIdx.x & 7, slot = blockIdx.x >> 3;
@@ -1147,14 +1180,15 @@
   const int pyr = (slot % groups) * 8 + xcd;
   if (pyr >= P.batch) return;
   strips_role<VEC16, HOOKS, ALIAS, ORBK, BUCK>(P, pyramids, pyr_stride, stage_kp, strip_count, score_dump, score_stride, prof, ovf,
-                                         stage_desc, smem, sh_ctr, pyr, slot / groups);
+                                         stage_desc, (const StripRec *)ptab, smem, sh_ctr, pyr, slot / groups);
 }
 
 template <bool VEC16, bool HOOKS>
 __global__ __launch_bounds__(NT) void k_fused_overflow(
     const FusedParams P, const uint8_t *__restrict__ pyramids, size_t pyr_stride,
     uint32_t *__restrict__ stage_kp, uint32_t *__restrict__ strip_count,
-    uint8_t *__restrict__ score_dump, size_t score_stride, const uint32_t *__restrict__ ovf) {
+    uint8_t *__restrict__ score_dump, size_t score_stride, const uint32_t *__restrict__ ovf,
+    const uint32_t *__restrict__ ptab) {
   extern __shared__ __attribute__((aligned(16))) uint8_t smem[];
   __shared__ uint32_t sh_ctr[8];
   const uint32_t n = ovf[0];
@@ -1167,36 +1201,21 @@
     asm volatile("" : "+s"(pyr_o), "+s"(sg_o));
     asm volatile("" : "+v"(tid_o));
     if (pyr_o >= P.batch || sg_o >= P.strips_per_pyr) continue;
-    int li = 0;
-    while (li + 1 < P.nlevels && sg_o >= P.lv[li + 1].strip0) li++;
-    const FusedLevel L = P.lv[li];
-    const int s = sg_o - L.strip0;
+    const StripRec *recs = (const StripRec *)ptab;
+    const FusedLevel L = P.lv[recs[sg_o].st.flags >> 8];
     const StripLds m = strip_lds<false>(smem, L);
-    const uint8_t *im = pyramids + (size_t)pyr_o * pyr_stride + (size_t)L.row0 * P.vstep + L.col0;
-    const ptrdiff_t lim = (ptrdiff_t)P.rows * P.vstep - ((ptrdiff_t)L.row0 * P.vstep + L.col0);
     const StripArgs A{P.border, P.thr, P.ablate, P.dump_score, P.lbs, P.limit, P.vstep, P.slots_per_pyr,
                       P.strips_per_pyr, P.hthr, P.words, 0};
-    const int ys = A.border + s * L.R;
-    const int ye = min(ys + L.R, L.h - A.border);
     bool issued = false;
     bool deferred = false;
-    strip_body<VEC16, HOOKS, false, false, true>(A, L, pyr_o, s, ys, ye, m.tile, m.sc, m.queues, m.shq, sh_ctr, sh_ctr, deferred, im, lim, stage_kp,
+    strip_body<VEC16, HOOKS, false, false, true>(A, L, pyr_o, (uint32_t)sg_o, recs, m.tile, m.sc, m.queues, m.shq, sh_ctr, sh_ctr, deferred, stage_kp,
                                     strip_count, score_dump, score_stride, false, tid_o, nullptr, pf, false, false, issued,
-                                    nullptr, 0u, nullptr, nullptr, 0u);
+                                    nullptr, 0u, nullptr, pyramids + (size_t)pyr_o * pyr_stride, (uint32_t)((size_t)P.rows * P.vstep));
     lds_barrier();
   }
 }
 
-struct PlanStrip {
-  int li;
-  int s;
-};
-__device__ __forceinline__ PlanStrip plan_strip(const FusedParams &P, int i) {
-  int li = 0;
-  while (li + 1 < P.nlevels && i >= P.lv[li + 1].strip0) li++;
-  return {li, i - P.lv[li].strip0};
-}
-__device__ __forceinline__ uint32_t strip_slot_of(const FusedParams &P, int li, int s) {
+__host__ __device__ __forceinline__ uint32_t strip_slot_of(const FusedParams &P, int li, int s) {
   return (uint32_t)(P.lv[li].slot0 + s * (P.lv[li].R >> 1) * P.lv[li].nbx);
 }
 template <class OFF>
@@ -1229,7 +1248,7 @@
                                                 const uint32_t *__restrict__ strip_count,
                                                 uint32_t *__restrict__ kp, size_t kp_stride,
                                                 uint32_t cap, uint32_t *__restrict__ counts,
-                                                uint32_t *__restrict__ ovf_reset) {
+                                                uint32_t *__restrict__ ovf_reset, const uint32_t *__restrict__ gtab) {
   extern __shared__ uint32_t soff[];
   __shared__ uint32_t wsum[4];
   __shared__ uint32_t carry;
@@ -1269,11 +1288,11 @@
   for (int st = wv; st < S; st += 4) {
     const uint32_t n = soff[st + 1] - soff[st];
     if (n == 0) continue;
-    const PlanStrip ps = plan_strip(P, st);
-    const uint32_t *list = stage + strip_slot_of(P, ps.li, ps.s);
+    const uint32_t ss = gtab[st], pr = gtab[S + st];
+    const uint32_t *list = stage + (ss & 0x7fffffffu);
     for (uint32_t k = lane; k < n; k += 64) {
       const uint32_t v = list[k];
-      const uint32_t pos = final_position(P, soff, stage, ps.li, ps.s, k, v);
+      const uint32_t pos = final_position(P, soff, stage, (int)(pr >> 24), (int)(pr & 0xffffffu), k, v);
       if (pos < cap) kp[(size_t)pyr * kp_stride + pos] = v;
     }
   }
@@ -1456,8 +1475,9 @@
                                          const uint32_t *__restrict__ stage_kp, const uint32_t *__restrict__ strip_count,
                                          const uint32_t *__restrict__ stage_desc, uint32_t *__restrict__ kp, size_t kp_stride,
                                          uint32_t cap, uint32_t *__restrict__ counts, uint32_t *__restrict__ desc,
-                                         size_t desc_stride, int words, uint32_t per_max, uint8_t *osm_all, const int pyr,
-                                         const int ch, const int nch, WAIT wait_producers = WAIT()) {
+                                         size_t desc_stride, int words, uint32_t per_max, const uint32_t *__restrict__ gtab,
+                                         uint8_t *osm_all, const int pyr, const int ch, const int nch,
+                                         WAIT wait_producers = WAIT()) {
   OrbShared *sh = (OrbShared *)osm_all;
   uint8_t *osm = osm_all + sizeof(OrbShared);
   sh->rtab[threadIdx.x] = ::g_vrecpe_tab.v[threadIdx.x];
@@ -1472,10 +1492,7 @@
   uint32_t *sslot = soff + ((S + 1 + 3) & ~3);
   uint32_t *kpl = sslot + ((S + 3) & ~3);
   uint32_t *kpos = kpl + per_max;
-  for (int i = tid; i < S; i += 256) {
-    const PlanStrip ps = plan_strip(P, i);
-    sslot[i] = strip_slot_of(P, ps.li, ps.s) | (P.lv[ps.li].gn > 1 ? 0x80000000u : 0u);
-  }
+  for (int i = tid; i < S; i += 256) sslot[i] = gtab[i];
 
   const uint32_t *cnt = strip_count + (size_t)pyr * S;
   if (tid == 0) sh->carry = 0;
@@ -1531,8 +1548,8 @@
       const uint32_t v = stage[(ss & 0x7fffffffu) + k];
       uint32_t pos = e;
       if (ss >> 31) {
-        const PlanStrip ps = plan_strip(P, a);
-        pos = final_position(P, soff, stage, ps.li, ps.s, k, v);
+        const uint32_t pr = gtab[S + a];
+        pos = final_position(P, soff, stage, (int)(pr >> 24), (int)(pr & 0xffffffu), k, v);
       }
       if (pos >= cap) continue;
       kp[(size_t)pyr * kp_stride + pos] = v;
@@ -1580,7 +1597,8 @@
     const uint32_t *__restrict__ stage_kp, const uint32_t *__restrict__ strip_count,
     const uint32_t *__restrict__ stage_desc,
     uint32_t *__restrict__ kp, size_t kp_stride, uint32_t cap, uint32_t *__restrict__ counts,
-    uint32_t *__restrict__ desc, size_t desc_stride, int words, uint32_t per_max, uint32_t *__restrict__ ovf_reset) {
+    uint32_t *__restrict__ desc, size_t desc_stride, int words, uint32_t per_max, uint32_t *__restrict__ ovf_reset,
+    const uint32_t *__restrict__ gtab) {
   asm volatile("" ::: "v79");
   extern __shared__ __attribute__((aligned(16))) uint8_t osm[];
   if (ovf_reset && blockIdx.x == 0 && blockIdx.y == 0 && threadIdx.x == 0) {
@@ -1588,7 +1606,7 @@
     ovf_reset[0] = 0;
   }
   orb_role<NoWait, GHOOKS>(P, pyramids, pyr_stride, stage_kp, strip_count, stage_desc, kp, kp_stride, cap, counts, desc, desc_stride,
-                           words, per_max, osm, (int)blockIdx.y, (int)blockIdx.x, (int)gridDim.x);
+                           words, per_max, gtab, osm, (int)blockIdx.y, (int)blockIdx.x, (int)gridDim.x);
 }
 
 constexpr int FRAME_SYNC_PYR = 8, FRAME_SYNC_DONE = 8, FRAME_SYNC_POISON = 9, FRAME_SYNC_WORDS = 12;
@@ -1598,14 +1616,15 @@
                                               uint32_t *__restrict__ kp, size_t kp_stride, uint32_t cap,
                                               uint32_t *__restrict__ counts, uint32_t *__restrict__ desc, size_t desc_stride,
                                               int words, uint32_t per_max, int nch, uint32_t *__restrict__ sync,
-                                              uint32_t *__restrict__ ovf, uint32_t *__restrict__ hflag, uint32_t test) {
+                                              uint32_t *__restrict__ ovf, uint32_t *__restrict__ hflag, uint32_t test,
+                                              const uint32_t *__restrict__ ptab) {
   extern __shared__ __attribute__((aligned(16))) uint8_t smem[];
   __shared__ uint32_t sh_ctr[16];
   const int n_strip = P.batch * P.runs_per_pyr;
   if ((int)blockIdx.x < n_strip) {
     const int pyr = (int)blockIdx.x % P.batch, run = (int)blockIdx.x / P.batch;
     strips_role<true, false, true, false, false, true>(P, pyramids, pyr_stride, stage_kp, strip_count, nullptr, 0, nullptr, ovf,
-                                                       nullptr, smem, sh_ctr, pyr, run);
+                                                       nullptr, (const StripRec *)ptab, smem, sh_ctr, pyr, run);
     __syncthreads();
     if (threadIdx.x == 0 && !((test & 1u) && blockIdx.x == 0))
       (void)__hip_atomic_fetch_add(&sync[pyr], 1u, __ATOMIC_RELEASE, __HIP_MEMORY_SCOPE_AGENT);
@@ -1637,7 +1656,7 @@
     return sh_ok != 0;
   };
   orb_role(P, pyramids, pyr_stride, stage_kp, strip_count, nullptr, kp, kp_stride, cap, counts, desc, desc_stride, words, per_max,
-           smem, pyr, ch, nch, wait);
+           ptab + plan_tab_gather(P.strips_per_pyr), smem, pyr, ch, nch, wait);
   __syncthreads();
   if (threadIdx.x == 0 && sh_ok != 0) {
     const uint32_t done = __hip_atomic_fetch_add(&sync[FRAME_SYNC_DONE], 1u, __ATOMIC_RELAXED, __HIP_MEMORY_SCOPE_AGENT);
diff --git a/pislam_amd/csrc/pislam_hip.hip b/pislam_amd/csrc/pislam_hip.hip
--- a/pislam_amd/csrc/pislam_hip.hip
+++ b/pislam_amd/csrc/pislam_hip.hip
@@ -110,6 +110,7 @@
   };
   std::vector<PlanTable *> plan_tables;
   const uint32_t *cur_utab = nullptr;
+  const uint32_t *cur_ptab = nullptr;
   DevBuf w_sync;
   uint32_t *frame_flag = nullptr;
   uint32_t *frame_flag_dev = nullptr;
@@ -1419,6 +1420,60 @@
   return t;
 }
 
+std::vector<uint32_t> strip_table(const pf::FusedParams &F, const pf::FusedParams *U) {
+  const int S = F.strips_per_pyr, Su = U ? U->strips_per_pyr : 0;
+  std::vector<uint32_t> t(pf::plan_tab_units(S) + 2 * (size_t)Su, 0u);
+  const int B = F.border;
+  const int64_t vstep = F.vstep, img_bytes = (int64_t)F.rows * vstep;
+  const int xbase = (B - 4) & ~15;
+  for (int l = 0; l < F.nlevels; l++) {
+    const pf::FusedLevel &L = F.lv[l];
+    const int vpr = L.tpitch >> 4;
+    const int64_t origin = (int64_t)L.row0 * vstep + L.col0 + xbase;
+    auto row_ofs = [&](int y) { return origin + (int64_t)y * vstep; };
+    auto inside = [&](int y_last) { return row_ofs(y_last) + L.tpitch <= img_bytes; };
+    for (int s = 0; s < L.nstrips; s++) {
+      pf::StripRec r{};
+      const int ys = B + s * L.R, ye = std::min(ys + L.R, L.h - B);
+      r.out.ys = ys;
+      r.out.own_rows = ye - ys;
+      const int y_lo = ys - 4, nrows = std::min(ye + 6, L.h) - y_lo;
+      const int r_lo = ys - 1 < B ? 1 : 0, r_hi = std::min(ye + 2, L.h - B) - (ys - 1);
+      r.st.rows = (uint32_t)nrows | ((uint32_t)r_hi << 16);
+      r.st.src = (uint32_t)row_ofs(y_lo);
+      r.st.nvec = nrows * vpr;
+      r.st.nvec_c = (nrows - 10) * vpr;
+      r.run.lin_lo = r_lo * L.tpitch;
+      r.run.lin_n = std::max(r_hi - r_lo, 0) * L.tpitch;
+      r.run.lin_lo_c = 3 * L.tpitch;
+      r.run.lin_n_c = std::max(r_hi - 3, 0) * L.tpitch;
+      r.out.slot = pf::strip_slot_of(F, l, s);
+      r.out.add_xy = ((uint32_t)L.col0 << 12) | (uint32_t)L.row0;
+      r.st.flags = (r_lo ? pf::STRIP_RLO1 : 0u) | (inside(y_lo + nrows - 1) ? 0u : pf::STRIP_TAIL) | ((uint32_t)l << 8);
+      if (s + 1 < L.nstrips && L.R >= 10 && L.R * vpr <= pf::PF_MAX * pf::NT) {
+        const int ylo_n = ye - 4, ye_n = std::min(ye + L.R, L.h - B);
+        const int nrows_n = std::min(ye_n + 6, L.h) - ylo_n;
+        if (inside(ylo_n + nrows_n - 1)) {
+          r.st.flags |= pf::STRIP_PF;
+          r.st.src_n = (uint32_t)row_ofs(ylo_n + 10);
+          r.st.nvec_n = (nrows_n - 10) * vpr;
+        }
+      }
+      memcpy(t.data() + (size_t)pf::REC_DW * (L.strip0 + s), &r, sizeof(r));
+    }
+  }
+  auto gather_arrays = [&](const pf::FusedParams &G, uint32_t *g) {
+    for (int l = 0; l < G.nlevels; l++)
+      for (int s = 0; s < G.lv[l].nstrips; s++) {
+        g[G.lv[l].strip0 + s] = pf::strip_slot_of(G, l, s) | (G.lv[l].gn > 1 ? 0x80000000u : 0u);
+        g[G.strips_per_pyr + G.lv[l].strip0 + s] = ((uint32_t)l << 24) | (uint32_t)s;
+      }
+  };
+  gather_arrays(F, t.data() + pf::plan_tab_gather(S));
+  if (U) gather_arrays(*U, t.data() + pf::plan_tab_units(S));
+  return t;
+}
+
 constexpr int FRAME_MAX_BATCH = 8;
 constexpr int FRAME_DEFAULT_BATCH = 2;
 inline int frame_max_batch(const pislam_ctx *c) { return c->opt_frame <= 0 ? 0 : c->opt_frame == 1 ? FRAME_DEFAULT_BATCH : std::min(c->opt_frame, FRAME_MAX_BATCH); }
@@ -1439,6 +1494,7 @@
   pf::SelectPlan Q{};
   pf::FusedParams U{};
   std::vector<uint32_t> utab;
+  std::vector<uint32_t> ptab;
   size_t sel_lds = 0, glds = 0;
   bool alias = false;
   size_t ovf_stride = 0, sdesc_per_pyr = 0;
@@ -1461,6 +1517,7 @@
     P->utab = unit_table(p, F, P->Q);
     P->sel_lds = sizeof(uint32_t) * pf::SEL_WAVES * (64 + 2 * (size_t)P->Q.nb_max);
   }
+  P->ptab = strip_table(F, P->sel ? &P->U : nullptr);
   const int Sg = P->sel ? P->Q.units_per_pyr : S;
   P->sdesc_per_pyr = F.orb_in_strip ? (size_t)S * pf::QS_SHARED * (size_t)p->words : 0;
   P->alias = c->opt_alias && submax <= 65535 && S <= 65535;
@@ -1545,6 +1602,49 @@
   return nullptr;
 }
 
+const char *strip_table_violation(const FrontendPlan &P, const pislam_frontend_params *p) {
+  const pf::FusedParams &F = P.F;
+  const int S = F.strips_per_pyr, B = p->border;
+  const int Su = P.sel ? P.U.strips_per_pyr : 0;
+  if (P.ptab.size() != pf::plan_tab_units(S) + 2 * (size_t)Su) return "strip table size";
+  const int64_t img_bytes = (int64_t)p->rows * p->vstep;
+  const uint32_t *gsl = P.ptab.data() + pf::plan_tab_gather(S), *gpr = gsl + S;
+  uint32_t slot_end = 0;
+  for (int l = 0; l < F.nlevels; l++) {
+    const pf::FusedLevel &L = F.lv[l];
+    const int vpr = L.tpitch >> 4;
+    int y = B;
+    for (int s = 0; s < L.nstrips; s++) {
+      pf::StripRec r;
+      memcpy(&r, P.ptab.data() + (size_t)pf::REC_DW * (L.strip0 + s), sizeof(r));
+      const pf::StripStage &st = r.st;
+      const int ys = r.out.ys, ye = ys + r.out.own_rows;
+      if (ys != y || ys >= ye || ye > L.h - B || r.out.own_rows > L.R) return "record rows";
+      y = ye;
+      const int nrows = (int)(st.rows & 0xffff), r_hi = (int)(st.rows >> 16);
+      if (nrows < 11 || nrows > L.R + 10 || r_hi > L.R + 3 || (int)(st.flags >> 8) != l) return "record tile rows";
+      if (st.nvec != nrows * vpr || st.nvec_c != (nrows - 10) * vpr) return "record vectors";
+      if (r.run.lin_lo + r.run.lin_n > (L.R + 3) * L.tpitch || r.run.lin_lo_c + r.run.lin_n_c > (L.R + 3) * L.tpitch ||
+          r.run.lin_lo < 0 || r.run.lin_n < 0 || r.run.lin_lo_c != 3 * L.tpitch || r.run.lin_n_c < 0)
+        return "record prefilter run";
+      if (!(st.flags & pf::STRIP_TAIL) && (int64_t)st.src + (int64_t)(nrows - 1) * p->vstep + L.tpitch > img_bytes) return "staged rows";
+      if (st.flags & pf::STRIP_PF) {
+        if (s + 1 >= L.nstrips || st.nvec_n <= 0 || st.nvec_n > pf::PF_MAX * pf::NT || st.nvec_n % vpr) return "prefetch vectors";
+        if ((int64_t)st.src_n + (int64_t)(st.nvec_n / vpr - 1) * p->vstep + L.tpitch > img_bytes) return "prefetch outside the pyramid";
+        if (st.src_n != st.src + (uint32_t)((L.R + 10) * p->vstep)) return "prefetch source";
+      }
+      if (r.out.slot < slot_end) return "record slots overlap";
+      slot_end = r.out.slot + (uint32_t)((L.R / 2) * L.nbx);
+      if (slot_end > (uint32_t)F.slots_per_pyr) return "record slots";
+      if ((gsl[L.strip0 + s] & 0x7fffffffu) != r.out.slot || (gsl[L.strip0 + s] >> 31) != (L.gn > 1 ? 1u : 0u) ||
+          gpr[L.strip0 + s] != (((uint32_t)l << 24) | (uint32_t)s))
+        return "gather arrays";
+    }
+    if (L.nstrips > 0 && y != L.h - B) return "records do not tile the entry";
+  }
+  return nullptr;
+}
+
 const char *select_plan_violation(const FrontendPlan &P, const pislam_frontend_params *p) {
   const pf::SelectPlan &Q = P.Q;
   int units = 0, uslots = 0;
@@ -1600,6 +1700,7 @@
       return fail(c, PISLAM_ERR_NOMEM, "hipMalloc(bucket selection staging)");
     PCHK(plan_table(c, P.utab, &c->cur_utab));
   }
+  PCHK(plan_table(c, P.ptab, &c->cur_ptab));
   return PISLAM_OK;
 }
 
@@ -1610,8 +1711,9 @@
   } while (0)
 
 using StripKernT = void (*)(const pf::FusedParams, const uint8_t *, size_t, uint32_t *, uint32_t *, uint8_t *, size_t,
-                            unsigned long long *, uint32_t *, uint32_t *);
-using OvfKernT = void (*)(const pf::FusedParams, const uint8_t *, size_t, uint32_t *, uint32_t *, uint8_t *, size_t, const uint32_t *);
+                            unsigned long long *, uint32_t *, uint32_t *, const uint32_t *);
+using OvfKernT = void (*)(const pf::FusedParams, const uint8_t *, size_t, uint32_t *, uint32_t *, uint8_t *, size_t, const uint32_t *,
+                          const uint32_t *);
 
 StripKernT strip_kernel(bool vec, bool alias, bool hooks, bool orb_in_strip, int lbs) {
   static const StripKernT kerns[8] = {
@@ -1688,7 +1790,7 @@
   hipLaunchKernelGGL(pf::k_frame, dim3(grid), dim3(pf::NT), P.flds, c->stream, F, k.pyramids, k.stride, c->w_stage.as<uint32_t>(),
                      c->w_stripcnt.as<uint32_t>(), k.kp, (size_t)p->max_keypoints, (uint32_t)p->max_keypoints, k.counts, k.desc,
                      (size_t)p->max_keypoints * p->words, p->words, (uint32_t)P.fper, P.fch, c->w_sync.as<uint32_t>(),
-                     c->w_ovf.as<uint32_t>(), c->frame_flag_dev, (uint32_t)c->opt_frame_test);
+                     c->w_ovf.as<uint32_t>(), c->frame_flag_dev, (uint32_t)c->opt_frame_test, c->cur_ptab);
   PCHK(launch_ok(c, "k_frame"));
   c->last_path = PISLAM_PATH_FUSED | PISLAM_PATH_ONE_LAUNCH;
   HIPCHK(c, hipEventRecord(c->ev[1], c->stream));
@@ -1725,7 +1827,7 @@
   for (int rep = 0; rep < std::max(1, c->opt_repeat_strips); rep++) {
     if (rep && ovf) HIPCHK(c, hipMemsetAsync(ovf, 0, sizeof(uint32_t), M));
     hipLaunchKernelGGL(k.kern, grid, dim3(pf::NT), P.klds, M, F, s_pyr, k.stride, s_stage, s_cnt, s_dump, dump_stride, prof, ovf,
-                       s_sdesc);
+                       s_sdesc, c->cur_ptab);
   }
   if (prof) PCHK(report_strip_profile(c, prof, prof_n, M, (double)S * n, grid.x));
   PCHK(launch_ok(c, "k_fused_strips"));
@@ -1743,12 +1845,13 @@
   }
   if (P.alias) {
     hipLaunchKernelGGL(k.okern, dim3((unsigned)std::max(8, c->num_cus / 2)), dim3(pf::NT), P.lds, X, F, s_pyr, k.stride, s_stage,
-                       s_cnt, s_dump, dump_stride, (const uint32_t *)ovf);
+                       s_cnt, s_dump, dump_stride, (const uint32_t *)ovf, c->cur_ptab);
     PCHK(launch_ok(c, "k_fused_overflow"));
   }
   if (nsub == 1) HIPCHK(c, hipEventRecord(c->ev[2], M));
   pf::FusedParams G = F;
   const uint32_t *g_stage = s_stage, *g_cnt = s_cnt;
+  const uint32_t *g_tab = c->cur_ptab + pf::plan_tab_gather(S);
   if (P.sel) {
     uint32_t *u_stage = c->w_ustage.as<uint32_t>() + (size_t)first * P.Q.uslots_per_pyr;
     uint32_t *u_cnt = c->w_ucount.as<uint32_t>() + (size_t)first * P.Q.units_per_pyr;
@@ -1759,17 +1862,18 @@
     G.batch = n;
     g_stage = u_stage;
     g_cnt = u_cnt;
+    g_tab = c->cur_ptab + pf::plan_tab_units(S);
   }
   if (P.generic_orb) {
     c->last_path |= PISLAM_PATH_GENERIC_ORB;
     hipLaunchKernelGGL(pf::k_gather, dim3(n), dim3(256), P.glds, X, G, g_stage, g_cnt, s_kp,
-                       (size_t)p->max_keypoints, (uint32_t)p->max_keypoints, s_counts, ovf);
+                       (size_t)p->max_keypoints, (uint32_t)p->max_keypoints, s_counts, ovf, g_tab);
     PCHK(launch_ok(c, "k_gather"));
     return launch_orb_batch(c, X, p, s_pyr, k.stride, n, s_kp, s_counts, s_desc);
   }
   hipLaunchKernelGGL(k.gkern, dim3(P.nch, n), dim3(256), P.olds, X, G, s_pyr, k.stride, g_stage, g_cnt,
                      (const uint32_t *)s_sdesc, s_kp, (size_t)p->max_keypoints, (uint32_t)p->max_keypoints, s_counts,
-                     s_desc, (size_t)p->max_keypoints * p->words, p->words, (uint32_t)P.per_max, ovf);
+                     s_desc, (size_t)p->max_keypoints * p->words, p->words, (uint32_t)P.per_max, ovf, g_tab);
   return launch_ok(c, "k_gather_orb");
 }
 
@@ -1844,8 +1948,9 @@
 
 }
 
-PISLAM_EXPORT int pislam_debug_build_plan(const pislam_frontend_params *p, const pislam_level *lv, int batch, int num_cus,
-                                          int lanes_in_flight, const char *options, uint32_t summary[8], char *err, size_t err_cap) {
+namespace {
+int debug_build_plan(const pislam_frontend_params *p, const pislam_level *lv, int batch, int num_cus, int lanes_in_flight,
+                     const char *options, uint32_t summary[8], std::vector<uint32_t> *table, char *err, size_t err_cap) {
   pislam_ctx c;
   auto say = [&](int rc) {
     if (err && err_cap) snprintf(err, err_cap, "%s", c.err.c_str());
@@ -1893,6 +1998,27 @@
     if (const char *what = select_plan_violation(P, p)) return bad(what);
     summary[7] = (uint32_t)P.Q.units_per_pyr;
   }
+  if (const char *what = strip_table_violation(P, p)) return bad(what);
+  if (table) *table = P.ptab;
+  return PISLAM_OK;
+}
+}
+
+PISLAM_EXPORT int pislam_debug_build_plan(const pislam_frontend_params *p, const pislam_level *lv, int batch, int num_cus,
+                                          int lanes_in_flight, const char *options, uint32_t summary[8], char *err, size_t err_cap) {
+  return debug_build_plan(p, lv, batch, num_cus, lanes_in_flight, options, summary, nullptr, err, err_cap);
+}
+
+PISLAM_EXPORT int pislam_debug_build_plan_table(const pislam_frontend_params *p, const pislam_level *lv, int batch, int num_cus,
+                                                int lanes_in_flight, const char *options, uint32_t summary[8], uint32_t *table,
+                                                size_t table_cap, size_t *table_n, char *err, size_t err_cap) {
+  if (!table_n) return PISLAM_ERR_INVALID;
+  *table_n = 0;
+  std::vector<uint32_t> t;
+  const int rc = debug_build_plan(p, lv, batch, num_cus, lanes_in_flight, options, summary, &t, err, err_cap);
+  if (rc != PISLAM_OK) return rc;
+  *table_n = t.size();
+  if (table && !t.empty()) memcpy(table, t.data(), sizeof(uint32_t) * std::min(t.size(), table_cap));
   return PISLAM_OK;
 }
 
```

New measurement: 1.219 billion. About the same (-0.9%).
